# PRBonn/semantic_suma

Measured on AMD Instinct MI355X. Metric: scans_per_sec, higher is better.
Workload: dtype f32; 1 GPU; BASELINE configs[1]: synthetic KITTI-like sequence, 64x2048 range images, semantic-weighted ICP (10 GN iterations + stats pass) + surfel fusion, one sequence per GPU, scans resident in HBM, processScan called scan after scan by the native host loop (suma_pipeline_run_scans); timed after 300 untimed scans of the same sequence (5 warm-up + pre-roll to the steady map size: 1016645 surfels at the star; preroll_scans=300, map_surfels_start=1016645, map_surfels_end=2308753, parallelism=single GPU

## Files before the change

### semantic_suma_amd/core.py

```python
from __future__ import annotations

import ctypes as C
import os

import numpy as np

from .types import (ACC_WORDS, DRAW_COLORS, DRAW_LIGHTS, DRAW_MATERIAL, DRAW_MAX_LIGHTS, SURFEL_DTYPE, DrawParams,
                    IcpStats, LoopParams, LoopStatus, PosegraphParams, PosegraphStats, SemanticKnnParams,
                    SemanticParams, SumaParams, WORLD_SURFEL_DTYPE, WorldParams, WorldStats, CheckpointInfo,
                    LocalizerParams, LocalizerResult)

_HERE = os.path.dirname(os.path.abspath(__file__))
LIB_PATH = os.environ.get("SUMA_HIP_LIB") or os.path.join(_HERE, "libsuma_hip.so")
_LIB = None


class SumaError(RuntimeError):
    """Raised for every negative return code of the C-ABI (the reference throws std::runtime_error)."""


class LoopResult(C.Structure):
    _fields_ = [("gn_pose", C.c_double * 16), ("after_minimize", IcpStats), ("passed", C.c_int32),
                ("pose_old", C.c_float * 16), ("composed", IcpStats), ("JtJ", C.c_double * 36)]

# ... 6 lines not shown
class ScanRef(C.Structure):
    _fields_ = [("points", C.c_void_p), ("labels", C.c_void_p), ("probs", C.c_void_p), ("n", C.c_uint32)]


class SequenceJob(C.Structure):
    _fields_ = [("scans", C.POINTER(ScanRef)), ("n_scans", C.c_uint32), ("on_device", C.c_int32)]


class SequenceResult(C.Structure):
    _fields_ = [("status", C.c_int32), ("scans_done", C.c_uint32), ("map_surfels", C.c_uint32), ("track_loss", C.c_uint32),
                ("end_pose", C.c_double * 16), ("seconds", C.c_double), ("error", C.c_char * 160)]


class HypothesisJob(C.Structure):
    _fields_ = [("scans", C.POINTER(ScanRef)), ("n_scans", C.c_uint32), ("on_device", C.c_int32),
                ("perturbations", C.c_void_p), ("n_hyp", C.c_uint32), ("rank", C.c_uint32), ("world", C.c_uint32)]


EXCHANGE_FN = C.CFUNCTYPE(C.c_int, C.c_void_p, C.POINTER(C.c_double), C.POINTER(C.c_double), C.c_uint32)


class IcpObjective(C.Structure):
    _fields_ = [("icp_max_distance", C.c_float), ("icp_max_angle", C.c_float), ("weight_function", C.c_int32),
                ("factor", C.c_float), ("bilinear_sampling", C.c_int32)]


class KernelTime(C.Structure):
    _fields_ = [("name", C.c_char * 48), ("launches", C.c_uint64), ("total_ms", C.c_double), ("bytes", C.c_double)]


def lib():
    global _LIB
    if _LIB is not None:
        return _LIB
    if not os.path.exists(LIB_PATH):
        raise SumaError(f"{LIB_PATH} not found: build it with `make -C semantic_suma_amd/csrc` "
                        "(there is no CPU fallback for the HIP path)")
    L = C.CDLL(LIB_PATH)
    vp, u32, i32, f32 = C.c_void_p, C.c_uint32, C.c_int32, C.c_float
    pp = C.POINTER(vp)
    L.suma_version.restype = C.c_char_p
    L.suma_posegraph_last_error.restype = C.c_char_p
    L.suma_posegraph_last_error.argtypes = [vp]
    L.suma_posegraph_create.argtypes = [C.c_int, u32, u32, pp]
    L.suma_posegraph_destroy.argtypes = [vp]
    L.suma_posegraph_destroy.restype = None
    L.suma_posegraph_clear.argtypes = [vp]
    L.suma_posegraph_clone.argtypes = [vp, pp]
    L.suma_posegraph_set_initial.argtypes = [vp, i32, vp]
    L.suma_posegraph_add_edge.argtypes = [vp, i32, i32, vp, vp]
    L.suma_posegraph_pose.argtypes = [vp, i32, vp]
    L.suma_posegraph_poses.argtypes = [vp, vp, u32, C.POINTER(u32)]
    L.suma_posegraph_size.argtypes = [vp]
    L.suma_posegraph_size.restype = i32
    L.suma_posegraph_edge_count.argtypes = [vp]
    L.suma_posegraph_edge_count.restype = u32
    L.suma_posegraph_error.argtypes = [vp, C.POINTER(C.c_double)]
    L.suma_posegraph_reinitialize.argtypes = [vp]
    L.suma_posegraph_optimize.argtypes = [vp, u32, C.POINTER(PosegraphParams), C.POINTER(PosegraphStats)]
    L.suma_posegraph_linearize.argtypes = [vp, vp, vp, vp, vp, vp, vp, u32, C.POINTER(u32)]
    L.suma_posegraph_reserve.argtypes = [vp, u32, u32]
    L.suma_posegraph_edge.argtypes = [vp, u32, C.POINTER(i32), C.POINTER(i32), vp, vp]
    L.suma_loop_params_default.argtypes = [C.POINTER(LoopParams)]
    L.suma_loop_params_default.restype = None
    L.suma_pipeline_enable_loop_closing.argtypes = [vp, C.POINTER(LoopParams)]
    L.suma_pipeline_check_loop_closure.argtypes = [vp]
    L.suma_pipeline_loop_status.argtypes = [vp, C.POINTER(LoopStatus)]
    L.suma_pipeline_posegraph.argtypes = [vp]
    L.suma_pipeline_posegraph.restype = vp
    L.suma_pipeline_trajectory_distances.argtypes = [vp, vp, u32, C.POINTER(u32)]
    L.suma_loop_find_candidate.argtypes = [vp, vp, u32, vp, f32, f32, i32]
    L.suma_loop_find_candidate.restype = i32
    L.suma_last_error.restype = C.c_char_p
    L.suma_last_error.argtypes = [vp]
    L.suma_ctx_create.argtypes = [C.POINTER(SumaParams), C.c_int, pp]
    L.suma_ctx_destroy.argtypes = [vp]
    L.suma_ctx_destroy.restype = None
    L.suma_set_params.argtypes = [vp, C.POINTER(SumaParams)]
    L.suma_synchronize.argtypes = [vp]
    L.suma_ctx_stream.restype = vp
    L.suma_ctx_stream.argtypes = [vp]
    L.suma_frame_create.argtypes = [vp, u32, u32, pp]
    L.suma_frame_destroy.argtypes = [vp]
    L.suma_frame_destroy.restype = None
    L.suma_frame_copy.argtypes = [vp, vp, vp]
    L.suma_frame_download.argtypes = [vp, vp, C.c_int, vp]
    L.suma_frame_upload.argtypes = [vp, vp, C.c_int, vp]
    L.suma_frame_width.restype = u32
    L.suma_frame_width.argtypes = [vp]
    L.suma_frame_height.restype = u32
    L.suma_frame_height.argtypes = [vp]
    L.suma_frame_device_ptr.restype = vp
    L.suma_frame_device_ptr.argtypes = [vp, C.c_int]
    L.suma_frame_swap.argtypes = [vp, vp, vp]
    L.suma_frame_export.argtypes = [vp, vp, C.c_int, pp, C.POINTER(u32), C.POINTER(u32), C.POINTER(u32)]
    L.suma_icp_set_objective.argtypes = [vp, C.POINTER(IcpObjective)]
    L.suma_icp_information.argtypes = [vp, vp]
    L.suma_map_export_surfels.argtypes = [vp, pp, C.POINTER(u32)]
    L.suma_map_export_data_surfels.argtypes = [vp, pp, C.POINTER(u32), C.POINTER(u32)]
    L.suma_pipeline_prefetch_scan.argtypes = [vp, vp, vp, vp, u32]
    L.suma_pipeline_process_prefetched.argtypes = [vp, i32]
    L.suma_pipeline_process_scan_async.argtypes = [vp, vp, vp, vp, u32, i32]
    L.suma_device_download.argtypes = [vp, vp, vp, C.c_uint64]
    L.suma_preprocess.argtypes = [vp, vp, vp, vp, u32, u32, vp]
    L.suma_preprocess_device.argtypes = [vp, vp, vp, vp, u32, u32, vp]
    L.suma_icp_set_data.argtypes = [vp, vp, vp]
    L.suma_icp_jacobian_products.argtypes = [vp, vp, u32, vp, vp, vp, C.POINTER(IcpStats)]
    L.suma_icp_minimize.argtypes = [vp, vp, vp, vp, u32, C.POINTER(u32), C.POINTER(IcpStats)]
    L.suma_icp_history.argtypes = [vp, vp, u32, C.POINTER(u32)]
    L.suma_icp_history_sequence.argtypes = [vp]
    L.suma_icp_history_sequence.restype = C.c_uint64
    L.suma_frame_touch.argtypes = [vp, vp]
    L.suma_pipeline_minimize_stats.argtypes = [vp, C.POINTER(IcpStats)]
    L.suma_icp_minimize_batch.argtypes = [vp, vp, u32, vp, vp]
    L.suma_map_reset.argtypes = [vp]
    L.suma_map_update.argtypes = [vp, vp, vp]
    L.suma_map_render.argtypes = [vp, vp, vp, f32, vp]
    L.suma_map_render_active.argtypes = [vp, vp, f32]
    L.suma_map_render_inactive.argtypes = [vp, vp, f32]
    L.suma_map_render_composed.argtypes = [vp, vp, vp, f32]
    L.suma_map_frame.restype = vp
    L.suma_map_frame.argtypes = [vp, C.c_int]
    L.suma_map_update_poses.argtypes = [vp, vp, u32]
    L.suma_map_size.argtypes = [vp, C.POINTER(u32)]
    L.suma_map_timestamp.argtypes = [vp, C.POINTER(u32)]
    L.suma_map_download.argtypes = [vp, vp, u32, C.POINTER(u32)]
    L.suma_map_upload.argtypes = [vp, vp, u32, u32]
    L.suma_map_download_index_map.argtypes = [vp, vp]
    L.suma_map_download_radius_conf.argtypes = [vp, vp]
    L.suma_map_download_poses.argtypes = [vp, vp, u32, C.POINTER(u32)]
    L.suma_map_download_integrated.argtypes = [vp, vp]
    L.suma_map_counts.argtypes = [vp, C.POINTER(u32), C.POINTER(u32), C.POINTER(u32), vp]
    L.suma_map_cache_stats.argtypes = [vp, C.POINTER(u32), C.POINTER(u32), C.POINTER(u32)]
    L.suma_map_download_cached_tile.argtypes = [vp, C.c_int32, C.c_int32, vp, u32, C.POINTER(u32)]
    L.suma_icp_set_iteration.argtypes = [vp, u32]
    L.suma_pipeline_host_entry_times.argtypes = [vp, vp, C.c_int]
    L.suma_loop_closure_verify.argtypes = [vp, vp, vp, vp, u32, vp, f32, f32, f32, C.POINTER(LoopResult)]
    L.suma_loop_closure_verify_serial.argtypes = [vp, vp, vp, vp, u32, vp, f32, f32, f32, C.POINTER(LoopResult)]
    L.suma_pipeline_create.argtypes = [C.POINTER(SumaParams), C.c_int, pp]
    L.suma_pipeline_destroy.argtypes = [vp]
    L.suma_pipeline_destroy.restype = None
    L.suma_pipeline_ctx.restype = vp
    L.suma_pipeline_ctx.argtypes = [vp]
    L.suma_pipeline_process_scan.argtypes = [vp, vp, vp, vp, u32, i32]
    L.suma_pipeline_process_scan_device.argtypes = [vp, vp, vp, vp, u32, i32]
    L.suma_pipeline_pose.argtypes = [vp, vp]
    L.suma_pipeline_begin_scan.argtypes = [vp, vp, vp, vp, u32]
    L.suma_pipeline_begin_scan_device.argtypes = [vp, vp, vp, vp, u32]
    L.suma_pipeline_begin_prefetched.argtypes = [vp]
    L.suma_pipeline_update_pose.argtypes = [vp, i32]
    L.suma_pipeline_update_map.argtypes = [vp]
    L.suma_pipeline_integrate_loop_closures.argtypes = [vp, vp, u32, vp]
    L.suma_pipeline_set_pose_old.argtypes = [vp, vp]
    L.suma_pipeline_get_pose.argtypes = [vp, C.c_int, vp]
    L.suma_pipeline_result_new.argtypes = [vp, C.POINTER(IcpStats)]
    L.suma_pipeline_verify_loop_closure.argtypes = [vp, vp, vp, u32, f32, f32, C.POINTER(LoopResult)]
    L.suma_pipeline_track_loop_closure.argtypes = [vp, C.c_double, C.c_double, C.c_double, C.POINTER(LoopTrack)]
    L.suma_loop_closure_track.argtypes = [vp, vp, vp, vp, vp, f32, C.c_double, C.c_double, C.c_double, C.POINTER(LoopTrack)]
    L.suma_se3_log.argtypes = [vp, vp]
    L.suma_se3_log.restype = None
    L.suma_pipeline_reset.argtypes = [vp]
    L.suma_pipeline_minimize_hypotheses.argtypes = [vp, vp, u32, i32, vp, vp]
    L.suma_pipeline_apply_increment.argtypes = [vp, vp]
    L.suma_run_sequences.argtypes = [C.POINTER(SumaParams), C.c_int, C.POINTER(SequenceJob), u32, u32, i32,
                                     C.POINTER(SequenceResult)]
    L.suma_run_hypotheses.argtypes = [C.POINTER(SumaParams), C.c_int, C.POINTER(HypothesisJob), i32, EXCHANGE_FN, vp, vp,
                                      vp, C.c_char_p]
    L.suma_pipeline_run_scans.argtypes = [vp, C.POINTER(SequenceJob), i32, C.POINTER(u32), vp]
    L.suma_pipeline_last_increment.argtypes = [vp, vp]
    L.suma_pipeline_last_stats.argtypes = [vp, C.POINTER(IcpStats)]
    L.suma_pipeline_timestamp.restype = u32
    L.suma_pipeline_timestamp.argtypes = [vp]
    L.suma_pipeline_track_loss.restype = u32
    L.suma_pipeline_track_loss.argtypes = [vp]
    L.suma_pipeline_frame.restype = vp
    L.suma_pipeline_frame.argtypes = [vp, C.c_int]
    sp = C.POINTER(SemanticParams)
    L.suma_semantic_project.argtypes = [vp, sp, vp, u32, vp, vp, vp]
    L.suma_semantic_unproject.argtypes = [vp, sp, vp, C.c_int, vp, u32, vp, vp]
    L.suma_pipeline_begin_scan_scores.argtypes = [vp, sp, vp, vp, C.c_int, vp, u32, vp]
    L.suma_pipeline_process_scan_scores.argtypes = [vp, sp, vp, vp, C.c_int, vp, u32, vp, i32]
    kp = C.POINTER(SemanticKnnParams)
    L.suma_semantic_unproject_knn.argtypes = [vp, sp, kp, vp, vp, C.c_int, vp, vp, u32, vp, vp]
    L.suma_pipeline_begin_scan_scores_knn.argtypes = [vp, sp, kp, vp, vp, C.c_int, vp, vp, u32, vp]
    L.suma_pipeline_process_scan_scores_knn.argtypes = [vp, sp, kp, vp, vp, C.c_int, vp, vp, u32, vp, i32]
    L.suma_map_draw.argtypes = [vp, C.POINTER(DrawParams), vp, vp]
    L.suma_world_params_default.argtypes = [C.POINTER(WorldParams)]
    L.suma_world_params_default.restype = None
    L.suma_map_cached_tiles.argtypes = [vp, vp, u32, C.POINTER(u32)]
    L.suma_map_export_world.argtypes = [vp, C.POINTER(WorldParams), vp, u32, C.POINTER(WorldStats)]
    L.suma_device_alloc.argtypes = [vp, C.c_uint64, pp]
    L.suma_device_free.argtypes = [vp, vp]
    L.suma_device_upload.argtypes = [vp, vp, vp, C.c_uint64]
    L.suma_profile_enable.argtypes = [vp, C.c_int]
    L.suma_profile_reset.argtypes = [vp]
    L.suma_profile_get.argtypes = [vp, C.POINTER(KernelTime), u32]
    u64p = C.POINTER(C.c_uint64)
    L.suma_pipeline_checkpoint_size.argtypes = [vp, u64p]
    L.suma_pipeline_checkpoint_save.argtypes = [vp, vp, C.c_uint64, u64p]
    L.suma_pipeline_checkpoint_load.argtypes = [vp, vp, C.c_uint64]
    L.suma_checkpoint_info.argtypes = [vp, C.c_uint64, C.POINTER(CheckpointInfo)]
    L.suma_checkpoint_params.argtypes = [vp, C.c_uint64, C.POINTER(SumaParams)]
    L.suma_checkpoint_digest.argtypes = [vp, C.c_uint64]
    L.suma_checkpoint_digest.restype = C.c_uint64
    lpp, lrp = C.POINTER(LocalizerParams), C.POINTER(LocalizerResult)
    L.suma_localizer_params_default.argtypes = [C.POINTER(SumaParams), lpp]
    L.suma_localizer_params_default.restype = None
    L.suma_localizer_create.argtypes = [C.POINTER(SumaParams), lpp, C.c_int, pp]
    L.suma_localizer_destroy.argtypes = [vp]
    L.suma_localizer_destroy.restype = None
    L.suma_localizer_ctx.argtypes = [vp]
    L.suma_localizer_ctx.restype = vp
    L.suma_localizer_set_map.argtypes = [vp, vp, u32, C.POINTER(u32)]
    L.suma_localizer_set_map_device.argtypes = [vp, vp, u32, C.POINTER(u32)]
    L.suma_localizer_set_pose.argtypes = [vp, vp]
    L.suma_localizer_process_scan.argtypes = [vp, vp, vp, vp, u32, i32, lrp]
    L.suma_localizer_process_scan_device.argtypes = [vp, vp, vp, vp, u32, i32, lrp]
    L.suma_localizer_window.argtypes = [vp, vp, C.POINTER(u32), C.POINTER(u32)]
    L.suma_localizer_download_window.argtypes = [vp, vp, u32, C.POINTER(u32)]
    _LIB = L
    return L


def _ptr(a):
    return None if a is None else a.ctypes.data_as(C.c_void_p)


def _cm(T, dtype):
    return np.ascontiguousarray(np.asarray(T, dtype=dtype).reshape(4, 4).T)


class Context:

    def __init__(self, params: SumaParams, device: int = 0, handle=None, owner=None):
        self.L = lib()
        self.params = params
        self._owner = owner
        if handle is None:
            h = C.c_void_p()
            rc = self.L.suma_ctx_create(C.byref(params), device, C.byref(h))
            if rc != 0:
                raise SumaError(f"suma_ctx_create failed ({rc}): {self.L.suma_last_error(None).decode()}")
            self.h, self.owned = h, True
        else:
            self.h, self.owned = handle, False

    def check(self, rc: int, what: str = ""):
        if rc != 0:
            raise SumaError(f"{what} failed ({rc}): {self.L.suma_last_error(self.h).decode()}")

    def set_params(self, params: SumaParams):
        self.check(self.L.suma_set_params(self.h, C.byref(params)), "suma_set_params")
        self.params = params

    def synchronize(self):
        self.check(self.L.suma_synchronize(self.h), "suma_synchronize")

    @property
    def stream(self) -> int:
        return int(self.L.suma_ctx_stream(self.h) or 0)

    def device_array(self, host: np.ndarray) -> int:
        host = np.ascontiguousarray(host)
        p = C.c_void_p()
        self.check(self.L.suma_device_alloc(self.h, host.nbytes, C.byref(p)), "suma_device_alloc")
        self.check(self.L.suma_device_upload(self.h, p, _ptr(host), host.nbytes), "suma_device_upload")
        return p.value

    def device_download(self, d_ptr: int, nbytes: int) -> np.ndarray:
        out = np.empty(nbytes, dtype=np.uint8)
        self.check(self.L.suma_device_download(self.h, _ptr(out), C.c_void_p(d_ptr), nbytes), "suma_device_download")
        return out

    def device_free(self, p: int):
        self.check(self.L.suma_device_free(self.h, C.c_void_p(p)), "suma_device_free")

    def profile(self, on):
        self.check(self.L.suma_profile_enable(self.h, int(on)))

    def profile_reset(self):
        self.check(self.L.suma_profile_reset(self.h))

    def profile_get(self):
        buf = (KernelTime * 64)()
        n = self.L.suma_profile_get(self.h, buf, 64)
        if n < 0:
            self.check(n, "suma_profile_get")
        return [dict(name=buf[i].name.decode(), launches=int(buf[i].launches), total_ms=float(buf[i].total_ms),
                     bytes=float(buf[i].bytes)) for i in range(min(n, 64))]

    def close(self):
        if getattr(self, "owned", False) and self.h:
            self.L.suma_ctx_destroy(self.h)
            self.h = None

    def __del__(self):
        try:
            self.close()
        except Exception:
            pass


class Frame:

    def __init__(self, ctx: Context, width: int, height: int, handle=None):
        self.ctx, self.width, self.height = ctx, width, height
        if handle is None:
            h = C.c_void_p()
            ctx.check(ctx.L.suma_frame_create(ctx.h, width, height, C.byref(h)), "suma_frame_create")
            self.h, self.owned = h, True
        else:
            self.h, self.owned = C.c_void_p(handle), False

    def download(self, which: int) -> np.ndarray:
        out = np.empty((self.height, self.width, 4), dtype=np.float32)
        self.ctx.check(self.ctx.L.suma_frame_download(self.ctx.h, self.h, which, _ptr(out)), "suma_frame_download")
        return out

    def upload(self, which: int, data: np.ndarray):
        data = np.ascontiguousarray(data, dtype=np.float32).reshape(self.height, self.width, 4)
        self.ctx.check(self.ctx.L.suma_frame_upload(self.ctx.h, self.h, which, _ptr(data)), "suma_frame_upload")

    def set(self, vertex, normal, semantic):
        self.upload(0, vertex)
        self.upload(1, normal)
        self.upload(2, semantic)

    @property
    def vertex(self):
        return self.download(0)

    @property
    def normal(self):
        return self.download(1)

    @property
    def semantic(self):
        return self.download(2)

    def swap(self, other: "Frame"):
        self.ctx.check(self.ctx.L.suma_frame_swap(self.ctx.h, self.h, other.h), "suma_frame_swap")

    def export(self, which: int):
        p, w, h, rb = C.c_void_p(), C.c_uint32(0), C.c_uint32(0), C.c_uint32(0)
        self.ctx.check(self.ctx.L.suma_frame_export(self.ctx.h, self.h, which, C.byref(p), C.byref(w), C.byref(h),
                                                    C.byref(rb)), "suma_frame_export")
        return p.value, w.value, h.value, rb.value

    def touch(self):
        self.ctx.check(self.ctx.L.suma_frame_touch(self.ctx.h, self.h), "suma_frame_touch")

    def copy(self, other: "Frame"):
        self.ctx.check(self.ctx.L.suma_frame_copy(self.ctx.h, self.h, other.h), "suma_frame_copy")

    def __del__(self):
        try:
            if getattr(self, "owned", False) and self.h and self.ctx.h:
                self.ctx.L.suma_frame_destroy(self.h)
                self.h = None
        except Exception:
            pass


class Preprocessing:

    def __init__(self, ctx: Context):
        self.ctx = ctx

    def process(self, points, frame: Frame, labels, probs, timestamp: int) -> Frame:
        points = np.ascontiguousarray(points, dtype=np.float32).reshape(-1, 4)
        labels = None if labels is None else np.ascontiguousarray(labels, dtype=np.float32)
        probs = None if probs is None else np.ascontiguousarray(probs, dtype=np.float32)
        c = self.ctx
        c.check(c.L.suma_preprocess(c.h, _ptr(points), _ptr(labels), _ptr(probs), points.shape[0], timestamp, frame.h),
                "suma_preprocess")
        return frame


class Frame2Model:
    num_parameters = 6
    _PARAM_NAMES = {"icp-max-distance": "icp_max_distance", "icp-max-angle": "icp_max_angle", "factor": "factor",
                    "bilinear_sampling": "bilinear_sampling"}
    _WEIGHTING = {"none": 0, "huber": 1, "turkey": 2, "stability": 3}

    def __init__(self, ctx: Context, params: SumaParams = None):
        self.ctx = ctx
        p = ctx.params if params is None else params
        self.objective = IcpObjective(p.icp_max_distance, p.icp_max_angle, p.weight_function, p.factor,
                                      p.bilinear_sampling)
        self._current = self._last = None
        self._pose = np.eye(4)
        self._iteration = 0
        self.stats = IcpStats()
        self.acc = np.zeros(ACC_WORDS, dtype=np.int64)

    def setParameter(self, name: str, value):
        if name == "weighting":
            self.objective.weight_function = self._WEIGHTING[value]
        elif name in self._PARAM_NAMES:
            setattr(self.objective, self._PARAM_NAMES[name], value)

    def setData(self, current: Frame, last: Frame):
        self._current, self._last = current, last
        self._iteration = 0

    def _bind(self):
        if self._current is None:
            raise SumaError("Frame2Model::setData has not been called")
        c = self.ctx
        c.check(c.L.suma_icp_set_data(c.h, self._current.h, self._last.h), "suma_icp_set_data")
# ... 1065 lines not shown
```

### semantic_suma_amd/csrc/k_render.hip

```cpp
#include <cstring>

#include "suma_internal.h"
#define EXDIV_FN __device__ __forceinline__
#include "exact_div.h"

enum { TIE_LOW_INDEX = 0, TIE_HIGH_INDEX_OLD = 1, TIE_HIGH_INDEX_NEW = 2 };

struct RenderSlot {
  int enabled;
  int mode;
  int tie;
  unsigned long long* zbuf;
  m4 inv_pose;
};

struct RenderArgs {
  const suma_surfel* surfels;
  const DevState* ds;
  const float* poses;
  proj_t q;
  float conf_threshold;
  int use_stability;
  int32_t thr;
  RenderSlot slot[2];
  int merged;
  const float* inv_pose_dev;
  int k7_enabled;
  int k7_same_proj;
  proj_t k7_q;
  unsigned long long* k7_zbuf;
};

struct rvtx {
  int32_t X, Y;
  float z, tu, tv;
};

__device__ __forceinline__ double edge_fn(const rvtx& a, const rvtx& b, int32_t px, int32_t py) {
  const double ux = (double)(b.X - a.X), uy = (double)(b.Y - a.Y), vx = (double)(px - a.X), vy = (double)(py - a.Y);
  return __builtin_fma(ux, vy, -(uy * vx));
}
__device__ __forceinline__ float edge_to_float(double w) { return (float)(w + 0.0); }
__device__ __forceinline__ bool owns_edge(const rvtx& s, const rvtx& t) {
  int32_t dx = t.X - s.X, dy = t.Y - s.Y;
  return dy > 0 || (dy == 0 && dx < 0);
}

__device__ __forceinline__ unsigned long long render_key(uint32_t z24, uint32_t id, int tie) {
  if (tie == TIE_LOW_INDEX) return ((unsigned long long)z24 << 32) | id;
  unsigned long long pass = (tie == TIE_HIGH_INDEX_OLD) ? 1u : 0u;
  return ((unsigned long long)z24 << 33) | (pass << 32) | (unsigned long long)(0xffffffffu - id);
}

__device__ __forceinline__ unsigned long long raster_key(rvtx A, rvtx B, rvtx C, int32_t i, int32_t j, uint32_t id,
                                                         int tie) {
  double area = edge_fn(A, B, C.X, C.Y);
  if (area < 0) {
    rvtx t = B;
    B = C;
    C = t;
    area = -area;
  }
  const int32_t px = 256 * i + 128, py = 256 * j + 128;
  const double w0 = edge_fn(B, C, px, py), w1 = edge_fn(C, A, px, py), w2 = edge_fn(A, B, px, py);
  const bool covered = (area != 0) && (w0 > 0 || (w0 == 0 && owns_edge(B, C))) &&
                       (w1 > 0 || (w1 == 0 && owns_edge(C, A))) && (w2 > 0 || (w2 == 0 && owns_edge(A, B)));
  unsigned long long key = SUMA_EMPTY_KEY;
  if (covered) {
    const float fa = (float)area;
#ifdef SUMA_BARY_PLAIN_DIV
    float b0 = edge_to_float(w0) / fa, b1 = edge_to_float(w1) / fa, b2 = edge_to_float(w2) / fa;
#else
    const float fr = exdiv_refine(fa, __builtin_amdgcn_rcpf(fa));
    float b0 = exdiv_quot(edge_to_float(w0), fa, fr), b1 = exdiv_quot(edge_to_float(w1), fa, fr),
          b2 = exdiv_quot(edge_to_float(w2), fa, fr);
#endif
    float tu = (b0 * A.tu + b1 * B.tu) + b2 * C.tu;
    float tv = (b0 * A.tv + b1 * B.tv) + b2 * C.tv;
    float z = (b0 * A.z + b1 * B.z) + b2 * C.z;
    if (!((tu * tu + tv * tv) > 1.0f) && (z >= 0.0f && z <= 1.0f)) key = render_key(depth24(z), id, tie);
  }
  return key;
}

__device__ __forceinline__ void surfel_to_sensor(const float* __restrict__ poses, const float* inv_pose, float count,
                                                 v3 pos, v3 nrm, v3* p, v3* n) {
  float Ps[16], M[16];
  const float4* src = reinterpret_cast<const float4*>(poses + 16 * (size_t)(int32_t)count);
#pragma unroll
  for (int k = 0; k < 4; ++k) {
    float4 col = src[k];
    Ps[4 * k] = col.x;
    Ps[4 * k + 1] = col.y;
    Ps[4 * k + 2] = col.z;
    Ps[4 * k + 3] = col.w;
  }
  m4_mul(inv_pose, Ps, M);
  *p = m4_point(M, pos);
  *n = m4_dir(M, nrm);
}

#ifdef SUMA_PHASE_TIMING
__device__ unsigned long long g_k4_phase[PH_BLOCKS][9];
extern "C" int suma_debug_k4_phases(unsigned long long* host, int reset) {
  hipError_t e = hipMemcpyFromSymbol(host, HIP_SYMBOL(g_k4_phase), sizeof(g_k4_phase));
  if (e == hipSuccess && reset) {
    void* p = nullptr;
    e = hipGetSymbolAddress(&p, HIP_SYMBOL(g_k4_phase));
    if (e == hipSuccess) e = hipMemset(p, 0, sizeof(g_k4_phase));
  }
  return (int)e;
}
#endif

#if !defined(K4_NO_PREFETCH)
#define K4_PREFETCH 1
#endif
#ifdef K4_PREFETCH
#define K4_BARRIER() lds_barrier()
#else
#define K4_BARRIER() __syncthreads()
#endif
#define RENDER_THREADS 256
#define RENDER_WAVES (RENDER_THREADS / 64)
#define RENDER_BATCH 2
#define SUMA_RENDER_MAX_BLOCKS 65536u

__device__ __forceinline__ uint32_t render_block_rank(bool flag, uint32_t* s_w, uint32_t* total) {
  const int lane = threadIdx.x & 63, wave = threadIdx.x >> 6;
  const unsigned long long ball = __ballot(flag);
  if (lane == 0) s_w[wave] = __popcll(ball);
  K4_BARRIER();
  uint32_t off = 0, tot = 0;
#pragma unroll
  for (int w = 0; w < RENDER_WAVES; ++w) {
    uint32_t c = s_w[w];
    if (w < wave) off += c;
    tot += c;
  }
  *total = tot;
  return off + __popcll(ball & ((1ull << lane) - 1ull));
}

template <bool BIG>
__global__ void __launch_bounds__(RENDER_THREADS) __attribute__((amdgpu_waves_per_eu(5, 8))) k_render(RenderArgs a) {
  __shared__ float s_cand[RENDER_THREADS][9];
  __shared__ int32_t s_rec[RENDER_THREADS][17];
  __shared__ uint32_t s_incl[RENDER_THREADS];
  __shared__ uint32_t s_w[2][RENDER_WAVES], s_w2[RENDER_WAVES];
  __shared__ uint8_t s_mask[RENDER_THREADS];
  const uint32_t S = a.ds->n_surfels;
  const float4* __restrict__ sf = reinterpret_cast<const float4*>(a.surfels);
  const int lane = threadIdx.x & 63, wave = threadIdx.x >> 6;
  const uint32_t ntile = (S + RENDER_THREADS - 1) / RENDER_THREADS;
  const int npass = a.merged ? 1 : 2;
  uint32_t trip = 0;
  float4 s0 = f4(0, 0, 0, 0), s1 = s0, s2 = s0;
  auto fetch_tile = [&](uint32_t t) {
    const uint32_t tt = t < ntile ? t : ntile - 1u;
    uint32_t j = (ntile - 1u - tt) * RENDER_THREADS + threadIdx.x;
    j = j < S ? j : S - 1u;
    s0 = sf[4 * (size_t)j];
    s1 = sf[4 * (size_t)j + 1];
    s2 = sf[4 * (size_t)j + 2];
  };
#ifdef K4_PREFETCH
  if (ntile) fetch_tile(blockIdx.x);
  const int last_pass = a.merged ? 0 : (a.slot[1].enabled ? 1 : 0);
#endif
  PH_BEGIN;
  for (uint32_t tile = blockIdx.x; tile < ntile; tile += gridDim.x) {
    PH(7);
    const uint32_t blk0 = (ntile - 1u - tile) * RENDER_THREADS;
    const uint32_t i = blk0 + threadIdx.x;
#ifndef K4_PREFETCH
    fetch_tile(tile);
#endif
    const bool live = (i < S) && !(a.use_stability && !(s1.w > a.conf_threshold));
    const float radius = s0.w, count = s2.w;
    const int32_t creation = (int32_t)count;
    const int32_t ts = (int32_t)__float_as_uint(s2.x);
#ifdef SUMA_PHASE_TIMING
    if (live && ts == 0x7fffffff) ph_acc[7] += 1;
#endif
    PH(0);
    for (int sl = 0; sl < npass; ++sl) {
      const RenderSlot& slot = a.slot[a.merged ? 1 : sl];
      if (!a.merged && !slot.enabled) continue;
      const float* inv_pose = (sl == 0 && a.inv_pose_dev != nullptr) ? a.inv_pose_dev : slot.inv_pose.m;
      uint32_t selmask;
      {
        const bool sel_old = live && (creation < a.thr), sel_new = live && (creation >= a.thr || ts >= a.thr);
        if (a.merged)
          selmask = ((sel_old && a.slot[0].enabled) ? 1u : 0u) | (sel_new ? 2u : 0u);
        else
          selmask = ((slot.mode == 0) ? sel_old : sel_new) ? (1u << sl) : 0u;
      }
      const bool selected = selmask != 0;
      const bool k7 = (sl == 0) && a.k7_enabled && (i < S);
      bool cand = false;
      unsigned long long k7_key = SUMA_EMPTY_KEY;
      uint32_t k7_pix = 0;
      v3 p = mk3(0, 0, 0), n = p;
      float ppx = 0.f;
      if (selected || k7) {
        surfel_to_sensor(a.poses, inv_pose, count, xyz(s0), xyz(s1), &p, &n);
        float lp = len3(p);
        if (dot3(n, divs3(neg3(p), lp)) > 0.01f) {
          v3 pp = mk3(0, 0, 0);
          if (selected || a.k7_same_proj) pp = project01(a.q, p);
          if (k7) {
            const v3 pr = a.k7_same_proj ? pp : project01(a.k7_q, p);
            float fx = sdm_floor(pr.x * a.k7_q.width), fy = sdm_floor(pr.y * a.k7_q.height);
            float zn = 2.0f * pr.z - 1.0f;
            if (fx >= 0.0f && fx < a.k7_q.width && fy >= 0.0f && fy < a.k7_q.height && zn >= -1.0f && zn <= 1.0f) {
              k7_key = ((unsigned long long)depth24(0.5f * zn + 0.5f) << 32) | i;
              k7_pix = (uint32_t)(int32_t)fy * (uint32_t)a.k7_q.W + (uint32_t)(int32_t)fx;
            }
          }
          if (selected) {
            cand = (pp.x >= 0.0f && pp.y >= 0.0f && pp.z >= 0.0f && pp.x < 1.0f && pp.y < 1.0f && pp.z < 1.0f);
            ppx = pp.x;
          }
        }
      }
#ifdef K4_PREFETCH
      if (sl == last_pass) fetch_tile(tile + gridDim.x);
#endif
      uint32_t ncand;
      const uint32_t crank = render_block_rank(cand, s_w[trip & 1u], &ncand);
      trip += 1;
      PH(1);
      if (ncand == 0) {
        if (k7_key != SUMA_EMPTY_KEY) zbuf_min(&a.k7_zbuf[k7_pix], k7_key);
        continue;
      }
      if (cand) {
        float* r = s_cand[crank];
        r[0] = p.x;
        r[1] = p.y;
        r[2] = p.z;
        r[3] = n.x;
        r[4] = n.y;
        r[5] = n.z;
        r[6] = radius;
        r[7] = ppx;
        r[8] = __uint_as_float(i);
        s_mask[crank] = (uint8_t)selmask;
      }
      K4_BARRIER();
      PH(2);
      uint32_t ntests = 0;
      if (threadIdx.x < ncand) {
        const float* r = s_cand[threadIdx.x];
        const v3 cp = mk3(r[0], r[1], r[2]), cn = mk3(r[3], r[4], r[5]);
        const float crad = r[6], cppx = r[7];
        v3 u = normalize3(mk3(cn.y - cn.z, -cn.x, cn.x));
        v3 v = normalize3(cross3(cn, u));
        v3 ru = scale3(crad, u), rv = scale3(crad, v);
        v3 corner[4];
        corner[0] = sub3(sub3(cp, ru), rv);
        corner[1] = sub3(add3(cp, ru), rv);
        corner[2] = add3(sub3(cp, ru), rv);
        corner[3] = add3(add3(cp, ru), rv);
        int32_t X[4], Y[4];
        float Z[4];
        bool bad = false;
#pragma unroll
        for (int k = 0; k < 4; ++k) {
          const float depth = len3(corner[k]);
          const float pitch = -sdm_asin(corner[k].z / depth);
          const float y01 = 1.0f - ((pitch * SUMA_RAD2DEG_F) + a.q.fov_up) / a.q.fov;
          Z[k] = 0.5f * (2.0f * ((depth - a.q.min_depth) / (a.q.max_depth - a.q.min_depth)) - 1.0f) + 0.5f;
          const float yw = y01 * a.q.height;
          if (sdm_isnan(yw) || sdm_isnan(Z[k])) bad = true;
          Y[k] = (int32_t)sdm_floor(yw * 256.0f + 0.5f);
        }
        const int32_t minY = min(min(Y[0], Y[1]), min(Y[2], Y[3])), maxY = max(max(Y[0], Y[1]), max(Y[2], Y[3]));
        int32_t j0 = (minY - 128 + 255) >> 8, j1 = (maxY - 128) >> 8;
        j0 = max(j0, 0);
        j1 = min(j1, a.q.H - 1);
        if (!bad && j0 <= j1) {
#pragma unroll
          for (int k = 0; k < 4; ++k) {
            const float yaw = sdm_atan2(corner[k].y, corner[k].x);
            float x01 = 0.5f * ((-yaw * SUMA_INV_PI_F) + 1.0f);
            if (cppx - x01 > 0.5f) x01 += 1.0f;
            if (x01 - cppx > 0.5f) x01 -= 1.0f;
            const float xw = x01 * a.q.width;
            if (sdm_isnan(xw)) bad = true;
            X[k] = (int32_t)sdm_floor(xw * 256.0f + 0.5f);
          }
          if (!bad) {
            const int32_t minX = min(min(X[0], X[1]), min(X[2], X[3])), maxX = max(max(X[0], X[1]), max(X[2], X[3]));
            int32_t i0 = (minX - 128 + 255) >> 8, i1 = (maxX - 128) >> 8;
            i0 = max(i0, 0);
            i1 = min(i1, a.q.W - 1);
            if (i0 <= i1) {
              const int32_t w = i1 - i0 + 1;
              ntests = (uint32_t)w * (uint32_t)(j1 - j0 + 1);
              int32_t* q = s_rec[threadIdx.x];
#pragma unroll
              for (int k = 0; k < 4; ++k) {
                q[k] = X[k];
                q[4 + k] = Y[k];
                q[8 + k] = __float_as_int(Z[k]);
              }
              q[12] = i0;
              q[13] = j0;
              q[14] = w;
              q[15] = __float_as_int(r[8]);
              q[16] = (int32_t)s_mask[threadIdx.x];
            }
          }
        }
      }
      PH(3);
      uint32_t incl = wave_inclusive_scan(ntests);
      if (lane == 63) s_w2[wave] = incl;
      K4_BARRIER();
      uint32_t woff = 0, total = 0;
#pragma unroll
      for (int w = 0; w < RENDER_WAVES; ++w) {
        uint32_t c = s_w2[w];
        if (w < wave) woff += c;
        total += c;
      }
      s_incl[threadIdx.x] = incl + woff;
      K4_BARRIER();
      PH(4);
      unsigned long long k7_cur = 0;
      if (k7_key != SUMA_EMPTY_KEY)
        k7_cur = __hip_atomic_load(&a.k7_zbuf[k7_pix], __ATOMIC_RELAXED, __HIP_MEMORY_SCOPE_AGENT);
      unsigned long long* const zb0 = a.slot[0].zbuf;
      unsigned long long* const zb1 = a.slot[1].zbuf;
      for (uint32_t t0 = threadIdx.x; t0 < total; t0 += RENDER_BATCH * RENDER_THREADS) {
        unsigned long long key[RENDER_BATCH];
        uint32_t pix[RENDER_BATCH], msk[RENDER_BATCH];
#pragma unroll
        for (int u = 0; u < RENDER_BATCH; ++u) {
          const uint32_t t = t0 + (uint32_t)u * RENDER_THREADS;
          key[u] = SUMA_EMPTY_KEY;
          pix[u] = 0;
          msk[u] = 0;
          if (t < total) {
            int lo = 0, hi = RENDER_THREADS - 1;
#pragma unroll
            for (int it = 0; it < 8; ++it) {
              int mid = (lo + hi) >> 1;
              if (s_incl[mid] > t)
                hi = mid;
              else
                lo = mid + 1;
            }
            const int src = lo;
            const uint32_t excl = src ? s_incl[src - 1] : 0u;
            const int32_t* r = s_rec[src];
            const uint32_t q = t - excl, w = (uint32_t)r[14];
            const uint32_t qj = BIG ? q / w : (uint32_t)(((float)q + 0.5f) * __builtin_amdgcn_rcpf((float)w));
            const uint32_t qi = q - __umul24(qj, w);
            const int32_t pi = r[12] + (int32_t)qi, pj = r[13] + (int32_t)qj;
            rvtx vt[4];
#pragma unroll
            for (int k = 0; k < 4; ++k) {
              vt[k].X = r[k];
              vt[k].Y = r[4 + k];
              vt[k].z = __int_as_float(r[8 + k]);
              vt[k].tu = (k & 1) ? 1.0f : -1.0f;
              vt[k].tv = (k & 2) ? 1.0f : -1.0f;
            }
            const uint32_t id = (uint32_t)r[15];
            const unsigned long long ka = raster_key(vt[0], vt[1], vt[2], pi, pj, id, slot.tie);
            const unsigned long long kb = raster_key(vt[2], vt[1], vt[3], pi, pj, id, slot.tie);
            key[u] = ka < kb ? ka : kb;
            pix[u] = __umul24((uint32_t)pj, (uint32_t)a.q.W) + (uint32_t)pi;
            msk[u] = (uint32_t)r[16];
          }
        }
        unsigned long long cur0[RENDER_BATCH], cur1[RENDER_BATCH];
#pragma unroll
        for (int u = 0; u < RENDER_BATCH; ++u) {
          cur0[u] = cur1[u] = 0;
          if (key[u] != SUMA_EMPTY_KEY) {
            if (msk[u] & 1u) cur0[u] = __hip_atomic_load(&zb0[pix[u]], __ATOMIC_RELAXED, __HIP_MEMORY_SCOPE_AGENT);
            if (msk[u] & 2u) cur1[u] = __hip_atomic_load(&zb1[pix[u]], __ATOMIC_RELAXED, __HIP_MEMORY_SCOPE_AGENT);
          }
        }
#pragma unroll
        for (int u = 0; u < RENDER_BATCH; ++u) {
          if (key[u] < cur0[u]) atomicMin(&zb0[pix[u]], key[u]);
          if (key[u] < cur1[u]) atomicMin(&zb1[pix[u]], key[u]);
        }
      }
      if (k7_key < k7_cur) atomicMin(&a.k7_zbuf[k7_pix], k7_key);
      PH(5);
      K4_BARRIER();
      PH(6);
    }
  }
  PH_END(g_k4_phase);
}

__device__ __forceinline__ uint32_t key_id(unsigned long long key, int tie) {
  uint32_t low = (uint32_t)(key & 0xffffffffull);
  return tie == TIE_LOW_INDEX ? low : (0xffffffffu - low);
}

struct ResolveOut {
  float4 v, n, s;
};

__device__ __forceinline__ ResolveOut resolve_pixel(unsigned long long key, int tie, const suma_surfel* surfels,
                                                    const float* poses, const float* inv_a, const float* inv_b) {
  ResolveOut o;
  if (key == SUMA_EMPTY_KEY) {
    o.v = o.n = o.s = f4(0.f, 0.f, 0.f, 0.f);
    return o;
  }
  uint32_t id = key_id(key, tie);
  const float4* sf = reinterpret_cast<const float4*>(surfels) + 4 * (size_t)id;
  float4 s0 = sf[0], s1 = sf[1], s2 = sf[2], s3 = sf[3];
  const float* inv = inv_a;
  if (tie != TIE_LOW_INDEX && ((key >> 32) & 1ull) == 0) inv = inv_b;
  v3 p, n;
  surfel_to_sensor(poses, inv, s2.w, xyz(s0), xyz(s1), &p, &n);
  o.v = f4(p.x, p.y, p.z, 1.0f);
  o.n = f4(n.x, n.y, n.z, 1.0f);
  o.s = s3;
  return o;
}

struct ResolveArgs {
  const suma_surfel* surfels;
  const float* poses;
  unsigned long long *zbuf_a, *zbuf_b;
  m4 inv_a, inv_b;
  int tie;
  uint32_t Pm;
  float max_distance;
  float4 *va, *na, *sa;
  float4 *vb, *nb, *sb;
  float4 *vo, *no, *so;
  float4 *vm, *nm, *sm;
  const float4* sm_src;
  const float* inv_dev;
};

__global__ void __launch_bounds__(256) k_resolve(ResolveArgs a) {
  uint32_t pix = blockIdx.x * blockDim.x + threadIdx.x;
  if (pix >= a.Pm) return;
  unsigned long long key = a.zbuf_a[pix];
  a.zbuf_a[pix] = SUMA_EMPTY_KEY;
  const float* ia = a.inv_dev ? a.inv_dev : a.inv_a.m;
  const float* ib = a.inv_dev ? a.inv_dev : a.inv_b.m;
  ResolveOut o = resolve_pixel(key, a.tie, a.surfels, a.poses, ia, ib);
  if (a.va) a.va[pix] = o.v;
  if (a.na) a.na[pix] = o.n;
  if (a.sa) a.sa[pix] = o.s;
  if (a.vm) {
    a.vm[pix] = o.v;
    a.nm[pix] = o.n;
    a.sm[pix] = a.sm_src[pix];
  }
}

__global__ void __launch_bounds__(256) k_resolve_compose(ResolveArgs a) {
  uint32_t pix = blockIdx.x * blockDim.x + threadIdx.x;
  if (pix >= a.Pm) return;
  unsigned long long ka = a.zbuf_a[pix], kb = a.zbuf_b[pix];
  a.zbuf_a[pix] = SUMA_EMPTY_KEY;
  a.zbuf_b[pix] = SUMA_EMPTY_KEY;
  ResolveOut o = resolve_pixel(ka, TIE_LOW_INDEX, a.surfels, a.poses, a.inv_a.m, a.inv_a.m);
  ResolveOut nw = resolve_pixel(kb, TIE_LOW_INDEX, a.surfels, a.poses, a.inv_b.m, a.inv_b.m);
  a.va[pix] = o.v;
  a.na[pix] = o.n;
  a.sa[pix] = o.s;
  a.vb[pix] = nw.v;
  a.nb[pix] = nw.n;
  a.sb[pix] = nw.s;
  float4 v = nw.v, n = nw.n, s = nw.s;
  bool valid = (o.v.w > 0.5f && o.n.w > 0.5f);
  bool new_valid = (v.w > 0.5f && n.w > 0.5f);
  if (!new_valid && valid && (v.w < 0.5f || len3(sub3(xyz(v), xyz(o.v))) < a.max_distance)) {
    v = o.v;
    n = o.n;
    s = o.s;
  }
  a.vo[pix] = v;
  a.no[pix] = n;
  a.so[pix] = s;
}

static void set_m4(m4& d, const float* s) {
  for (int i = 0; i < 16; ++i) d.m[i] = s[i];
}

static void run_render(suma_ctx* c, const RenderArgs& a, uint32_t grid) {
  if ((size_t)a.q.W * (size_t)a.q.H >= ((size_t)1 << 21))
    k_render<true><<<grid, RENDER_THREADS, 0, c->ls>>>(a);
  else
    k_render<false><<<grid, RENDER_THREADS, 0, c->ls>>>(a);
}
static RenderArgs render_args(suma_ctx* c, float conf_threshold, int32_t thr) {
  RenderArgs a;
  a.surfels = c->surfels[c->cur];
  a.ds = c->ds;
  a.poses = c->poses;
  a.q = c->pm;
  a.conf_threshold = conf_threshold;
  a.use_stability = c->p.use_stability;
  a.thr = thr;
  a.slot[0].enabled = a.slot[1].enabled = 0;
  a.slot[0].zbuf = a.slot[1].zbuf = c->zbuf_a;
  a.slot[0].tie = a.slot[1].tie = TIE_LOW_INDEX;
  a.merged = 0;
  a.inv_pose_dev = nullptr;
  a.k7_enabled = 0;
  a.k7_q = c->pd;
  a.k7_same_proj = (memcmp(&c->pd, &c->pm, sizeof(proj_t)) == 0) ? 1 : 0;
  a.k7_zbuf = c->zbuf_data;
  return a;
}
static uint32_t stream_grid(suma_ctx* c) {
  uint64_t est = (uint64_t)c->known_surfels + 2 * c->P;
  uint64_t blocks = (est + 255) / 256;
  if (blocks > SUMA_RENDER_MAX_BLOCKS) blocks = SUMA_RENDER_MAX_BLOCKS;
  if (blocks < 256) blocks = 256;
  return (uint32_t)blocks;
}
static ResolveArgs resolve_args(suma_ctx* c) {
  ResolveArgs r;
  memset(&r, 0, sizeof(r));
  r.surfels = c->surfels[c->cur];
  r.poses = c->poses;
  r.zbuf_a = c->zbuf_a;
  r.zbuf_b = c->zbuf_b;
  r.Pm = (uint32_t)c->Pm;
  r.max_distance = c->p.max_loop_closure_distance;
  return r;
}

hipError_t launch_map_render(suma_ctx* c, const float* pose_old, const float* pose_new, float conf_threshold,
                             suma_frame* out) {
  float inv_old[16], inv_new[16];
  rigid_inverse_f(pose_old, inv_old);
  rigid_inverse_f(pose_new, inv_new);
  const double S = (double)c->known_surfels;
  const uint32_t Pm = (uint32_t)c->Pm;
  if (c->p.compose_rendering) {
    int32_t thr = (int32_t)(c->timestamp - 100u);
    RenderArgs a = render_args(c, conf_threshold, thr);
    a.slot[0].enabled = thr > 0 ? 1 : 0;
    a.slot[0].mode = 0;
    a.slot[0].tie = TIE_LOW_INDEX;
    a.slot[0].zbuf = c->zbuf_a;
    set_m4(a.slot[0].inv_pose, inv_old);
    a.slot[1].enabled = 1;
    a.slot[1].mode = 1;
    a.slot[1].tie = TIE_LOW_INDEX;
    a.slot[1].zbuf = c->zbuf_b;
    set_m4(a.slot[1].inv_pose, inv_new);
    a.merged = (memcmp(inv_old, inv_new, sizeof(inv_old)) == 0 && !getenv("SUMA_RENDER_NO_MERGE")) ? 1 : 0;
    {
      ProfScope ps(c, "k4_render_surfels", 64.0 * S);
      run_render(c, a, stream_grid(c));
    }
    ResolveArgs r = resolve_args(c);
    set_m4(r.inv_a, inv_old);
    set_m4(r.inv_b, inv_new);
    r.va = c->old_frame->map[0];
    r.na = c->old_frame->map[1];
    r.sa = c->old_frame->map[2];
    r.vb = c->new_frame->map[0];
    r.nb = c->new_frame->map[1];
    r.sb = c->new_frame->map[2];
    r.vo = out->map[0];
    r.no = out->map[1];
    r.so = out->map[2];
    {
      ProfScope ps(c, "k5_resolve_compose", (16.0 + 144.0) * Pm);
      k_resolve_compose<<<(Pm + 255) / 256, 256, 0, c->ls>>>(r);
    }
  } else {
    RenderArgs a = render_args(c, conf_threshold, 0);
    a.slot[0].enabled = 1;
    a.slot[0].mode = 1;
    a.slot[0].tie = TIE_LOW_INDEX;
    a.slot[0].zbuf = c->zbuf_a;
    set_m4(a.slot[0].inv_pose, inv_old);
    {
      ProfScope ps(c, "k4_render_surfels", 64.0 * S);
      run_render(c, a, stream_grid(c));
    }
    ResolveArgs r = resolve_args(c);
    set_m4(r.inv_a, inv_old);
    set_m4(r.inv_b, inv_old);
    r.tie = TIE_LOW_INDEX;
    r.va = out->map[0];
    r.na = out->map[1];
    r.sa = out->map[2];
    {
      ProfScope ps(c, "k5_resolve", (8.0 + 48.0) * Pm);
      k_resolve<<<(Pm + 255) / 256, 256, 0, c->ls>>>(r);
    }
    size_t bytes = c->Pm * sizeof(float4);
    for (int m = 0; m < 3; ++m) {
      hipMemcpyAsync(c->new_frame->map[m], out->map[m], bytes, hipMemcpyDeviceToDevice, c->ls);
      hipMemcpyAsync(c->old_frame->map[m], out->map[m], bytes, hipMemcpyDeviceToDevice, c->ls);
    }
  }
  return hipGetLastError();
}

hipError_t launch_map_render_single(suma_ctx* c, const float* pose, float conf_threshold, int active, int fuse_k7,
                                    suma_frame* mirror) {
  float inv[16] = {1, 0, 0, 0, 0, 1, 0, 0, 0, 0, 1, 0, 0, 0, 0, 1};
  if (pose) rigid_inverse_f(pose, inv);
  int32_t thr = (int32_t)(c->timestamp - 100u);
  RenderArgs a = render_args(c, conf_threshold, thr);
  if (!pose) a.inv_pose_dev = c->pose_block + 16;
  a.slot[0].enabled = 1;
  a.slot[0].mode = active ? 1 : 0;
  a.slot[0].tie = TIE_LOW_INDEX;
  a.slot[0].zbuf = c->zbuf_a;
  set_m4(a.slot[0].inv_pose, inv);
  a.k7_enabled = fuse_k7;
  {
    ProfScope ps(c, fuse_k7 ? "k4k7_render_indexmap" : "k4_render_surfels", 64.0 * (double)c->known_surfels);
    run_render(c, a, stream_grid(c));
  }
  ResolveArgs r = resolve_args(c);
  set_m4(r.inv_a, inv);
  set_m4(r.inv_b, inv);
  r.tie = TIE_LOW_INDEX;
  if (!pose) r.inv_dev = c->pose_block + 16;
  suma_frame* tgt = active ? c->new_frame : c->old_frame;
  r.va = tgt->map[0];
  r.na = tgt->map[1];
  r.sa = nullptr;
  if (mirror) {
    r.vm = mirror->map[0];
    r.nm = mirror->map[1];
    r.sm = mirror->map[2];
    r.sm_src = tgt->map[2];
  }
  {
    ProfScope ps(c, "k5_resolve", (8.0 + 32.0 + (mirror ? 64.0 : 0.0)) * (double)c->Pm);
    k_resolve<<<((uint32_t)c->Pm + 255) / 256, 256, 0, c->ls>>>(r);
  }
  return hipGetLastError();
}

hipError_t launch_map_render_composed(suma_ctx* c, const float* pose_old, const float* pose_new,
                                      float conf_threshold) {
  float inv_old[16], inv_new[16];
  rigid_inverse_f(pose_old, inv_old);
  rigid_inverse_f(pose_new, inv_new);
  int32_t thr = (int32_t)(c->timestamp - 100u);
  RenderArgs a = render_args(c, conf_threshold, thr);
  a.slot[0].enabled = 1;
  a.slot[0].mode = 0;
  a.slot[0].tie = TIE_HIGH_INDEX_OLD;
  a.slot[0].zbuf = c->zbuf_a;
  set_m4(a.slot[0].inv_pose, inv_old);
  a.slot[1].enabled = 1;
  a.slot[1].mode = 1;
  a.slot[1].tie = TIE_HIGH_INDEX_NEW;
  a.slot[1].zbuf = c->zbuf_a;
  set_m4(a.slot[1].inv_pose, inv_new);
  {
    ProfScope ps(c, "k4_render_surfels", 64.0 * (double)c->known_surfels);
    run_render(c, a, stream_grid(c));
  }
  ResolveArgs r = resolve_args(c);
  set_m4(r.inv_a, inv_old);
  set_m4(r.inv_b, inv_new);
  r.tie = TIE_HIGH_INDEX_OLD;
  r.va = c->composed_frame->map[0];
  r.na = c->composed_frame->map[1];
  r.sa = nullptr;
  {
    ProfScope ps(c, "k5_resolve", (8.0 + 32.0) * (double)c->Pm);
    k_resolve<<<((uint32_t)c->Pm + 255) / 256, 256, 0, c->ls>>>(r);
  }
  return hipGetLastError();
}
```

### semantic_suma_amd/csrc/k_update.hip

```cpp
#include <cstddef>
#include <cstring>

#include "suma_internal.h"

#define ST_AGG 1u
#define ST_INC 2u

__device__ __forceinline__ unsigned long long st_pack(uint32_t epoch, uint32_t flag, uint32_t value) {
  return ((unsigned long long)epoch << 34) | ((unsigned long long)flag << 32) | value;
}

struct Pair {
  uint32_t a, x;
};
__device__ __forceinline__ void lookback_publish(unsigned long long* __restrict__ status,
                                                 unsigned long long* __restrict__ group, uint32_t tile, uint32_t agg,
                                                 uint32_t epoch, uint32_t aggx = 0) {
  __hip_atomic_store(&status[tile], st_pack(epoch, ST_AGG, (aggx << 16) | agg), __ATOMIC_RELAXED, __HIP_MEMORY_SCOPE_AGENT);
  __hip_atomic_fetch_add(&group[tile >> 6], (1ull << 56) | ((unsigned long long)aggx << 32) | (unsigned long long)agg,
                         __ATOMIC_RELAXED, __HIP_MEMORY_SCOPE_AGENT);
}
#define SUMA_SPIN_LIMIT (1u << 26)
#ifndef LB_BATCH
#define LB_BATCH 4
// ... 37 lines not shown
  if (timed_out) {
    atomicOr(fault, 8u);
    atomicOr(fault + (offsetof(DevState, fault_site) - offsetof(DevState, overflow)) / 4, 0x2u);
  }
  Pair r;
  r.a = (uint32_t)__builtin_amdgcn_readlane((int)wave_inclusive_scan(sum), 63);
  r.x = PAIR ? (uint32_t)__builtin_amdgcn_readlane((int)wave_inclusive_scan(sumx), 63) : 0u;
  return r;
}
__device__ __forceinline__ uint32_t lookback_collect(unsigned long long* __restrict__ status,
                                                     unsigned long long* __restrict__ group, uint32_t tile, uint32_t epoch,
                                                     int lane, uint32_t* __restrict__ fault) {
  return lookback_collect2<false>(status, group, tile, epoch, lane, fault).a;
}
__device__ uint32_t lookback_prefix(unsigned long long* __restrict__ status, unsigned long long* __restrict__ group,
                                    uint32_t tile, uint32_t agg, uint32_t epoch, int lane, uint32_t* __restrict__ fault) {
  if (lane == 0) lookback_publish(status, group, tile, agg, epoch);
  return lookback_collect(status, group, tile, epoch, lane, fault);
}

struct BlockRank {
  uint32_t rank, total;
};
#define TILE_WAVES (SUMA_TILE / 64)
__device__ __forceinline__ BlockRank block_rank(bool flag, uint32_t* s_wave ) {
  const int lane = threadIdx.x & 63, wave = threadIdx.x >> 6;
  const unsigned long long ball = __ballot(flag);
  const uint32_t below = __popcll(ball & ((1ull << lane) - 1ull));
  if (lane == 0) s_wave[wave] = __popcll(ball);
  __syncthreads();
  uint32_t off = 0, tot = 0;
#pragma unroll
  for (int w = 0; w < (int)TILE_WAVES; ++w) {
    uint32_t cnt = s_wave[w];
    if (w < wave) off += cnt;
    tot += cnt;
  }
  BlockRank r;
  r.rank = off + below;
  r.total = tot;
  return r;
}

__device__ __forceinline__ void block_rank2(bool fa, bool fb, uint32_t* s_wa, uint32_t* s_wb, BlockRank* ra, BlockRank* rb) {
  const int lane = threadIdx.x & 63, wave = threadIdx.x >> 6;
  const unsigned long long ba = __ballot(fa), bb = __ballot(fb);
  const unsigned long long lo = (1ull << lane) - 1ull;
  if (lane == 0) {
    s_wa[wave] = __popcll(ba);
    s_wb[wave] = __popcll(bb);
  }
  __syncthreads();
  uint32_t offa = 0, tota = 0, offb = 0, totb = 0;
#pragma unroll
  for (int w = 0; w < (int)TILE_WAVES; ++w) {
    const uint32_t ca = s_wa[w], cb = s_wb[w];
    if (w < wave) {
      offa += ca;
      offb += cb;
    }
    tota += ca;
    totb += cb;
  }
  ra->rank = offa + __popcll(ba & lo);
  ra->total = tota;
  rb->rank = offb + __popcll(bb & lo);
  rb->total = totb;
}

__device__ __forceinline__ bool is_finaliser(uint32_t failing_ticket, uint32_t ntiles) {
  return failing_ticket == ntiles + gridDim.x - 1;
}
__device__ __forceinline__ void finalise_tickets(DevState* ds, unsigned long long* group_next, uint32_t group_words) {
  for (uint32_t gi = threadIdx.x; gi < group_words; gi += blockDim.x) group_next[gi] = 0;
  if (threadIdx.x == 0) ds->ticket = 0;
}

__device__ __forceinline__ void commit_extraction(DevState* ds, CacheSlot* slots, uint32_t slot, uint32_t base,
                                                  uint32_t arena_cap, uint32_t n) {
  if (n > SUMA_EXTRACT_CAPACITY) {
    n = SUMA_EXTRACT_CAPACITY;
    atomicOr(&ds->overflow, 4u);
  }
  if ((uint64_t)base + n > arena_cap) {
    n = arena_cap - base;
    atomicOr(&ds->overflow, 2u);
  }
  slots[slot].offset = base;
  slots[slot].count = n;
  ds->cache_used = base + n;
  ds->n_extracted = n;
}

__device__ __forceinline__ void write_pose_entry(float* poses, float* poses_inv, uint32_t pose_idx, const m4& pose) {
  float inv[16];
  rigid_inverse_dev(pose.m, inv);
  for (int i = 0; i < 16; ++i) {
    poses[16 * (size_t)pose_idx + i] = pose.m[i];
    poses_inv[16 * (size_t)pose_idx + i] = inv[i];
  }
}
__global__ void __launch_bounds__(256)
    k8_radius(const float4* __restrict__ V, const float4* __restrict__ N, K8Out o, uint32_t P, DevState* ds,
              float* poses, float* poses_inv, uint32_t pose_idx, m4 pose, const float4* __restrict__ Sem) {
  uint32_t pix = blockIdx.x * blockDim.x + threadIdx.x;
  if (pix >= P) return;
  if (pix == 0) {
    ds->n_updated = 0;
    ds->n_data = 0;
    ds->n_kept_updated = 0;
    ds->n_kept_data = 0;
    write_pose_entry(poses, poses_inv, pose_idx, pose);
  }
  k8_pixel(o, pix, V[pix], N[pix], Sem[pix]);
}
__global__ void k8_pose_only(float* poses, float* poses_inv, uint32_t pose_idx, m4 pose) {
  if (threadIdx.x == 0 && blockIdx.x == 0) write_pose_entry(poses, poses_inv, pose_idx, pose);
}

struct UpdArgs {
  const suma_surfel* in;
  suma_surfel* out;
  DevState* ds;
  const float* poses;
  const float* poses_inv;
  unsigned long long* zbuf;
  unsigned long long* status;
  unsigned long long *group, *group_next;
  uint32_t group_words;
  uint32_t epoch;
  const float4 *V, *N, *Sem;
  const float4* radius_conf;
  const float4* pixrec;
  uint8_t* integrated;
  uint32_t* index_map;
  proj_t q;
  m4 pose, inv_pose;
  int32_t timestamp;
  uint32_t max_surfels;
  float confidence_threshold, map_max_distance, update_angle_thresh;
  float p_stable, p_unstable, log_prior, log_unstable, sigma_angle, sigma_distance, max_weight;
  int32_t use_stability, unstable_age, confidence_mode, active_timestamps, weighting_scheme, averaging_scheme,
      update_always;
  float cx, cy, extent;
  uint8_t* ex_flags;
  float ex_cx, ex_cy, ex_extent;
  suma_surfel* x_arena;
  CacheSlot* x_slots;
  uint32_t x_cap, x_slot;
  float* poses_w;
  float* poses_inv_w;
  uint32_t pose_idx;
  int write_pose;
};

__device__ __forceinline__ void load_pose(const float* __restrict__ table, int32_t idx, float* M) {
  const float4* src = reinterpret_cast<const float4*>(table + 16 * (size_t)idx);
#pragma unroll
  for (int k = 0; k < 4; ++k) {
    float4 col = src[k];
    M[4 * k] = col.x;
    M[4 * k + 1] = col.y;
    M[4 * k + 2] = col.z;
    M[4 * k + 3] = col.w;
  }
}

__global__ void __launch_bounds__(256) k7_indexmap(UpdArgs a) {
  const uint32_t S = a.ds->n_surfels;
  const float4* __restrict__ sf = reinterpret_cast<const float4*>(a.in);
  for (uint32_t i = blockIdx.x * blockDim.x + threadIdx.x; i < S; i += gridDim.x * blockDim.x) {
    float4 s0 = sf[4 * (size_t)i], s1 = sf[4 * (size_t)i + 1];
    float count = sf[4 * (size_t)i + 2].w;
    float Ps[16], M[16];
    load_pose(a.poses, (int32_t)count, Ps);
    m4_mul(a.inv_pose.m, Ps, M);
    v3 p = m4_point(M, xyz(s0)), n = m4_dir(M, xyz(s1));
    float lp = len3(p);
    if (!(dot3(n, divs3(neg3(p), lp)) > 0.01f)) continue;
    v3 pr = project01(a.q, p);
    float fx = sdm_floor(pr.x * a.q.width), fy = sdm_floor(pr.y * a.q.height);
    if (!(fx >= 0.0f && fx < a.q.width && fy >= 0.0f && fy < a.q.height)) continue;
    float zn = 2.0f * pr.z - 1.0f;
    if (!(zn >= -1.0f && zn <= 1.0f)) continue;
    unsigned long long key = ((unsigned long long)depth24(0.5f * zn + 0.5f) << 32) | i;
    zbuf_min(&a.zbuf[(size_t)(int32_t)fy * a.q.W + (size_t)(int32_t)fx], key);
  }
}

__device__ __forceinline__ v3 slerp3(v3 v0, v3 v1, float weight) {
  float omega = sdm_acos(dot3(normalize3(v0), normalize3(v1)));
  float so = sdm_sin(omega);
  if (!(so > 0.0f)) return v0;
  float eta = 1.0f / so;
  float w0 = eta * sdm_sin(weight * omega);
  float w1 = eta * sdm_sin((1.0f - weight) * omega);
  return add3(scale3(w0, v0), scale3(w1, v1));
}

struct Surfel4 {
  float4 a, b, c, d;
};

__device__ __forceinline__ bool in_active_area(const UpdArgs& a, const Surfel4& s, bool* in_tile) {
  float Ps[16];
  load_pose(a.poses, (int32_t)s.c.w, Ps);
  v3 pos = m4_point(Ps, xyz(s.a));
  *in_tile = !(sdm_abs(pos.x - a.ex_cx) > a.ex_extent || sdm_abs(pos.y - a.ex_cy) > a.ex_extent);
  if ((int32_t)__float_as_uint(s.c.x) < 0) return false;
  if (sdm_abs(pos.x - a.cx) > a.extent || sdm_abs(pos.y - a.cy) > a.extent) return false;
  return true;
}

__device__ __forceinline__ void store_surfel(suma_surfel* out, uint32_t idx, const Surfel4& s) {
  float4* o = reinterpret_cast<float4*>(out) + 4 * (size_t)idx;
  store_stream(o, s.a);
  store_stream(o + 1, s.b);
  store_stream(o + 2, s.c);
  store_stream(o + 3, s.d);
}

struct K9Pre {
  v3 old_position, old_normal;
  float imz;
  int32_t tx, ty;
  uint32_t rpix;
  bool in_tex, visible, inside;
};
struct K9Rec {
  float4 dv, dn, dx;
  unsigned long long k7key;
};

__device__ __forceinline__ K9Pre k9_prepare(const UpdArgs& a, const Surfel4& in) {
  K9Pre p;
  const int32_t creation_timestamp = (int32_t)in.c.w;
  float Ps[16];
  load_pose(a.poses, creation_timestamp, Ps);
  p.old_position = m4_point(Ps, xyz(in.a));
  p.old_normal = m4_dir(Ps, xyz(in.b));
  const v3 vertex = m4_point(a.inv_pose.m, p.old_position);
  const v3 normal = normalize3(m4_dir(a.inv_pose.m, p.old_normal));
  p.visible = dot3(normal, divs3(neg3(vertex), len3(vertex))) > 0.0f;
  const v3 pr = project01(a.q, vertex);
  const float imx = sdm_floor(pr.x * a.q.width) + 0.5f, imy = sdm_floor(pr.y * a.q.height) + 0.5f;
  p.imz = pr.z;
  p.in_tex = (imx >= 0.0f && imx < a.q.width && imy >= 0.0f && imy < a.q.height);
  p.tx = p.in_tex ? (int32_t)sdm_floor(imx) : -1;
  p.ty = p.in_tex ? (int32_t)sdm_floor(imy) : -1;
  p.rpix = (uint32_t)max(p.ty, 0) * (uint32_t)a.q.W + (uint32_t)max(p.tx, 0);
  p.inside = (imx < a.q.width && imy < a.q.height && p.imz < 1.0f) && !(imx < 0.0f && imy < 0.0f && p.imz < 0.0f);
  return p;
}

__device__ __forceinline__ K9Rec k9_gather(const UpdArgs& a, const K9Pre& p) {
  K9Rec r;
  const float4* __restrict__ rec = a.pixrec + 4 * (size_t)p.rpix;
  r.dv = rec[0];
  r.dn = rec[1];
  r.dx = rec[2];
  r.k7key = a.zbuf[p.rpix];
  return r;
}

__device__ __forceinline__ bool k9_finish(const UpdArgs& a, uint32_t i, const Surfel4& in, const K9Pre& p,
                                          const K9Rec& g, Surfel4& o, int32_t* mark_pix) {
  const int32_t timestamp = a.timestamp;
  const int32_t W = a.q.W;
  const int32_t surfel_age = timestamp - (int32_t)__float_as_uint(in.c.x);
  const int32_t creation_timestamp = (int32_t)in.c.w;
  const v3 old_position = p.old_position, old_normal = p.old_normal;
  const float old_radius = in.a.w, old_confidence = in.b.w, old_weight = in.c.z;

  bool keep = true;
  if (old_confidence < a.confidence_threshold && a.use_stability) keep = (surfel_age < a.unstable_age);
  o = in;
  o.c.y = pack_rgb(0.3f, 0.3f, 0.3f);

  float4 dv = g.dv, dn = g.dn, dx = g.dx;
  if (!p.in_tex) dv = dn = dx = f4(0.f, 0.f, 0.f, 0.f);
  const float4 ds = f4(dx.x, 0.f, 0.f, dx.y), rc = f4(dx.z, 0.f, 0.f, 0.f);
  const unsigned long long k7key = g.k7key;
  const bool valid = (dv.w > 0.5f) && (dn.w > 0.5f);
  const float imz = p.imz;
  const int32_t tx = p.tx, ty = p.ty;

  float penalty = 0.0f;
  float update_confidence = a.log_prior;
  bool mark = false;

  if (valid && p.inside && p.visible) {
    const float data_label = ds.x * 255.0f, data_prob = ds.w;
    const float model_label = in.d.x * 255.0f, model_prob = in.d.w;
    if (sdm_round(data_label) != sdm_round(model_label)) {
      if (is_dynamic_label(model_label)) penalty = 1.0f;
    }
    const v3 v = xyz(dv), n = xyz(dn);
    const v3 v_global = m4_point(a.pose.m, v);
    const v3 n_global = normalize3(m4_dir(a.pose.m, n));
    const v3 view_dir = divs3(neg3(v), len3(v));
    const float distance = sdm_abs(dot3(old_normal, sub3(v_global, old_position)));
    const float angle = len3(cross3(n_global, old_normal));
    const float new_radius = rc.x, new_confidence = rc.y;

    if ((distance < a.map_max_distance) && (angle < a.update_angle_thresh)) {
      mark = true;
      const float confidence = old_confidence + new_confidence;
      o.b.w = confidence;
      o.c.x = __uint_as_float((uint32_t)timestamp);
      float avg_radius = fmin_(new_radius, old_radius);
      avg_radius = fmax_(avg_radius, 0.0f);
      o.a.w = avg_radius;
      keep = true;
      o.c.y = pack_rgb(0.0f, 0.7f, 0.0f);
      o.c.w = (float)creation_timestamp;

      float pst = a.p_stable;
      if (a.confidence_mode == 1 || a.confidence_mode == 3)
        pst *= sdm_exp((-angle * angle) / (a.sigma_angle * a.sigma_angle));
      if (a.confidence_mode == 2 || a.confidence_mode == 3)
        pst *= sdm_exp((-distance * distance) / (a.sigma_distance * a.sigma_distance));
      pst = fclamp(pst, a.p_unstable, 1.0f);
      update_confidence = sdm_log(pst / (1.0f - pst));

      if ((new_radius < old_radius && timestamp - creation_timestamp < a.active_timestamps) || a.update_always) {
        float w1 = 0.9f, w2 = 0.1f;
        if (a.weighting_scheme > 0) {
          w1 = old_weight;
          w2 = 1.0f;
          if (a.weighting_scheme == 2) w2 = dot3(n, view_dir);
          o.c.z = fmin_(a.max_weight, w1 + w2);
          float sum = w1 + w2;
          w1 /= sum;
          w2 /= sum;
        }
        v3 avg_position = add3(scale3(w1, old_position), scale3(w2, v_global));
        v3 avg_normal = slerp3(old_normal, n_global, w1);
        float avg_prob;
        if (sdm_round(data_label) != sdm_round(model_label))
          avg_prob = w1 * model_prob + w2 * (1.0f - data_prob);
        else
          avg_prob = w1 * model_prob + w2 * data_prob;
        o.d.w = avg_prob;
        if (a.averaging_scheme == 1) {
          avg_position = add3(old_position, scale3(w2 * distance, old_normal));
          avg_normal = slerp3(old_normal, n_global, w1);
        }
        avg_normal = normalize3(avg_normal);
        float Pi[16];
        load_pose(a.poses_inv, creation_timestamp, Pi);
        avg_position = m4_point(Pi, avg_position);
        avg_normal = m4_dir(Pi, avg_normal);
        o.a = f4(avg_position.x, avg_position.y, avg_position.z, avg_radius);
        o.b = f4(avg_normal.x, avg_normal.y, avg_normal.z, confidence);
        o.c.y = pack_rgb(1.0f, 0.0f, 1.0f);
      }
    } else {
      int32_t idx = (k7key == SUMA_EMPTY_KEY) ? -1 : (int32_t)(uint32_t)(k7key & 0xffffffffull);
      if (idx == (int32_t)i) {
        update_confidence = sdm_log(a.p_unstable / (1.0f - a.p_unstable));
        o.c.y = pack_rgb(0.0f, 1.0f, 1.0f);
      }
    }
  }
  update_confidence = update_confidence - penalty;
  if (a.use_stability)
    o.b.w = fmin_((old_confidence + update_confidence) - a.log_prior, 20.0f);
  else
    o.b.w = old_confidence;
  if (o.b.w < a.log_unstable && a.use_stability) keep = false;

  *mark_pix = -1;
  if (keep && mark) {
    float zn = 2.0f * imz - 1.0f;
    if (zn >= -1.0f && zn <= 1.0f) *mark_pix = ty * W + tx;
  }
  return keep;
}

#ifndef K9_PER
#define K9_PER 1
#endif
#define K9_THREADS (SUMA_TILE / K9_PER)
#define K9_WAVES (K9_THREADS / 64)
static_assert(SUMA_TILE % K9_PER == 0 && K9_THREADS <= 1024, "K9 tile split");

__device__ __forceinline__ Surfel4 load_surfel(const float4* __restrict__ sf, uint32_t i) {
  Surfel4 r;
  r.a = sf[4 * (size_t)i];
  r.b = sf[4 * (size_t)i + 1];
  r.c = sf[4 * (size_t)i + 2];
  r.d = sf[4 * (size_t)i + 3];
  return r;
}

#if defined(__HIP_DEVICE_COMPILE__) && !defined(UPD_NO_ARG_RELOAD)
#define UPD_ARG_RELOAD 1
#endif
#ifdef UPD_ARG_RELOAD
typedef const UpdArgs __attribute__((address_space(4))) * UpdArgsK;
__device__ __forceinline__ UpdArgsK upd_args_again(UpdArgsK p) {
  asm volatile("" : "+s"(p));
  return p;
}
#endif

#ifdef SUMA_PHASE_TIMING
__device__ unsigned long long g_k9_phase[PH_BLOCKS][9];
extern "C" int suma_debug_k9_phases(unsigned long long* host, int reset) {
  hipError_t e = hipMemcpyFromSymbol(host, HIP_SYMBOL(g_k9_phase), sizeof(g_k9_phase));
  if (e == hipSuccess && reset) {
    void* p = nullptr;
    e = hipGetSymbolAddress(&p, HIP_SYMBOL(g_k9_phase));
    if (e == hipSuccess) e = hipMemset(p, 0, sizeof(g_k9_phase));
  }
  return (int)e;
}
#endif

#ifndef K9_DEFER
#define K9_DEFER 1
#endif
#define K9_BUFS (K9_DEFER ? 2 : 1)
template <bool XF>
__global__ void __launch_bounds__(K9_THREADS)
#if !K9_DEFER
    __attribute__((amdgpu_waves_per_eu(2 * K9_WAVES / 4, 2 * K9_WAVES / 4)))
#endif
    k9_update(UpdArgs a) {
  __shared__ float4 s_out[K9_BUFS][SUMA_TILE][4];
  __shared__ uint16_t s_slot[K9_BUFS][SUMA_TILE];
  __shared__ uint8_t s_ext[K9_BUFS][SUMA_TILE];
  __shared__ uint16_t s_xrank[XF ? K9_BUFS : 1][XF ? SUMA_TILE : 1];
  __shared__ uint32_t s_cnt_emit[K9_PER][K9_WAVES], s_cnt_keep[K9_WAVES], s_cnt_x[K9_PER][K9_WAVES];
  __shared__ uint32_t s_tile, s_prefix, s_prefix_x;
  const uint32_t xbase = XF ? a.ds->cache_used : 0u;
  float4* __restrict__ xdst4 = reinterpret_cast<float4*>(a.x_arena);
  const uint32_t S = a.ds->n_surfels;
  const uint32_t ntiles = (S + SUMA_TILE - 1) / SUMA_TILE;
  const float4* __restrict__ sf = reinterpret_cast<const float4*>(a.in);
  float4* __restrict__ dst4 = reinterpret_cast<float4*>(a.out);
  const int lane = threadIdx.x & 63, wave = threadIdx.x >> 6;
  uint32_t keep_count = 0;
  if (a.write_pose && blockIdx.x == 0 && threadIdx.x == 0) write_pose_entry(a.poses_w, a.poses_inv_w, a.pose_idx, a.pose);
  uint32_t prev_tile = 0xffffffffu, prev_total = 0, prev_totalx = 0, buf = 0;
#ifdef UPD_ARG_RELOAD
  const UpdArgsK ka = (UpdArgsK)__builtin_amdgcn_kernarg_segment_ptr();
#endif
  auto stream_out = [&](uint32_t pb, uint32_t tile_id, uint32_t count, uint32_t countx) {
    const uint32_t prefix = s_prefix, prefix_x = XF ? s_prefix_x : 0u;
    for (uint32_t c = threadIdx.x; c < 4u * count; c += K9_THREADS) {
      const uint64_t d = 4ull * prefix + c;
      if (d < 4ull * a.max_surfels) {
        const uint32_t slot = s_slot[pb][c >> 2];
        const float4 v = s_out[pb][slot][c & 3u];
        store_stream(&dst4[d], v);
        if (XF) {
          if (s_ext[pb][slot]) {
            const uint32_t xr = prefix_x + s_xrank[pb][slot];
            if (xr < SUMA_EXTRACT_CAPACITY && (uint64_t)xbase + xr < a.x_cap)
              store_stream(&xdst4[4ull * ((uint64_t)xbase + xr) + (c & 3u)], v);
          }
        } else if (a.ex_flags != nullptr && (c & 3u) == 0) {
          a.ex_flags[d >> 2] = s_ext[pb][slot];
        }
      }
    }
    if (tile_id == ntiles - 1 && threadIdx.x == 0) {
      const uint32_t tot = prefix + count;
      a.ds->n_kept_updated = tot < a.max_surfels ? tot : a.max_surfels;
      if (XF) a.ds->n_ext_update = prefix_x + countx;
    }
  };
  PH_BEGIN;
  for (;;) {
    PH(7);
    lds_barrier();
    if (threadIdx.x == 0)
      s_tile = __hip_atomic_fetch_add(&a.ds->ticket, 1u, __ATOMIC_RELAXED, __HIP_MEMORY_SCOPE_AGENT);
    lds_barrier();
    const uint32_t tile = s_tile;
    PH(0);
    uint32_t total = 0, totalx = 0;
    if (tile < ntiles) {
      uint32_t idx[K9_PER];
      bool live[K9_PER], emit[K9_PER];
      Surfel4 in[K9_PER];
      K9Pre pre[K9_PER];
      K9Rec rec[K9_PER];
#pragma unroll
      for (int u = 0; u < K9_PER; ++u) {
        idx[u] = tile * SUMA_TILE + (uint32_t)u * K9_THREADS + threadIdx.x;
        live[u] = idx[u] < S;
        in[u] = load_surfel(sf, live[u] ? idx[u] : 0u);
      }
#ifdef UPD_ARG_RELOAD
      const UpdArgs aA = *upd_args_again(ka);
#else
      const UpdArgs& aA = a;
#endif
#pragma unroll
      for (int u = 0; u < K9_PER; ++u) pre[u] = k9_prepare(aA, in[u]);
#ifdef SUMA_PHASE_TIMING
      if (__float_as_uint(in[0].a.x) == 0x7fc12345u) ph_acc[7] += 1;
#endif
      PH(1);
#pragma unroll
      for (int u = 0; u < K9_PER; ++u) rec[u] = k9_gather(aA, pre[u]);
#ifdef UPD_ARG_RELOAD
      const UpdArgs aB = *upd_args_again(ka);
#else
      const UpdArgs& aB = a;
#endif
      uint32_t kept = 0;
      unsigned long long eb[K9_PER], xb[K9_PER];
      bool xt[K9_PER];
#pragma unroll
      for (int u = 0; u < K9_PER; ++u) {
        Surfel4 o;
        int32_t mark_pix;
        const bool keep = k9_finish(aB, idx[u], in[u], pre[u], rec[u], o, &mark_pix) && live[u];
        if (keep && mark_pix >= 0) aB.integrated[mark_pix] = 1;
        bool in_tile;
        emit[u] = in_active_area(aB, o, &in_tile) && keep;
        const uint32_t slot = (uint32_t)u * K9_THREADS + threadIdx.x;
        xt[u] = in_tile && emit[u];
        xb[u] = XF ? __ballot(xt[u]) : 0ull;
        s_ext[buf][slot] = in_tile ? 1 : 0;
        s_out[buf][slot][0] = o.a;
        s_out[buf][slot][1] = o.b;
        s_out[buf][slot][2] = o.c;
        s_out[buf][slot][3] = o.d;
        eb[u] = __ballot(emit[u]);
        kept += __popcll(__ballot(keep));
      }
      PH(2);
      if (lane == 0) {
        s_cnt_keep[wave] = kept;
#pragma unroll
        for (int u = 0; u < K9_PER; ++u) {
          s_cnt_emit[u][wave] = __popcll(eb[u]);
          if (XF) s_cnt_x[u][wave] = __popcll(xb[u]);
        }
      }
      lds_barrier();
      uint32_t kc = 0, base = 0, basex = 0;
      const unsigned long long below = (1ull << lane) - 1ull;
#pragma unroll
      for (int u = 0; u < K9_PER; ++u) {
        uint32_t off = 0, tot = 0;
#pragma unroll
        for (int w = 0; w < K9_WAVES; ++w) {
          const uint32_t cnt = s_cnt_emit[u][w];
          if (w < wave) off += cnt;
          tot += cnt;
        }
        if (emit[u]) s_slot[buf][base + off + __popcll(eb[u] & below)] = (uint16_t)((uint32_t)u * K9_THREADS + threadIdx.x);
        base += tot;
        if (XF) {
          uint32_t offx = 0, totx = 0;
#pragma unroll
          for (int w = 0; w < K9_WAVES; ++w) {
            const uint32_t cnt = s_cnt_x[u][w];
            if (w < wave) offx += cnt;
            totx += cnt;
          }
          if (xt[u]) s_xrank[buf][(uint32_t)u * K9_THREADS + threadIdx.x] = (uint16_t)(basex + offx + __popcll(xb[u] & below));
          basex += totx;
        }
      }
#pragma unroll
      for (int w = 0; w < K9_WAVES; ++w) kc += s_cnt_keep[w];
      total = base;
      totalx = basex;
      if (threadIdx.x == 0) {
        keep_count += kc;
        lookback_publish(a.status, a.group, tile, total, a.epoch, totalx);
      }
      PH(3);
    }
    if (prev_tile != 0xffffffffu) {
      if (threadIdx.x < 64) {
        const Pair pre = lookback_collect2<XF>(a.status, a.group, prev_tile, a.epoch, threadIdx.x, &a.ds->overflow);
        if (threadIdx.x == 0) {
          s_prefix = pre.a;
          if (XF) s_prefix_x = pre.x;
        }
      }
      lds_barrier();
      PH(4);
      stream_out(buf ^ 1u, prev_tile, prev_total, prev_totalx);
      PH(5);
    }
    if (tile >= ntiles) break;
    prev_tile = tile;
    prev_total = total;
    prev_totalx = totalx;
#if K9_DEFER
    buf ^= 1u;
#else
    if (threadIdx.x < 64) {
      const Pair pre = lookback_collect2<XF>(a.status, a.group, prev_tile, a.epoch, threadIdx.x, &a.ds->overflow);
      if (threadIdx.x == 0) {
        s_prefix = pre.a;
        if (XF) s_prefix_x = pre.x;
      }
    }
    lds_barrier();
    stream_out(0u, prev_tile, prev_total, prev_totalx);
    prev_tile = 0xffffffffu;
#endif
  }
  PH_END(g_k9_phase);
  if (threadIdx.x == 0 && keep_count)
    __hip_atomic_fetch_add(&a.ds->n_updated, keep_count, __ATOMIC_RELAXED, __HIP_MEMORY_SCOPE_AGENT);
  if (is_finaliser(s_tile, ntiles)) {
    finalise_tickets(a.ds, a.group_next, a.group_words);
    if (threadIdx.x == 0 && ntiles == 0) {
      a.ds->n_kept_updated = 0;
      if (XF) a.ds->n_ext_update = 0;
    }
  }
}

template <bool XF>
__global__ void __launch_bounds__(SUMA_TILE) k10_generate(UpdArgs a) {
  __shared__ uint32_t s_tile;
  __shared__ uint32_t s_wave_a[TILE_WAVES], s_wave_b[TILE_WAVES], s_wave_x[TILE_WAVES];
  __shared__ uint32_t s_prefix, s_prefix_x;
  __shared__ uint8_t s_flag[SUMA_TILE];
  __shared__ uint32_t s_rank[SUMA_TILE];
  const int32_t W = a.q.W, H = a.q.H;
  const uint32_t P = (uint32_t)W * (uint32_t)H;
  const uint32_t ntiles = (P + SUMA_TILE - 1) / SUMA_TILE;
  const uint32_t base = a.ds->n_kept_updated;
  const uint32_t xbase = XF ? a.ds->cache_used : 0u;
  const uint32_t xfirst = XF ? a.ds->n_ext_update : 0u;
  const float color = pack_rgb(0.0f, 0.0f, 1.0f);
  uint32_t new_count = 0;
#ifdef UPD_ARG_RELOAD
  const UpdArgsK ka = (UpdArgsK)__builtin_amdgcn_kernarg_segment_ptr();
#endif
  for (;;) {
    __syncthreads();
    if (threadIdx.x == 0)
      s_tile = __hip_atomic_fetch_add(&a.ds->ticket, 1u, __ATOMIC_RELAXED, __HIP_MEMORY_SCOPE_AGENT);
    __syncthreads();
    const uint32_t tile = s_tile;
    if (tile >= ntiles) break;
#ifdef UPD_ARG_RELOAD
    const UpdArgs aT = *upd_args_again(ka);
#else
    const UpdArgs& aT = a;
#endif
    const bool patch = (SUMA_TILE % (uint32_t)H) == 0;
    const uint32_t cols = patch ? SUMA_TILE / (uint32_t)H : 1u;
    uint32_t q;
    if (patch) {
      const uint32_t yy = threadIdx.x / cols, xx = threadIdx.x - yy * cols;
      q = xx * (uint32_t)H + yy;
    } else {
      q = threadIdx.x;
    }
    const uint32_t t = tile * SUMA_TILE + q;
    bool gen = false, emit = false, in_tile = false;
    Surfel4 s;
    if (t < P) {
      const int32_t x = (int32_t)(t / (uint32_t)H), y = (int32_t)(t % (uint32_t)H);
      const size_t pix = (size_t)y * W + x;
      const float4 v = aT.V[pix], n = aT.N[pix], rc = aT.radius_conf[pix];
      const unsigned long long key = aT.zbuf[pix];
      aT.index_map[pix] = (key == SUMA_EMPTY_KEY) ? 0u : (uint32_t)(key & 0xffffffffull) + 1u;
      aT.zbuf[pix] = SUMA_EMPTY_KEY;
      bool invalid = (v.w < 1.0f) || (n.w < 1.0f);
      invalid = invalid || (rc.w < 0.5f);
      const bool integrated = aT.integrated[pix] != 0;
      const v3 vv = xyz(v), nn = xyz(n);
      const v3 view_dir = divs3(neg3(vv), len3(vv));
      gen = (!invalid && !integrated && (dot3(nn, view_dir) > 0.01f));
      if (gen) {
        const v3 ng = normalize3(nn);
        const float4 sem = aT.Sem[pix];
        float conf = aT.log_prior;
        if (is_dynamic_label(sem.x * 255.0f)) conf = aT.log_prior - 0.5f;
        s.a = f4(v.x, v.y, v.z, rc.x);
        s.b = f4(ng.x, ng.y, ng.z, conf);
        s.c = f4(__uint_as_float((uint32_t)aT.timestamp), color, 1.0f, (float)aT.timestamp);
        s.d = sem;
        emit = in_active_area(aT, s, &in_tile);
      }
    }
    {
      const unsigned long long gb = __ballot(gen);
      if ((threadIdx.x & 63) == 0) s_wave_b[threadIdx.x >> 6] = __popcll(gb);
    }
    s_flag[q] = (emit ? 1 : 0) | ((XF && emit && in_tile) ? 2 : 0);
    __syncthreads();
    BlockRank br, brx;
    if (XF) {
      block_rank2((s_flag[threadIdx.x] & 1) != 0, (s_flag[threadIdx.x] & 2) != 0, s_wave_a, s_wave_x, &br, &brx);
      s_rank[threadIdx.x] = br.rank | (brx.rank << 16);
    } else {
      br = block_rank(s_flag[threadIdx.x] != 0, s_wave_a);
      brx.rank = brx.total = 0;
      s_rank[threadIdx.x] = br.rank;
    }
    if (threadIdx.x == 0)
      for (int w = 0; w < (int)TILE_WAVES; ++w) new_count += s_wave_b[w];
    if (threadIdx.x < 64) {
      if (threadIdx.x == 0) lookback_publish(aT.status, aT.group, tile, br.total, aT.epoch, brx.total);
      const Pair pre = lookback_collect2<XF>(aT.status, aT.group, tile, aT.epoch, threadIdx.x, &aT.ds->overflow);
      if (threadIdx.x == 0) {
        s_prefix = pre.a;
        if (XF) s_prefix_x = pre.x;
      }
    }
    __syncthreads();
    if (emit) {
      const uint32_t rk = s_rank[q];
      uint64_t dst = (uint64_t)base + s_prefix + (XF ? (rk & 0xffffu) : rk);
      if (dst < aT.max_surfels) {
        store_surfel(aT.out, (uint32_t)dst, s);
        if (XF) {
          if (in_tile) {
            const uint64_t xr = (uint64_t)xfirst + s_prefix_x + (rk >> 16);
            if (xr < SUMA_EXTRACT_CAPACITY && (uint64_t)xbase + xr < aT.x_cap) store_surfel(aT.x_arena, (uint32_t)(xbase + xr), s);
          }
        } else if (aT.ex_flags != nullptr) {
          aT.ex_flags[dst] = in_tile ? 1 : 0;
        }
      }
    }
    if (tile == ntiles - 1 && threadIdx.x == 0) {
      uint64_t kept = (uint64_t)s_prefix + br.total;
      uint64_t total = (uint64_t)base + kept;
      aT.ds->n_kept_data = (uint32_t)kept;
      if (total > aT.max_surfels) {
        total = aT.max_surfels;
        atomicOr(&aT.ds->overflow, 1u);
      }
      aT.ds->n_surfels = (uint32_t)total;
      if (XF) aT.ds->n_extracted = xfirst + s_prefix_x + brx.total;
    }
  }
  if (threadIdx.x == 0 && new_count)
    __hip_atomic_fetch_add(&a.ds->n_data, new_count, __ATOMIC_RELAXED, __HIP_MEMORY_SCOPE_AGENT);
  if (is_finaliser(s_tile, ntiles)) {
    finalise_tickets(a.ds, a.group_next, a.group_words);
    if (XF && threadIdx.x == 0) commit_extraction(a.ds, a.x_slots, a.x_slot, xbase, a.x_cap, a.ds->n_extracted);
  }
}

static void set_m4(m4& d, const float* s) {
  for (int i = 0; i < 16; ++i) d.m[i] = s[i];
}

static uint32_t compact_grid(suma_ctx* c, uint64_t items) {
  uint64_t blocks = (items + SUMA_TILE - 1) / SUMA_TILE;
  if (blocks > SUMA_COMPACT_BLOCKS) blocks = SUMA_COMPACT_BLOCKS;
  if (blocks < 1) blocks = 1;
  return (uint32_t)blocks;
}
static uint32_t stream_grid(suma_ctx* c, uint64_t items) {
  uint64_t blocks = (items + 255) / 256;
  if (blocks > SUMA_STREAM_BLOCKS) blocks = SUMA_STREAM_BLOCKS;
  if (blocks < 256) blocks = 256;
  return (uint32_t)blocks;
}

K8Out launch_k8_out(suma_ctx* c) {
  K8Out o;
  o.radius_conf = c->radius_conf;
  o.integrated = c->integrated;
  o.pixrec = c->pixrec;
  o.pixel_size = c->mc.pixel_size;
  o.angle_thresh = c->mc.radconf_angle_thresh;
  o.min_radius = c->p.min_radius;
  o.max_radius = c->p.max_radius;
  return o;
}

hipError_t launch_map_update(suma_ctx* c, const float* pose, const float* inv_pose, const suma_frame* f, float cx,
                             float cy, float extent, int k7_done, const float* ex, int fused_slot) {
  const uint32_t P = (uint32_t)c->P;
  const double S = (double)c->known_surfels;
  UpdArgs a;
  memset(&a, 0, sizeof(a));
  a.in = c->surfels[c->cur];
  a.out = c->surfels[c->cur ^ 1];
  a.ds = c->ds;
  a.poses = c->poses;
  a.poses_inv = c->poses_inv;
  a.poses_w = c->poses;
  a.poses_inv_w = c->poses_inv;
  a.zbuf = c->zbuf_data;
  a.status = c->tile_status;
  a.group_words = c->group_words;
  a.V = f->map[SUMA_MAP_VERTEX];
  a.N = f->map[SUMA_MAP_NORMAL];
  a.Sem = f->map[SUMA_MAP_SEMANTIC];
  a.radius_conf = c->radius_conf;
  a.pixrec = c->pixrec;
  a.integrated = c->integrated;
  a.index_map = c->index_map;
  a.q = c->pd;
  set_m4(a.pose, pose);
  set_m4(a.inv_pose, inv_pose);
  a.timestamp = (int32_t)c->timestamp;
  a.max_surfels = c->p.max_surfels;
  a.confidence_threshold = c->p.confidence_threshold;
  a.map_max_distance = c->p.map_max_distance;
  a.update_angle_thresh = c->mc.update_angle_thresh;
  a.p_stable = c->p.p_stable;
  a.p_unstable = c->mc.p_unstable;
  a.log_prior = c->mc.log_prior;
  a.log_unstable = c->mc.log_unstable;
  a.sigma_angle = c->p.sigma_angle;
  a.sigma_distance = c->p.sigma_distance;
  a.max_weight = c->p.max_weight;
  a.use_stability = c->p.use_stability;
  a.unstable_age = c->p.unstable_age;
  a.confidence_mode = c->p.confidence_mode;
  a.active_timestamps = c->p.active_timestamps;
  a.weighting_scheme = c->p.weighting_scheme;
  a.averaging_scheme = c->p.averaging_scheme;
  a.update_always = c->p.update_always;
  a.cx = cx;
  a.cy = cy;
  a.extent = extent;
  a.ex_flags = (ex && fused_slot < 0) ? c->extract_flags : nullptr;
  const bool xf = ex && fused_slot >= 0;
  a.x_arena = xf ? c->cache_arena : nullptr;
  a.x_slots = c->cache_slots;
  a.x_cap = c->cache_cap;
  a.x_slot = xf ? (uint32_t)fused_slot : 0u;
  a.ex_cx = ex ? ex[0] : 0.0f;
  a.ex_cy = ex ? ex[1] : 0.0f;
  a.ex_extent = ex ? ex[2] : 0.0f;
  hipStream_t st = c->ls;
  const uint32_t gridS = stream_grid(c, (uint64_t)c->known_surfels + 2 * c->P);
  a.pose_idx = c->timestamp;
  a.write_pose = 0;
  if (c->k8_fused_frame == f && c->k8_fused_stamp == c->timestamp && c->k8_fused_params == c->params_version) {
    a.write_pose = 1;
  } else {
    ProfScope ps(c, "k8_radius", 48.0 * P);
    k8_radius<<<(P + 255) / 256, 256, 0, st>>>(a.V, a.N, launch_k8_out(c), P, c->ds, c->poses, c->poses_inv, c->timestamp,
                                                a.pose, a.Sem);
  }
  c->k8_fused_frame = nullptr;
  if (!k7_done) {
    ProfScope ps(c, "k7_indexmap", 64.0 * S + 8.0 * P);
    k7_indexmap<<<gridS, 256, 0, st>>>(a);
  }
  {
    ProfScope ps(c, "k9_update_surfels", 128.0 * S + 16.0 * P);
    a.epoch = ++c->epoch;
    a.group = c->tile_group + (size_t)(a.epoch & 1u) * c->group_words;
    a.group_next = c->tile_group + (size_t)((a.epoch + 1u) & 1u) * c->group_words;
    const uint32_t grid = compact_grid(c, (uint64_t)c->known_surfels + 2 * c->P);
    if (xf)
      k9_update<true><<<grid, K9_THREADS, 0, st>>>(a);
    else
      k9_update<false><<<grid, K9_THREADS, 0, st>>>(a);
  }
  {
    ProfScope ps(c, "k10_generate_surfels", (80.0 + 12.0) * P + 64.0 * P * 0.5);
    a.epoch = ++c->epoch;
    a.group = c->tile_group + (size_t)(a.epoch & 1u) * c->group_words;
    a.group_next = c->tile_group + (size_t)((a.epoch + 1u) & 1u) * c->group_words;
    if (xf)
      k10_generate<true><<<compact_grid(c, P), SUMA_TILE, 0, st>>>(a);
    else
      k10_generate<false><<<compact_grid(c, P), SUMA_TILE, 0, st>>>(a);
  }
  return hipGetLastError();
}

__global__ void k_set_poses(float* poses, float* poses_inv, const float* src, uint32_t first, uint32_t n) {
  uint32_t k = blockIdx.x * blockDim.x + threadIdx.x;
  if (k >= n) return;
  float m[16], inv[16];
  for (int i = 0; i < 16; ++i) m[i] = src[16 * (size_t)k + i];
  rigid_inverse_dev(m, inv);
  for (int i = 0; i < 16; ++i) {
    poses[16 * (size_t)(first + k) + i] = m[i];
    poses_inv[16 * (size_t)(first + k) + i] = inv[i];
  }
}
__global__ void k_identity_poses(float* poses, float* poses_inv, uint32_t n) {
  uint32_t k = blockIdx.x * blockDim.x + threadIdx.x;
  if (k >= n) return;
  for (int i = 0; i < 16; ++i) {
    float v = (i % 5 == 0) ? 1.0f : 0.0f;
    poses[16 * (size_t)k + i] = v;
    poses_inv[16 * (size_t)k + i] = v;
  }
}

__global__ void k_clear_keys(unsigned long long* z, uint32_t n) {
  uint32_t i = blockIdx.x * blockDim.x + threadIdx.x;
  if (i < n) z[i] = SUMA_EMPTY_KEY;
}
hipError_t launch_clear_index_zbuf(suma_ctx* c) {
  uint32_t P = (uint32_t)c->P;
  k_clear_keys<<<(P + 255) / 256, 256, 0, c->ls>>>(c->zbuf_data, P);
  return hipGetLastError();
}

hipError_t launch_set_poses(suma_ctx* c, const float* d_src, uint32_t first, uint32_t n) {
  if (n == 0) return hipSuccess;
  k_set_poses<<<(n + 255) / 256, 256, 0, c->ls>>>(c->poses, c->poses_inv, d_src, first, n);
  return hipGetLastError();
}
hipError_t launch_fill_identity_poses(suma_ctx* c) {
  uint32_t n = c->p.max_poses;
  k_identity_poses<<<(n + 255) / 256, 256, 0, c->ls>>>(c->poses, c->poses_inv, n);
  return hipGetLastError();
}

struct ExtractArgs {
  const suma_surfel* in;
  suma_surfel* arena;
  DevState* ds;
  CacheSlot* slots;
  const float* poses;
  unsigned long long* status;
  unsigned long long *group, *group_next;
  uint32_t group_words;
  uint32_t epoch, slot, arena_cap;
  float cx, cy, extent;
  const uint8_t* flags;
};

#define K12_ITEMS 4u
template <bool FLAGS>
__global__ void __launch_bounds__(SUMA_TILE) k12_extract(ExtractArgs a) {
  __shared__ uint32_t s_tile, s_prefix;
  __shared__ uint32_t s_cnt[K12_ITEMS][TILE_WAVES];
  const uint32_t S = a.ds->n_surfels;
  const uint32_t span = SUMA_TILE * K12_ITEMS;
  const uint32_t ntiles = (S + span - 1) / span;
  const float4* __restrict__ sf = reinterpret_cast<const float4*>(a.in);
  const uint32_t base = a.ds->cache_used;
  const int lane = threadIdx.x & 63, wave = threadIdx.x >> 6;
  for (;;) {
    __syncthreads();
    if (threadIdx.x == 0)
      s_tile = __hip_atomic_fetch_add(&a.ds->ticket, 1u, __ATOMIC_RELAXED, __HIP_MEMORY_SCOPE_AGENT);
    __syncthreads();
    const uint32_t tile = s_tile;
    if (tile >= ntiles) break;
    float4 pa[K12_ITEMS];
    float cnt[K12_ITEMS];
    uint32_t fl[K12_ITEMS];
#pragma unroll
    for (uint32_t k = 0; k < K12_ITEMS; ++k) {
      const uint32_t i = tile * span + k * SUMA_TILE + threadIdx.x;
      pa[k] = f4(0.f, 0.f, 0.f, 0.f);
      cnt[k] = 0.f;
      fl[k] = 0;
      if (i < S) {
        if (FLAGS) {
          fl[k] = a.flags[i];
        } else {
          pa[k] = sf[4 * (size_t)i];
          cnt[k] = sf[4 * (size_t)i + 2].w;
        }
      }
    }
    bool sel[K12_ITEMS];
    uint32_t below[K12_ITEMS];
#pragma unroll
    for (uint32_t k = 0; k < K12_ITEMS; ++k) {
      const uint32_t i = tile * span + k * SUMA_TILE + threadIdx.x;
      sel[k] = false;
      if (FLAGS) {
        sel[k] = fl[k] != 0;
      } else if (i < S) {
        float Ps[16];
        load_pose(a.poses, (int32_t)cnt[k], Ps);
        v3 pos = m4_point(Ps, xyz(pa[k]));
        sel[k] = !(sdm_abs(pos.x - a.cx) > a.extent || sdm_abs(pos.y - a.cy) > a.extent);
      }
      const unsigned long long b = __ballot(sel[k]);
      below[k] = __popcll(b & ((1ull << lane) - 1ull));
      if (lane == 0) s_cnt[k][wave] = __popcll(b);
    }
    __syncthreads();
    uint32_t total = 0, rank[K12_ITEMS];
#pragma unroll
    for (uint32_t k = 0; k < K12_ITEMS; ++k) {
      uint32_t off = total;
#pragma unroll
      for (int w = 0; w < (int)TILE_WAVES; ++w) {
        const uint32_t c = s_cnt[k][w];
        if (w < wave) off += c;
        total += c;
      }
      rank[k] = off + below[k];
    }
    if (threadIdx.x < 64) {
      uint32_t pre = lookback_prefix(a.status, a.group, tile, total, a.epoch, threadIdx.x, &a.ds->overflow);
      if (threadIdx.x == 0) s_prefix = pre;
    }
    __syncthreads();
#pragma unroll
    for (uint32_t k = 0; k < K12_ITEMS; ++k) {
      if (sel[k]) {
        const uint32_t i = tile * span + k * SUMA_TILE + threadIdx.x;
        const uint32_t dst = s_prefix + rank[k];
        if (dst < SUMA_EXTRACT_CAPACITY && (uint64_t)base + dst < a.arena_cap) {
          Surfel4 s;
          s.a = FLAGS ? sf[4 * (size_t)i] : pa[k];
          s.b = sf[4 * (size_t)i + 1];
          s.c = sf[4 * (size_t)i + 2];
          s.d = sf[4 * (size_t)i + 3];
          store_surfel(a.arena, base + dst, s);
        }
      }
    }
    if (tile == ntiles - 1 && threadIdx.x == 0) a.ds->n_extracted = s_prefix + total;
  }
  if (is_finaliser(s_tile, ntiles)) {
    finalise_tickets(a.ds, a.group_next, a.group_words);
    if (threadIdx.x == 0) commit_extraction(a.ds, a.slots, a.slot, base, a.arena_cap, (ntiles == 0) ? 0u : a.ds->n_extracted);
  }
}

hipError_t launch_extract(suma_ctx* c, uint32_t slot, float cx, float cy, float extent, int use_flags) {
  ExtractArgs a;
  a.flags = use_flags ? c->extract_flags : nullptr;
  a.in = c->surfels[c->cur];
  a.arena = c->cache_arena;
  a.ds = c->ds;
  a.slots = c->cache_slots;
  a.poses = c->poses;
  a.status = c->tile_status;
  a.epoch = ++c->epoch;
  a.group_words = c->group_words;
  a.group = c->tile_group + (size_t)(a.epoch & 1u) * c->group_words;
  a.group_next = c->tile_group + (size_t)((a.epoch + 1u) & 1u) * c->group_words;
  a.slot = slot;
  a.arena_cap = c->cache_cap;
  a.cx = cx;
  a.cy = cy;
  a.extent = extent;
  ProfScope ps(c, "k12_extract_submap", (use_flags ? 1.0 : 64.0) * (double)c->known_surfels);
  const uint32_t grid = compact_grid(c, ((uint64_t)c->known_surfels + 2 * c->P + K12_ITEMS - 1) / K12_ITEMS);
  if (use_flags)
    k12_extract<true><<<grid, SUMA_TILE, 0, c->ls>>>(a);
  else
    k12_extract<false><<<grid, SUMA_TILE, 0, c->ls>>>(a);
  return hipGetLastError();
}

__global__ void __launch_bounds__(256)
    k_append_cached(suma_surfel* surfels, const suma_surfel* arena, DevState* ds, const CacheSlot* slots,
                    uint32_t slot, uint32_t max_surfels, const float* poses, uint8_t* ex_flags, float ex_cx, float ex_cy,
                    float ex_extent) {
  const CacheSlot cs = slots[slot];
  const uint32_t S = ds->n_surfels;
  const float4* __restrict__ src = reinterpret_cast<const float4*>(arena + cs.offset);
  float4* __restrict__ dst = reinterpret_cast<float4*>(surfels);
  uint32_t n = cs.count;
  if ((uint64_t)S + n > max_surfels) n = max_surfels - S;
  for (uint64_t k = (uint64_t)blockIdx.x * blockDim.x + threadIdx.x; k < 4ull * n; k += (uint64_t)gridDim.x * blockDim.x)
    dst[4ull * S + k] = src[k];
  if (ex_flags != nullptr)
    for (uint64_t k = (uint64_t)blockIdx.x * blockDim.x + threadIdx.x; k < n; k += (uint64_t)gridDim.x * blockDim.x) {
      const float4 pa = src[4 * k];
      float Ps[16];
      load_pose(poses, (int32_t)src[4 * k + 2].w, Ps);
      const v3 pos = m4_point(Ps, xyz(pa));
      ex_flags[S + k] = !(sdm_abs(pos.x - ex_cx) > ex_extent || sdm_abs(pos.y - ex_cy) > ex_extent) ? 1 : 0;
    }
}
__global__ void k_append_commit(DevState* ds, const CacheSlot* slots, uint32_t slot, uint32_t max_surfels) {
  uint32_t S = ds->n_surfels, n = slots[slot].count;
  if ((uint64_t)S + n > max_surfels) {
    n = max_surfels - S;
    atomicOr(&ds->overflow, 1u);
  }
  ds->n_surfels = S + n;
}

hipError_t launch_append_cached(suma_ctx* c, uint32_t slot) {
  float ex[3] = {0.f, 0.f, 0.f};
  if (c->flagged.valid) {
    ex[0] = (float)(2.0 * c->flagged.i * c->p.submap_extent);
    ex[1] = (float)(2.0 * c->flagged.j * c->p.submap_extent);
    ex[2] = c->p.submap_extent;
  }
  k_append_cached<<<1024, 256, 0, c->ls>>>(c->surfels[c->cur], c->cache_arena, c->ds, c->cache_slots, slot,
                                               c->p.max_surfels, c->poses, c->flagged.valid ? c->extract_flags : nullptr,
                                               ex[0], ex[1], ex[2]);
  k_append_commit<<<1, 1, 0, c->ls>>>(c->ds, c->cache_slots, slot, c->p.max_surfels);
  return hipGetLastError();
}
```

### semantic_suma_amd/csrc/suma_api.hip

```cpp
#include <cmath>
#include <cstdio>
#include <cstring>
#include <mutex>
#include <new>
#include <set>

#include <time.h>

#include "suma_internal.h"

static std::mutex g_ctx_mu;
static std::set<const suma_ctx*> g_live_ctx;
static bool ctx_alive(const suma_ctx* c) {
  std::lock_guard<std::mutex> lk(g_ctx_mu);
  return g_live_ctx.count(c) != 0;
}

static thread_local std::string g_create_error;

extern "C" const char* suma_version(void) { return "suma-hip 0.1 (gfx950)"; }
extern "C" const char* suma_last_error(const suma_ctx* ctx) { return ctx ? ctx->err.c_str() : g_create_error.c_str(); }
int fail_without_ctx(int code, const std::string& msg) {
  g_create_error = msg;
  return code;
// ... 40 lines not shown
  float hpix = (float)tan(0.5 * ((double)hfov * M_PI / 180.0) / (double)p.data_width);
  c->mc.pixel_size = vpix < hpix ? hpix : vpix;
  c->mc.p_unstable = 1.0f - p.p_stable;
  c->mc.log_prior = (float)log((double)p.p_prior / (1.0 - (double)p.p_prior));
  c->mc.log_unstable = (float)log((double)c->mc.p_unstable / (1.0 - (double)c->mc.p_unstable));
  c->mc.radconf_angle_thresh = (float)cos((double)deg2rad_f(p.max_angle));
  c->mc.update_angle_thresh = sinf(((float)M_PI / 180.f) * p.map_max_angle);
}

#define CK(expr)                                                                 \
  do {                                                                           \
    hipError_t e__ = (expr);                                                     \
    if (e__ != hipSuccess) {                                                     \
      c->err = std::string(#expr) + ": " + hipGetErrorString(e__);               \
      return SUMA_ERR_HIP;                                                       \
    }                                                                            \
  } while (0)

static inline void accessed(suma_ctx* c, const suma_frame* f) {
  if (f) const_cast<suma_frame*>(f)->last_access = ++c->enq_seq;
}
static inline void host_synced(suma_ctx* c) { c->done_seq = c->enq_seq; }

int fail(suma_ctx* c, int code, const std::string& msg) {
  c->err = msg;
  return code;
}

int prof_begin(suma_ctx* c, const char* name, double bytes, uint32_t launches) {
  int id = -1;
  for (size_t i = 0; i < c->prof_names.size(); ++i)
    if (c->prof_names[i] == name) id = (int)i;
  if (id < 0) {
    id = (int)c->prof_names.size();
    c->prof_names.push_back(name);
    c->prof_ms.push_back(0.0);
    c->prof_bytes.push_back(0.0);
    c->prof_launches.push_back(0);
  }
  ProfEvent ev;
  ev.id = id;
  ev.bytes = bytes;
  ev.launches = launches;
  for (hipEvent_t* e : {&ev.a, &ev.b}) {
    if (!c->prof_pool.empty()) {
      *e = c->prof_pool.back();
      c->prof_pool.pop_back();
    } else if (hipEventCreate(e) != hipSuccess) {
      return -1;
    }
  }
  ev.stream = c->ls;
  hipEventRecord(ev.a, ev.stream);
  c->prof_events.push_back(ev);
  return (int)c->prof_events.size() - 1;
}
void prof_end(suma_ctx* c, int token) { hipEventRecord(c->prof_events[token].b, c->prof_events[token].stream); }

static void prof_collect(suma_ctx* c) {
  if (c->prof_events.empty()) return;
  hipStreamSynchronize(c->stream);
  if (c->side_stream) hipStreamSynchronize(c->side_stream);
  for (auto& ev : c->prof_events) {
    float ms = 0.f;
    if (hipEventElapsedTime(&ms, ev.a, ev.b) == hipSuccess) {
      c->prof_ms[ev.id] += ms;
      c->prof_bytes[ev.id] += ev.bytes;
      c->prof_launches[ev.id] += ev.launches;
    }
    c->prof_pool.push_back(ev.a);
    c->prof_pool.push_back(ev.b);
  }
  c->prof_events.clear();
}

extern "C" int suma_profile_enable(suma_ctx* c, int on) {
  if (!c) return SUMA_ERR_INVALID;
  prof_collect(c);
  c->profiling = on < 0 ? 0 : (on > 3 ? 1 : on);
  if (c->prof_filter.empty()) c->prof_filter = "k6_icp_step";
  return SUMA_OK;
}
extern "C" int suma_profile_reset(suma_ctx* c) {
  if (!c) return SUMA_ERR_INVALID;
  prof_collect(c);
  for (size_t i = 0; i < c->prof_ms.size(); ++i) {
    c->prof_ms[i] = 0.0;
    c->prof_bytes[i] = 0.0;
    c->prof_launches[i] = 0;
  }
  return SUMA_OK;
}
extern "C" int suma_profile_get(suma_ctx* c, suma_kernel_time* out, uint32_t cap) {
  if (!c) return SUMA_ERR_INVALID;
  prof_collect(c);
  uint32_t n = (uint32_t)c->prof_names.size();
  for (uint32_t i = 0; i < n && i < cap; ++i) {
    memset(&out[i], 0, sizeof(out[i]));
    snprintf(out[i].name, sizeof(out[i].name), "%s", c->prof_names[i].c_str());
    out[i].launches = c->prof_launches[i];
    out[i].total_ms = c->prof_ms[i];
    out[i].bytes = c->prof_bytes[i];
  }
  return (int)n;
}

static int frame_create_raw(suma_ctx* c, uint32_t w, uint32_t h, suma_frame** out) {
  suma_frame* f = new (std::nothrow) suma_frame();
  if (!f) return fail(c, SUMA_ERR_NOMEM, "out of host memory");
  f->ctx = c;
  f->width = w;
  f->height = h;
  size_t P = (size_t)w * h;
  hipError_t e = f->block.alloc(3 * P);
  if (e != hipSuccess) {
    delete f;
    c->err = std::string("hipMalloc(frame): ") + hipGetErrorString(e);
    return SUMA_ERR_HIP;
  }
  hipMemsetAsync(f->block, 0, 3 * P * sizeof(float4), c->stream);
  for (int m = 0; m < 3; ++m) f->map[m] = f->block + m * P;
  accessed(c, f);
  *out = f;
  return SUMA_OK;
}

static int read_state(suma_ctx* c) {
  CK(hipMemcpyAsync(c->h_ds, c->ds, sizeof(DevState), hipMemcpyDeviceToHost, c->stream));
  CK(hipStreamSynchronize(c->stream));
  c->known_surfels = c->h_ds->n_surfels;
  return SUMA_OK;
}

static int map_reset_impl(suma_ctx* c) {
  c->cache_bound = 0;
  if (c->k7.valid) CK(launch_clear_index_zbuf(c));
  CK(hipMemsetAsync(c->ds, 0, sizeof(DevState), c->stream));
  if (c->cache_slots) CK(hipMemsetAsync(c->cache_slots, 0, (size_t)c->cache_slots_cap * sizeof(CacheSlot), c->stream));
  c->cache_compactions = 0;
  c->cache_nothing_stale = false;
  c->flagged.valid = false;
  c->k7_spec.on = true;
  c->k7_spec.have_last = false;
  CK(launch_fill_identity_poses(c));
  c->timestamp = 0;
  c->cur = 0;
  c->origin_i = c->origin_j = 0;
  c->cache_index.clear();
  c->extraction.clear();
  c->known_surfels = 0;
  c->map_version++;
  c->rendered.valid = false;
  c->k7.valid = false;
  c->k8_fused_frame = nullptr;
  return SUMA_OK;
}

static const char* filter_params_error(const suma_params* p) {
  if (p->filter_sampling != SUMA_FILTER_SAMPLING_GL_INITIAL && p->filter_sampling != SUMA_FILTER_SAMPLING_NEAREST)
    return "filter_sampling: unknown value";
  if (p->filter_vertexmap && !(p->bilateral_sigma_space > 0.0f && p->bilateral_sigma_range > 0.0f))
    return "filter_vertexmap needs bilateral_sigma_space and bilateral_sigma_range > 0 (config/default.xml holds no "
           "bilateral_sigma_space; Preprocessing.cpp:86 would throw on the missing key)";
  if (p->model_width > SUMA_MAX_MODEL_WIDTH)
    return "model_width above 5461 columns is outside the range of the rasteriser's fixed-point window coordinates "
           "(k_render.hip: |X| < 2^21 in 1/256 pixel)";
  if ((p->filter_vertexmap || p->avg_vertexmap) && (p->data_width > 8192 || p->data_height > 8192))
    return "avg_vertexmap / filter_vertexmap: images above 8192 texels per side are not covered (k_filters.hip)";
  return nullptr;
}

extern "C" int suma_ctx_create(const suma_params* params, int hip_device, suma_ctx** out) {
  if (!params || !out) {
    g_create_error = "suma_ctx_create: null argument";
    return SUMA_ERR_INVALID;
  }
  *out = nullptr;
  int ndev = 0;
  hipError_t e = hipGetDeviceCount(&ndev);
  if (e != hipSuccess || ndev <= 0) {
    g_create_error = std::string("no HIP device available (") + hipGetErrorString(e) +
                     "); this library has no CPU fallback";
    return SUMA_ERR_HIP;
  }
  if (hip_device < 0 || hip_device >= ndev) {
    g_create_error = "suma_ctx_create: device index out of range";
    return SUMA_ERR_INVALID;
  }
  if (params->data_width == 0 || params->data_height == 0 || params->model_width == 0 || params->model_height == 0 ||
      params->max_surfels == 0 || params->max_poses == 0) {
    g_create_error = "suma_ctx_create: zero image size or capacity";
    return SUMA_ERR_INVALID;
  }
  if (const char* fe = filter_params_error(params)) {
    g_create_error = std::string("suma_ctx_create: ") + fe;
    return SUMA_ERR_INVALID;
  }
  suma_ctx* c = new (std::nothrow) suma_ctx();
  if (!c) {
    g_create_error = "out of host memory";
    return SUMA_ERR_NOMEM;
  }
  c->p = *params;
  c->device = hip_device;
  derive(c);
  c->P = (size_t)params->data_width * params->data_height;
  c->Pm = (size_t)params->model_width * params->model_height;
  int rc = SUMA_OK;
  auto body = [&]() -> int {
    CK(hipSetDevice(hip_device));
    CK(hipStreamCreateWithFlags(&c->stream, hipStreamNonBlocking));
    c->ls = c->stream;
    CK(c->sync_flags.alloc(16));
    CK(hipMemsetAsync(c->sync_flags, 0, 16 * sizeof(uint32_t), c->stream));
    const size_t P = c->P, Pm = c->Pm;
    CK(c->zbuf_data.alloc(P));
    CK(hipMemsetAsync(c->zbuf_data, 0xFF, P * 8, c->stream));
    CK(c->eroded.alloc(P));
    CK(c->radius_conf.alloc(P));
    CK(hipMemsetAsync(c->radius_conf, 0, P * sizeof(float4), c->stream));
    CK(c->pixrec.alloc(P * 4));
    CK(c->integrated.alloc(P));
    CK(hipMemsetAsync(c->integrated, 0, P, c->stream));
    CK(c->extract_flags.alloc(params->max_surfels));
    CK(c->index_map.alloc(P));
    CK(hipMemsetAsync(c->index_map, 0, P * 4, c->stream));
    CK(c->zbuf_a.alloc(Pm));
    CK(c->zbuf_b.alloc(Pm));
    CK(hipMemsetAsync(c->zbuf_a, 0xFF, Pm * 8, c->stream));
    CK(hipMemsetAsync(c->zbuf_b, 0xFF, Pm * 8, c->stream));
    for (int b = 0; b < 2; ++b) CK(c->surfels[b].alloc(params->max_surfels));
    CK(c->poses.alloc((size_t)params->max_poses * 16));
    CK(c->poses_inv.alloc((size_t)params->max_poses * 16));
    c->n_tiles_cap = (uint32_t)(((size_t)params->max_surfels + 2 * P) / SUMA_TILE + 2);
    CK(c->tile_status.alloc(c->n_tiles_cap));
    CK(hipMemsetAsync(c->tile_status, 0, (size_t)c->n_tiles_cap * 8, c->stream));
    c->group_words = c->n_tiles_cap / 64 + 2;
    CK(c->tile_group.alloc((size_t)2 * c->group_words));
    CK(hipMemsetAsync(c->tile_group, 0, (size_t)2 * c->group_words * 8, c->stream));
    CK(c->ds.alloc(1));
    CK(c->h_ds.alloc(1));
    memset(c->h_ds, 0, sizeof(DevState));
    c->icp_blocks = 256;
    CK(c->gn.alloc(2 * SUMA_MAX_HYP));
    CK(hipMemsetAsync(c->gn, 0, 2 * SUMA_MAX_HYP * sizeof(GnState), c->stream));
    CK(c->gn_partial.alloc((size_t)2 * SUMA_MAX_HYP * c->icp_blocks * SUMA_ACC_WORDS));
    CK(hipMemset(c->gn_partial, 0, (size_t)2 * SUMA_MAX_HYP * c->icp_blocks * SUMA_ACC_WORDS * sizeof(int64_t)));
    c->gn_history_cap = 1025;
    CK(c->gn_history.alloc((size_t)c->gn_history_cap * 16));
    CK(c->gn_T0s.alloc((size_t)SUMA_MAX_HYP * 16));
    CK(c->h_gn.alloc(SUMA_MAX_HYP));
    CK(c->pose_block.alloc(32));
    CK(c->h_rec.alloc(2));
    memset(c->h_rec, 0, 2 * sizeof(HostResult));
    uint64_t cache = params->cache_surfels ? params->cache_surfels : 16ull * params->max_surfels;
    if (cache > 0xffffffffull) cache = 0xffffffffull;
    c->cache_cap = (uint32_t)cache;
    CK(c->cache_arena.alloc(c->cache_cap));
    c->cache_slots_cap = 65536;
    CK(c->cache_slots.alloc(c->cache_slots_cap));
    int r = frame_create_raw(c, params->model_width, params->model_height, &c->old_frame);
    if (r) return r;
    r = frame_create_raw(c, params->model_width, params->model_height, &c->new_frame);
    if (r) return r;
    r = frame_create_raw(c, params->model_width, params->model_height, &c->composed_frame);
    if (r) return r;
    r = map_reset_impl(c);
    if (r) return r;
    CK(hipStreamSynchronize(c->stream));
    return SUMA_OK;
  };
  rc = body();
  if (rc != SUMA_OK) {
    g_create_error = c->err;
    suma_ctx_destroy(c);
    return rc;
  }
  {
    std::lock_guard<std::mutex> lk(g_ctx_mu);
    g_live_ctx.insert(c);
  }
  *out = c;
  return SUMA_OK;
}

extern "C" void suma_ctx_destroy(suma_ctx* c) {
  if (!c) return;
  {
    std::lock_guard<std::mutex> lk(g_ctx_mu);
    g_live_ctx.erase(c);
  }
  hipSetDevice(c->device);
  ingest_destroy(c);
  if (c->stream) hipStreamSynchronize(c->stream);
  if (c->side_stream) {
    hipStreamSynchronize(c->side_stream);
    side_stream_released(c);
    hipStreamDestroy(c->side_stream);
    if (c->pre_event) hipEventDestroy(c->pre_event);
    if (c->order_event) hipEventDestroy(c->order_event);
  }
  for (auto& ev : c->prof_events) {
    hipEventDestroy(ev.a);
    hipEventDestroy(ev.b);
  }
  for (auto& e : c->prof_pool) hipEventDestroy(e);
  suma_frame_destroy(c->old_frame);
  suma_frame_destroy(c->new_frame);
  suma_frame_destroy(c->composed_frame);
  if (c->stream) hipStreamDestroy(c->stream);
  delete c;
}

extern "C" int suma_set_params(suma_ctx* c, const suma_params* p) {
  if (!c || !p) return SUMA_ERR_INVALID;
  if (p->data_width != c->p.data_width || p->data_height != c->p.data_height || p->model_width != c->p.model_width ||
      p->model_height != c->p.model_height || p->max_surfels != c->p.max_surfels || p->max_poses != c->p.max_poses)
    return fail(c, SUMA_ERR_INVALID, "suma_set_params: image sizes and capacities are fixed at creation");
  if (const char* fe = filter_params_error(p)) {
    c->err = std::string("suma_set_params: ") + fe;
    return SUMA_ERR_INVALID;
  }
  uint32_t cache = c->p.cache_surfels;
  c->p = *p;
  c->p.cache_surfels = cache;
  derive(c);
  c->params_version++;
  c->obj_set = false;
  return SUMA_OK;
}
extern "C" int suma_synchronize(suma_ctx* c) {
  if (!c) return SUMA_ERR_INVALID;
  if (c->side_stream) CK(hipStreamSynchronize(c->side_stream));
  CK(hipStreamSynchronize(c->stream));
  return SUMA_OK;
}
extern "C" void* suma_ctx_stream(suma_ctx* c) { return c ? (void*)c->stream : nullptr; }

extern "C" int suma_frame_create(suma_ctx* c, uint32_t w, uint32_t h, suma_frame** out) {
  if (!c || !out || w == 0 || h == 0) return SUMA_ERR_INVALID;
  return frame_create_raw(c, w, h, out);
}
extern "C" void suma_frame_destroy(suma_frame* f) {
  if (!f) return;
  if (suma_ctx* c = ctx_alive(f->ctx) ? f->ctx : nullptr) {
    if (c->k8_fused_frame == f) c->k8_fused_frame = nullptr;
    if (c->gate_frame == f) c->gate_frame = nullptr;
    if (c->rendered.out == f) c->rendered.valid = false;
  }
  delete f;
}
extern "C" int suma_frame_copy(suma_ctx* c, suma_frame* dst, const suma_frame* src) {
  if (!c || !dst || !src || dst->width != src->width || dst->height != src->height) return SUMA_ERR_INVALID;
  size_t bytes = 3 * (size_t)src->width * src->height * sizeof(float4);
  if (c->gate_pending) CK(flush_gate(c));
  dst->version++;
  accessed(c, dst);
  accessed(c, src);
  CK(hipMemcpyAsync(dst->map[0], src->map[0], bytes, hipMemcpyDeviceToDevice, c->stream));
  return SUMA_OK;
}
extern "C" int suma_frame_download(suma_ctx* c, const suma_frame* f, int which, suma_float4* host) {
  if (!c || !f || !host || which < 0 || which > 2) return SUMA_ERR_INVALID;
  size_t bytes = (size_t)f->width * f->height * sizeof(float4);
  if (c->gate_pending) CK(flush_gate(c));
  CK(hipMemcpyAsync(host, f->map[which], bytes, hipMemcpyDeviceToHost, c->stream));
  CK(hipStreamSynchronize(c->stream));
  host_synced(c);
  return SUMA_OK;
}
extern "C" int suma_frame_touch(suma_ctx* c, suma_frame* f) {
  if (!c || !f) return SUMA_ERR_INVALID;
  f->version++;
  return SUMA_OK;
}
extern "C" int suma_frame_upload(suma_ctx* c, suma_frame* f, int which, const suma_float4* host) {
  if (!c || !f || !host || which < 0 || which > 2) return SUMA_ERR_INVALID;
  size_t bytes = (size_t)f->width * f->height * sizeof(float4);
  if (c->gate_pending) CK(flush_gate(c));
  f->version++;
  CK(hipMemcpyAsync(f->map[which], host, bytes, hipMemcpyHostToDevice, c->stream));
  CK(hipStreamSynchronize(c->stream));
  host_synced(c);
  return SUMA_OK;
// ... 415 lines not shown
  }
  DevBuf<suma_surfel> fresh;
  CK(fresh.alloc(c->cache_cap));
  uint32_t off = 0;
  hipError_t e = hipSuccess;
  for (auto& q : slots) {
    if (q.count && e == hipSuccess)
      e = hipMemcpyAsync(fresh + off, c->cache_arena + q.offset, (size_t)q.count * sizeof(suma_surfel),
                         hipMemcpyDeviceToDevice, c->stream);
    q.offset = off;
    off += q.count;
  }
  if (ns && e == hipSuccess) e = hipMemcpyAsync(c->cache_slots, slots.data(), ns * sizeof(CacheSlot), hipMemcpyHostToDevice, c->stream);
  if (e == hipSuccess) e = hipMemcpyAsync(&c->ds->cache_used, &off, sizeof(uint32_t), hipMemcpyHostToDevice, c->stream);
  if (e == hipSuccess) e = hipStreamSynchronize(c->stream);
  CK(e);
  c->cache_arena = std::move(fresh);
  c->h_ds->cache_used = off;
  c->cache_bound = off;
  c->cache_compactions += 1;
  c->cache_nothing_stale = false;
  return SUMA_OK;
}

static int extract_surfels(suma_ctx* c, bool partially) {
  while (!c->extraction.empty()) {
    auto idx = c->extraction.back();
    c->extraction.pop_back();
    float cx, cy;
    submap_center(c, idx.first, idx.second, &cx, &cy);
    const auto account = [&]() {
      const uint64_t most = (uint64_t)c->known_surfels + 2 * c->P;
      c->cache_bound += most < SUMA_EXTRACT_CAPACITY ? most : SUMA_EXTRACT_CAPACITY;
    };
    if (c->flagged.valid && c->flagged.fused && c->flagged.i == idx.first && c->flagged.j == idx.second) {
      c->flagged.valid = false;
      account();
      if (partially) break;
      continue;
    }
    if (c->flagged.valid && c->flagged.fused)
      return fail(c, SUMA_ERR_INVALID, "internal: the update extracted a tile other than the one updateActiveSubmaps asks for");
    uint32_t slot;
    int r = cache_slot_for(c, idx.first, idx.second, &slot);
    if (r) return r;
    r = cache_compact_if_needed(c, slot);
    if (r) return r;
    const int use_flags = (c->flagged.valid && c->flagged.i == idx.first && c->flagged.j == idx.second) ? 1 : 0;
    c->flagged.valid = false;
    CK(launch_extract(c, slot, cx, cy, c->p.submap_extent, use_flags));
    account();
    if (partially) break;
  }
  return SUMA_OK;
}

static int append_cached(suma_ctx* c, int32_t i, int32_t j) {
  auto it = c->cache_index.find(std::make_pair(i, j));
  if (it == c->cache_index.end()) return SUMA_OK;
  CK(launch_append_cached(c, it->second));
  return SUMA_OK;
}

static bool peek_extraction(const suma_ctx* c, const float* pose, int32_t* ti, int32_t* tj, bool* appends) {
  *appends = false;
  const auto cached = [&](int32_t i, int32_t j) { return c->cache_index.find(std::make_pair(i, j)) != c->cache_index.end(); };
  if (!c->p.partial_extraction || getenv("SUMA_NO_EXTRACT_FLAGS")) return false;
  const int32_t dim = c->p.submap_dimension;
  const float ext = c->p.submap_extent;
  int32_t oi = c->origin_i, oj = c->origin_j;
  float cx, cy;
  submap_center(c, oi, oj, &cx, &cy);
  const float changex = pose[12] - cx, changey = pose[13] - cy, factor = 1.1f;
  bool have = !c->extraction.empty();
  std::pair<int32_t, int32_t> last = have ? c->extraction.back() : std::make_pair(0, 0);
  if (fabsf(changex) > factor * ext) {
    const int32_t dir = (changex < 0) ? -1 : 1;
    last = {oi - dir * dim, oj + dim};
    have = true;
    oi += dir;
    for (int32_t k = -dim; k <= dim; ++k) *appends |= cached(oi + dir * dim, oj + k);
  }
  if (fabsf(changey) > factor * ext) {
    const int32_t dir = (changey < 0) ? -1 : 1;
    last = {oi + dim, oj - dir * dim};
    have = true;
    for (int32_t r0 = -dim; r0 <= dim; ++r0) *appends |= cached(oi + r0, oj + dir + dir * dim);
  }
  if (!have) return false;
  *ti = last.first;
  *tj = last.second;
  return true;
}

static int update_active_submaps(suma_ctx* c, const float* pose) {
  const int32_t dim = c->p.submap_dimension;
  const float ext = c->p.submap_extent;
  float cx, cy;
  submap_center(c, c->origin_i, c->origin_j, &cx, &cy);
  float changex = pose[12] - cx, changey = pose[13] - cy;
  const float factor = 1.1f;
  if (fabsf(changex) > factor * ext || fabsf(changey) > factor * ext) {
    if (fabsf(changex) > factor * ext) {
      int32_t dir = (changex < 0) ? -1 : 1;
      for (int32_t k = -dim; k <= dim; ++k) c->extraction.push_back({c->origin_i - dir * dim, c->origin_j + k});
      c->origin_i += dir;
      for (int32_t k = -dim; k <= dim; ++k) {
        int r = append_cached(c, c->origin_i + dir * dim, c->origin_j + k);
        if (r) return r;
      }
    }
    if (fabsf(changey) > factor * ext) {
      int32_t dir = (changey < 0) ? -1 : 1;
      for (int32_t r0 = -dim; r0 <= dim; ++r0) c->extraction.push_back({c->origin_i + r0, c->origin_j - dir * dim});
      c->origin_j += dir;
      for (int32_t r0 = -dim; r0 <= dim; ++r0) {
        int r = append_cached(c, c->origin_i + r0, c->origin_j + dir * dim);
        if (r) return r;
      }
    }
  }
  if (!c->extraction.empty()) return extract_surfels(c, c->p.partial_extraction != 0);
  return SUMA_OK;
}

extern "C" int suma_map_update(suma_ctx* c, const float pose[16], const suma_frame* frame) {
  if (c && c->gate_pending) CK(flush_gate(c));
  if (!c || !pose || !frame) return SUMA_ERR_INVALID;
  if (frame->width != c->p.data_width || frame->height != c->p.data_height)
    return fail(c, SUMA_ERR_INVALID, "suma_map_update: frame size differs from data_width x data_height");
  if (c->timestamp >= c->p.max_poses)
    return fail(c, SUMA_ERR_CAPACITY, "pose table full (max_poses; reference: maxPoses_ = 10000, SurfelMap.h:205)");
  float inv_pose[16];
  rigid_inverse_f(pose, inv_pose);
  float cx, cy;
  submap_center(c, c->origin_i, c->origin_j, &cx, &cy);
  float extent = 2.0f * (float)c->p.submap_dimension * c->p.submap_extent + c->p.submap_extent;
  if (c->p.partial_extraction && !c->extraction.empty()) extent += 2.0f * c->p.submap_extent;
  int k7_done = 0;
  if (c->k7.valid) {
    k7_done = (c->k7.map_version == c->map_version && c->k7.params_version == c->params_version &&
               memcmp(c->k7.pose, pose, 16 * sizeof(float)) == 0 && frame->width == c->p.data_width);
    if (!k7_done) {
      CK(launch_clear_index_zbuf(c));
      c->k7_spec.on = false;
    }
    c->k7.valid = false;
  }
  if (k7_done || (c->k7_spec.have_last && c->k7_spec.map_version == c->map_version &&
                  c->k7_spec.params_version == c->params_version &&
                  memcmp(c->k7_spec.last_pose, pose, 16 * sizeof(float)) == 0))
    c->k7_spec.on = true;
  c->k7_spec.have_last = false;
  accessed(c, frame);
  if (c->k8_fused_frame == frame && c->k8_fused_version != frame->version) c->k8_fused_frame = nullptr;
  float ex[3];
  int32_t ti = 0, tj = 0;
  bool appends = false;
  const bool flag_tile = peek_extraction(c, pose, &ti, &tj, &appends);
  int fused_slot = -1;
  if (flag_tile) {
    submap_center(c, ti, tj, &ex[0], &ex[1]);
    ex[2] = c->p.submap_extent;
    if (!appends && !getenv("SUMA_NO_FUSED_EXTRACT") && c->cache_index.size() < c->cache_slots_cap) {
      uint32_t slot;
      if (cache_slot_for(c, ti, tj, &slot) == SUMA_OK && cache_compact_if_needed(c, slot) == SUMA_OK) fused_slot = (int)slot;
    }
  }
  c->flagged.valid = flag_tile;
  c->flagged.i = ti;
  c->flagged.j = tj;
  c->flagged.fused = fused_slot >= 0;
  c->flagged.slot = fused_slot >= 0 ? (uint32_t)fused_slot : 0u;
  CK(launch_map_update(c, pose, inv_pose, frame, cx, cy, extent, k7_done, flag_tile ? ex : nullptr, fused_slot));
  c->cur ^= 1;
  c->map_version++;
  int r = update_active_submaps(c, pose);
  if (r) return r;
  c->timestamp += 1;
  return SUMA_OK;
}

static int map_render_dedup(suma_ctx* c, const float* pose_old, const float* pose_new, float conf_threshold,
                            suma_frame* out) {
  auto& r = c->rendered;
  if (r.valid && r.out == out && r.map_version == c->map_version && r.params_version == c->params_version &&
      r.out_version == out->version && r.old_version == c->old_frame->version && r.new_version == c->new_frame->version &&
      memcmp(&r.conf_threshold, &conf_threshold, sizeof(float)) == 0 &&
      memcmp(r.pose_old, pose_old, 16 * sizeof(float)) == 0 && memcmp(r.pose_new, pose_new, 16 * sizeof(float)) == 0)
    return SUMA_OK;
  if (c->gate_pending && c->gate_frame == out) CK(flush_gate(c));
  CK(launch_map_render(c, pose_old, pose_new, conf_threshold, out));
  out->version++;
  if (c->old_frame != out) c->old_frame->version++;
  if (c->new_frame != out) c->new_frame->version++;
  accessed(c, out);
  accessed(c, c->old_frame);
  accessed(c, c->new_frame);
  r.out_version = out->version;
  r.old_version = c->old_frame->version;
  r.new_version = c->new_frame->version;
  r.valid = true;
  r.out = out;
  r.map_version = c->map_version;
  r.params_version = c->params_version;
  r.conf_threshold = conf_threshold;
  memcpy(r.pose_old, pose_old, 16 * sizeof(float));
  memcpy(r.pose_new, pose_new, 16 * sizeof(float));
  return SUMA_OK;
}

extern "C" int suma_map_render(suma_ctx* c, const float pose_old[16], const float pose_new[16], float conf_threshold,
                               suma_frame* out) {
  if (!c || !pose_old || !pose_new || !out) return SUMA_ERR_INVALID;
  if (out->width != c->p.model_width || out->height != c->p.model_height)
    return fail(c, SUMA_ERR_INVALID, "suma_map_render: frame size differs from model_width x model_height");
  return map_render_dedup(c, pose_old, pose_new, conf_threshold, out);
}
extern "C" int suma_map_render_active(suma_ctx* c, const float pose[16], float conf_threshold) {
  if (!c || !pose) return SUMA_ERR_INVALID;
  if (c->gate_pending && c->gate_frame == c->new_frame) CK(flush_gate(c));
  int fuse_k7 = 0;
  if (c->k7.valid) {
    CK(launch_clear_index_zbuf(c));
    c->k7.valid = false;
    c->k7_spec.on = false;
  } else if (c->k7_spec.on && c->p.data_width == c->p.model_width && !getenv("SUMA_NO_K7_SPECULATION")) {
    fuse_k7 = 1;
  }
  CK(launch_map_render_single(c, pose, conf_threshold, 1, fuse_k7, nullptr));
  c->new_frame->version++;
  accessed(c, c->new_frame);
  if (fuse_k7) {
    c->k7.valid = true;
    c->k7.map_version = c->map_version;
    c->k7.params_version = c->params_version;
    memcpy(c->k7.pose, pose, 16 * sizeof(float));
  }
  c->k7_spec.have_last = true;
  c->k7_spec.map_version = c->map_version;
  c->k7_spec.params_version = c->params_version;
  memcpy(c->k7_spec.last_pose, pose, 16 * sizeof(float));
  return SUMA_OK;
}
extern "C" int suma_map_render_inactive(suma_ctx* c, const float pose[16], float conf_threshold) {
  if (!c || !pose) return SUMA_ERR_INVALID;
  if (c->gate_pending && c->gate_frame == c->old_frame) CK(flush_gate(c));
  CK(launch_map_render_single(c, pose, conf_threshold, 0, 0, nullptr));
  c->old_frame->version++;
  accessed(c, c->old_frame);
  return SUMA_OK;
}
extern "C" int suma_map_render_composed(suma_ctx* c, const float pose_old[16], const float pose_new[16],
                                        float conf_threshold) {
  if (!c || !pose_old || !pose_new) return SUMA_ERR_INVALID;
  if (c->gate_pending && c->gate_frame == c->composed_frame) CK(flush_gate(c));
  CK(launch_map_render_composed(c, pose_old, pose_new, conf_threshold));
  c->composed_frame->version++;
  accessed(c, c->composed_frame);
  return SUMA_OK;
}
extern "C" suma_frame* suma_map_frame(suma_ctx* c, int which) {
  if (!c) return nullptr;
  return which == SUMA_FRAME_OLD ? c->old_frame : (which == SUMA_FRAME_NEW ? c->new_frame : c->composed_frame);
}

extern "C" int suma_map_update_poses(suma_ctx* c, const float* poses16, uint32_t n) {
  if (!c || (!poses16 && n)) return SUMA_ERR_INVALID;
  if (n > c->p.max_poses) n = c->p.max_poses;
  if (n == 0) return SUMA_OK;
  hipError_t e;
  {
    DevBuf<float> d_tmp;
    CK(d_tmp.alloc((size_t)n * 16));
    e = hipMemcpyAsync(d_tmp, poses16, (size_t)n * 16 * sizeof(float), hipMemcpyHostToDevice, c->stream);
    if (e == hipSuccess) e = launch_set_poses(c, d_tmp, 0, n);
    if (e == hipSuccess) e = hipStreamSynchronize(c->stream);
  }
  c->map_version++;
  CK(e);
  return SUMA_OK;
}

int check_overflow(suma_ctx* c) {
  if (c->h_ds->overflow & 1u) return fail(c, SUMA_ERR_CAPACITY, "surfel capacity (max_surfels) exceeded; map truncated");
  if (c->h_ds->overflow & 2u) return fail(c, SUMA_ERR_CAPACITY, "submap cache arena (cache_surfels) exhausted");
  if (c->h_ds->overflow & 8u) {
    char msg[160];
    snprintf(msg, sizeof(msg), "stable-compaction / stream hand-off timed out (internal error, site mask 0x%x)", c->h_ds->fault_site);
    return fail(c, SUMA_ERR_HIP, msg);
  }
  return SUMA_OK;
}

extern "C" int suma_map_size(suma_ctx* c, uint32_t* n) {
  if (!c || !n) return SUMA_ERR_INVALID;
  int r = read_state(c);
  if (r) return r;
  *n = c->h_ds->n_surfels;
  return check_overflow(c);
}
extern "C" int suma_map_timestamp(suma_ctx* c, uint32_t* t) {
  if (!c || !t) return SUMA_ERR_INVALID;
  *t = c->timestamp;
  return SUMA_OK;
}
extern "C" int suma_map_download(suma_ctx* c, suma_surfel* host, uint32_t cap, uint32_t* n) {
  if (!c) return SUMA_ERR_INVALID;
  int r = read_state(c);
  if (r) return r;
  uint32_t S = c->h_ds->n_surfels;
  if (n) *n = S;
  uint32_t m = S < cap ? S : cap;
  if (m && host) {
    CK(hipMemcpyAsync(host, c->surfels[c->cur], (size_t)m * sizeof(suma_surfel), hipMemcpyDeviceToHost, c->stream));
    CK(hipStreamSynchronize(c->stream));
  }
  return SUMA_OK;
}
extern "C" int suma_map_export_surfels(suma_ctx* c, void** d_ptr, uint32_t* n) {
  if (!c || !d_ptr || !n) return SUMA_ERR_INVALID;
  int r = read_state(c);
  if (r) return r;
  *d_ptr = (void*)c->surfels[c->cur];
  *n = c->h_ds->n_surfels;
  return check_overflow(c);
}
extern "C" int suma_map_export_data_surfels(suma_ctx* c, void** d_ptr, uint32_t* first, uint32_t* n_data) {
  if (!c || !d_ptr || !first || !n_data) return SUMA_ERR_INVALID;
  int r = read_state(c);
  if (r) return r;
  *d_ptr = (void*)c->surfels[c->cur];
  *first = c->h_ds->n_kept_updated;
  *n_data = c->h_ds->n_kept_data;
  return check_overflow(c);
}
extern "C" int suma_map_upload(suma_ctx* c, const suma_surfel* host, uint32_t n, uint32_t timestamp) {
  if (!c || (!host && n)) return SUMA_ERR_INVALID;
  if (n > c->p.max_surfels) n = c->p.max_surfels;
  if (n) CK(hipMemcpyAsync(c->surfels[c->cur], host, (size_t)n * sizeof(suma_surfel), hipMemcpyHostToDevice, c->stream));
  CK(hipMemcpyAsync(&c->ds->n_surfels, &n, sizeof(uint32_t), hipMemcpyHostToDevice, c->stream));
  CK(hipStreamSynchronize(c->stream));
  c->timestamp = timestamp;
  c->known_surfels = n;
  c->map_version++;
  return SUMA_OK;
}
extern "C" int suma_map_download_index_map(suma_ctx* c, uint32_t* host) {
  if (!c || !host) return SUMA_ERR_INVALID;
  CK(hipMemcpyAsync(host, c->index_map, c->P * 4, hipMemcpyDeviceToHost, c->stream));
  CK(hipStreamSynchronize(c->stream));
  return SUMA_OK;
}
extern "C" int suma_map_download_radius_conf(suma_ctx* c, suma_float4* host) {
  if (!c || !host) return SUMA_ERR_INVALID;
  CK(hipMemcpyAsync(host, c->radius_conf, c->P * sizeof(float4), hipMemcpyDeviceToHost, c->stream));
  CK(hipStreamSynchronize(c->stream));
  return SUMA_OK;
}
extern "C" int suma_map_download_poses(suma_ctx* c, float* host, uint32_t capacity, uint32_t* n) {
  if (!c || !n || (capacity && !host)) return SUMA_ERR_INVALID;
  *n = c->timestamp;
  const uint32_t m = c->timestamp < capacity ? c->timestamp : capacity;
  if (m) {
    CK(hipMemcpyAsync(host, c->poses, (size_t)m * 16 * sizeof(float), hipMemcpyDeviceToHost, c->stream));
    CK(hipStreamSynchronize(c->stream));
    host_synced(c);
  }
  return SUMA_OK;
}
extern "C" int suma_map_download_integrated(suma_ctx* c, uint8_t* host) {
  if (!c || !host) return SUMA_ERR_INVALID;
  CK(hipMemcpyAsync(host, c->integrated, c->P, hipMemcpyDeviceToHost, c->stream));
  CK(hipStreamSynchronize(c->stream));
  return SUMA_OK;
}
extern "C" int suma_map_counts(suma_ctx* c, uint32_t* n_updated, uint32_t* n_new, uint32_t* n_cached,
                               int32_t origin_ij[2]) {
  if (!c) return SUMA_ERR_INVALID;
  int r = read_state(c);
  if (r) return r;
  if (n_updated) *n_updated = c->h_ds->n_updated;
  if (n_new) *n_new = c->h_ds->n_data;
  if (n_cached) {
    uint32_t ns = (uint32_t)c->cache_index.size();
    std::vector<CacheSlot> slots(ns);
    if (ns) {
      CK(hipMemcpyAsync(slots.data(), c->cache_slots, ns * sizeof(CacheSlot), hipMemcpyDeviceToHost, c->stream));
      CK(hipStreamSynchronize(c->stream));
    }
    uint32_t s = 0;
    for (auto& q : slots) s += q.count;
    *n_cached = s;
  }
  if (origin_ij) {
    origin_ij[0] = c->origin_i;
    origin_ij[1] = c->origin_j;
  }
  return SUMA_OK;
}

// ... 215 lines not shown
  for (int k = 0; k < 4; ++k) {
    bool data = k < 2;
    r = frame_create_raw(c, data ? params->data_width : params->model_width,
                         data ? params->data_height : params->model_height, fr[k]);
    if (r) {
      g_create_error = c->err;
      suma_pipeline_destroy(s);
      return r;
    }
  }
  if (s->h_res.alloc(3) != hipSuccess) {
    g_create_error = "hipHostMalloc failed";
    suma_pipeline_destroy(s);
    return SUMA_ERR_HIP;
  }
  memset(s->h_res, 0, 3 * sizeof(HostResult));
  if (ensure_side_stream(c) != SUMA_OK) {
    g_create_error = "side stream setup failed: " + c->err;
    suma_pipeline_destroy(s);
    return SUMA_ERR_HIP;
  }
  mat4_eye(s->current_pose);
  mat4_eye(s->last_pose);
  mat4_eye(s->pose_old);
  mat4_eye(s->pose_new);
  mat4_eye(s->last_increment);
  mat4_eye(s->last_pose_old);
  float p_unstable = 0.1f;
  s->log_unstable = (float)log((double)(p_unstable / (1.0f - p_unstable)));
  *out = s;
  return SUMA_OK;
}
extern "C" void suma_pipeline_destroy(suma_pipeline* s) {
  if (!s) return;
  loop_destroy(s);
  ingest_destroy(s->c);
  if (s->c && s->c->stream) hipStreamSynchronize(s->c->stream);
  suma_frame_destroy(s->last_frame);
  suma_frame_destroy(s->current_frame);
  suma_frame_destroy(s->current_model);
  suma_frame_destroy(s->last_model);
  suma_ctx_destroy(s->c);
  delete s;
}
extern "C" suma_ctx* suma_pipeline_ctx(suma_pipeline* s) { return s ? s->c : nullptr; }
extern "C" int suma_pipeline_pose(const suma_pipeline* s, double pose[16]) {
  if (!s || !pose) return SUMA_ERR_INVALID;
  memcpy(pose, s->current_pose, 16 * sizeof(double));
  return SUMA_OK;
}
extern "C" int suma_pipeline_last_increment(const suma_pipeline* s, double inc[16]) {
  if (!s || !inc) return SUMA_ERR_INVALID;
  memcpy(inc, s->last_increment, 16 * sizeof(double));
  return SUMA_OK;
}
extern "C" int suma_pipeline_last_stats(const suma_pipeline* s, suma_icp_stats* st) {
  if (!s || !st) return SUMA_ERR_INVALID;
  int r = resolve_stats(const_cast<suma_pipeline*>(s), true);
  *st = s->stats;
  return r;
}
extern "C" int suma_pipeline_minimize_stats(const suma_pipeline* s, suma_icp_stats* st) {
  if (!s || !st) return SUMA_ERR_INVALID;
  *st = s->stats_mst;
  return SUMA_OK;
}
extern "C" uint32_t suma_pipeline_timestamp(const suma_pipeline* s) { return s ? s->timestamp : 0; }
extern "C" uint32_t suma_pipeline_track_loss(const suma_pipeline* s) { return s ? s->track_loss : 0; }
extern "C" suma_frame* suma_pipeline_frame(suma_pipeline* s, int which) {
  if (!s) return nullptr;
  return which == 0 ? s->current_frame : (which == 1 ? s->last_model : s->current_model);
}

static int resolve_stats(suma_pipeline* s, bool need_sync) {
  if (!s->stats_pending) return SUMA_OK;
  suma_ctx* c = s->c;
  if (need_sync) CK(hipStreamSynchronize(c->stream));
  int r = wait_host_result(c, &s->h_res[1 + s->stats_slot], s->stats_seq);
  s->stats_pending = false;
  if (r) return fail(c, SUMA_ERR_HIP, "statistics pass did not report (launch failed?)");
  suma_icp_stats st;
  fill_stats_host(s->h_res[1 + s->stats_slot], &st);
  st.iterations = s->stats_mst.iterations;
  st.converged = s->stats_mst.converged;
  s->stats = st;
  return SUMA_OK;
}

static float conf_threshold(const suma_pipeline* s) {
  float ct = s->c->p.confidence_threshold;
  const uint32_t time_init = 10;
  if (s->timestamp < time_init) {
    float alpha = (float)s->timestamp / (float)time_init;
    ct = (float)((1.0 - (double)alpha) * (double)s->log_unstable + (double)(alpha * s->c->p.confidence_threshold));
  }
  return ct;
}

static GnChain pipeline_chain(suma_pipeline* s, const suma_frame* model, const double* T0s, uint32_t n_hyp,
                              int32_t fixed_iterations, bool fallback) {
  suma_ctx* c = s->c;
  c->icp_current = s->current_frame;
  c->icp_model = model;
  GnChain ch = gn_chain_ctx(c, T0s, n_hyp);
  if (fixed_iterations > 0) {
    ch.max_iterations = (uint32_t)fixed_iterations;
    ch.epsilon = 0.0;
    ch.delta = 0.0;
  }
  if (fallback && !c->obj_set) {
    ch.obj.icp_max_distance = c->p.fallback_max_distance;
    ch.obj.icp_max_angle = c->p.fallback_max_angle;
  }
  return ch;
}

static int minimize_cfg(suma_pipeline* s, const GnChain& ch, double* T, suma_icp_stats* st) {
  suma_ctx* c = s->c;
  int r = enqueue_minimize(c, ch);
  if (r) return r;
  CK(hipMemcpyAsync(c->h_gn, gn_result(c), sizeof(GnState), hipMemcpyDeviceToHost, c->stream));
  CK(hipMemcpyAsync(c->h_ds, c->ds, sizeof(DevState), hipMemcpyDeviceToHost, c->stream));
  for (;;) {
    hipError_t q = hipStreamQuery(c->stream);
    if (q == hipSuccess) break;
    if (q != hipErrorNotReady) CK(q);
  }
  int rs = resolve_stats(s, false);
  if (rs) return rs;
  c->known_surfels = c->h_ds->n_surfels;
  memcpy(T, c->h_gn[0].Tk, 16 * sizeof(double));
  fill_stats(c->h_gn[0], st);
  return check_overflow(c);
}

static int update_pose(suma_pipeline* s, int32_t fixed_iterations) {
  suma_ctx* c = s->c;
  double T0[16], increment[16];
  if (!c->p.initialize_identity)
    memcpy(T0, s->last_increment, sizeof(T0));
  else
    mat4_eye(T0);
  suma_icp_stats mst;
  {
    GnChain ch = pipeline_chain(s, c->new_frame, T0, 1, fixed_iterations, false);
    ch.pose_base = s->pose_new;
    s->res_seq += 1;
    ch.report = &s->h_res[0];
    ch.report_seq = s->res_seq;
    int r0 = enqueue_minimize(c, ch);
    if (r0) return r0;
  }
  c->rendered.valid = false;
  CK(launch_map_render_single(c, nullptr, conf_threshold(s), 1, 1, s->last_model));
  c->new_frame->version++;
  s->last_model->version++;
  double I[16];
  mat4_eye(I);
  GnChain st = gn_chain_ctx(c, I, 1);
  CK(launch_gn_init(c, st));
  const uint32_t slot = s->stats_slot ^ 1u;
  {
    ProfScope ps(c, "k6k8_stats_radius", (96.0 + 81.0) * (double)c->P);
    st.report = &s->h_res[1 + slot];
    st.report_seq = s->res_seq;
    st.fuse_k8 = 1;
    CK(launch_icp_iteration(c, st, 1, 1));
    c->k8_fused_frame = s->current_frame;
    c->k8_fused_version = s->current_frame->version;
    c->k8_fused_stamp = c->timestamp;
    c->k8_fused_params = c->params_version;
  }
  struct timespec tw0, tw1;
  clock_gettime(CLOCK_MONOTONIC, &tw0);
  int r = wait_host_result(c, &s->h_res[0], s->res_seq);
  clock_gettime(CLOCK_MONOTONIC, &tw1);
  c->het.result_wait_s += (double)(tw1.tv_sec - tw0.tv_sec) + 1e-9 * (double)(tw1.tv_nsec - tw0.tv_nsec);
  if (r) return r;
  r = resolve_stats(s, false);
  if (r) return r;
  s->stats_slot = slot;
  *c->h_ds = s->h_res[0].ds;
  c->known_surfels = c->h_ds->n_surfels;
  memcpy(increment, s->h_res[0].Tk, sizeof(increment));
  fill_stats_host(s->h_res[0], &mst);
  r = check_overflow(c);
  if (r) return r;
  s->stats_mst = mst;
  s->stats_seq = s->res_seq;
  s->stats_pending = true;

  double inv_last[16], delta[16], posed[16];
  float posef[16];
  mat4_rigid_inv(s->last_increment, inv_last);
  mat4_mul(inv_last, increment, delta);
  mat4_mul(s->pose_new, increment, posed);
  mat4_cast_f(posed, posef);
  c->k7.valid = true;
  c->k7.map_version = c->map_version;
  c->k7.params_version = c->params_version;
  memcpy(c->k7.pose, posef, sizeof(posef));

  float t_err = (float)sqrt((delta[12] * delta[12] + delta[13] * delta[13]) + delta[14] * delta[14]);
  float angle = (float)(0.5 * (((delta[0] + delta[5]) + delta[10]) - 1.0));
  float r_err = (float)acos((double)fmaxf(fminf(angle, 1.0f), -1.0f));
  const bool fallback = (s->timestamp > 1 && ((double)t_err > 0.4 || (double)r_err > 0.1) && c->p.fallback_mode);
  if (fallback) {
    s->track_loss += 1;
    r = minimize_cfg(s, pipeline_chain(s, s->last_frame, T0, 1, fixed_iterations, true), increment, &mst);
    if (r) return r;
  }
  memcpy(s->last_pose, s->current_pose, sizeof(s->last_pose));
  double np[16];
  mat4_mul(s->current_pose, increment, np);
  memcpy(s->current_pose, np, sizeof(np));
  memcpy(s->last_pose_old, s->pose_old, sizeof(s->last_pose_old));
  memcpy(s->pose_old, np, sizeof(np));
  memcpy(s->pose_new, np, sizeof(np));
  memcpy(s->last_increment, increment, sizeof(increment));
  return SUMA_OK;
}

int pipeline_begin_scan_impl(suma_pipeline* s, const suma_float4* d_points, const float* d_labels, const float* d_probs,
                             uint32_t n, hipEvent_t upload_done) {
  if (!s || (n > 0 && !d_points)) return SUMA_ERR_INVALID;
  suma_ctx* c = s->c;
  if (s->phase != 0) return fail(c, SUMA_ERR_INVALID, "suma_pipeline_begin_scan: the previous scan has not been closed with suma_pipeline_update_map");
  c->obj_set = false;
  if (s->loop) {
    int ri = loop_integrate(s);
    if (ri) return ri;
  }
  std::swap(s->last_frame, s->current_frame);
  std::swap(s->last_model, s->current_model);
  int r;
  if (c->side_stream) {
    if (upload_done) HIP_TRY(c, hipStreamWaitEvent(c->side_stream, upload_done, 0));
    c->ls = c->side_stream;
    r = suma_preprocess_device(c, d_points, d_labels, d_probs, n, s->timestamp, s->current_frame);
    c->ls = c->stream;
    if (r) return r;
    r = side_handoff(c, s->current_frame);
    if (r) return r;
  } else {
    if (upload_done) HIP_TRY(c, hipStreamWaitEvent(c->stream, upload_done, 0));
    r = suma_preprocess_device(c, d_points, d_labels, d_probs, n, s->timestamp, s->current_frame);
    if (r) return r;
  }
  float po[16], pn[16];
  mat4_cast_f(s->pose_old, po);
  mat4_cast_f(s->pose_new, pn);
  r = map_render_dedup(c, po, pn, conf_threshold(s), s->last_model);
  if (r) return r;
  s->phase = 1;
  return SUMA_OK;
}

int pipeline_update_pose_impl(suma_pipeline* s, int32_t fixed_iterations) {
  if (!s) return SUMA_ERR_INVALID;
  if (s->phase != 1) return fail(s->c, SUMA_ERR_INVALID, "suma_pipeline_update_pose: call suma_pipeline_begin_scan first");
  if (s->timestamp > 0) {
    int r = update_pose(s, fixed_iterations);
    if (r) return r;
    if (s->loop && (r = loop_odometry_edge(s)) != SUMA_OK) return r;
  }
  s->phase = 2;
  return SUMA_OK;
}

int pipeline_update_map_impl(suma_pipeline* s) {
  if (!s) return SUMA_ERR_INVALID;
  suma_ctx* c = s->c;
  if (s->phase != 2) return fail(c, SUMA_ERR_INVALID, "suma_pipeline_update_map: call suma_pipeline_update_pose first");
  float pc[16];
  mat4_cast_f(s->current_pose, pc);
  int r = suma_map_update(c, pc, s->current_frame);
  if (r) return r;
  r = map_render_dedup(c, pc, pc, conf_threshold(s), s->current_model);
  if (r) return r;
  s->timestamp += 1;
  s->phase = 0;
  return SUMA_OK;
}

hipStream_t pipeline_input_stream(suma_pipeline* s) { return s->c->side_stream ? s->c->side_stream : s->c->stream; }

int pipeline_process_scan_impl(suma_pipeline* s, const suma_float4* d_points, const float* d_labels,
                               const float* d_probs, uint32_t n, int32_t fixed_iterations, hipEvent_t upload_done) {
  return pipeline_finish_scan(s, pipeline_begin_scan_impl(s, d_points, d_labels, d_probs, n, upload_done),
                              fixed_iterations, false);
}
int pipeline_finish_scan(suma_pipeline* s, int r, int32_t fixed_iterations, bool begin_only) {
  if (r == SUMA_OK && !begin_only) r = pipeline_update_pose_impl(s, fixed_iterations);
  if (r == SUMA_OK && !begin_only && s->loop && s->timestamp > 0) r = loop_check(s);
  if (r == SUMA_OK && !begin_only) r = pipeline_update_map_impl(s);
  if (r != SUMA_OK && s) s->phase = 0;
  return r;
}

extern "C" int suma_pipeline_begin_scan_device(suma_pipeline* s, const suma_float4* d_points, const float* d_labels,
                                               const float* d_probs, uint32_t n) {
  return pipeline_begin_scan_impl(s, d_points, d_labels, d_probs, n, nullptr);
}
extern "C" int suma_pipeline_update_pose(suma_pipeline* s, int32_t fixed_iterations) {
  return pipeline_update_pose_impl(s, fixed_iterations);
}
extern "C" int suma_pipeline_update_map(suma_pipeline* s) { return pipeline_update_map_impl(s); }

extern "C" int suma_pipeline_reset(suma_pipeline* s) {
  if (!s) return SUMA_ERR_INVALID;
  suma_ctx* c = s->c;
  int r = suma_synchronize(c);
  if (r) return r;
  if (c->gate_pending) c->gate_pending = 0;
  host_synced(c);
  ingest_drain(c);
  r = map_reset_impl(c);
  if (r) return r;
  r = loop_reset(s);
  if (r) return r;
  s->stats_pending = false;
  memset(&s->stats, 0, sizeof(s->stats));
  s->timestamp = 0;
  s->track_loss = 0;
  s->phase = 0;
  mat4_eye(s->current_pose);
  mat4_eye(s->last_pose);
  mat4_eye(s->pose_old);
  mat4_eye(s->pose_new);
  mat4_eye(s->last_increment);
  mat4_eye(s->last_pose_old);
  c->obj_set = false;
  c->k8_fused_frame = nullptr;
  return suma_synchronize(c);
}

extern "C" int suma_pipeline_minimize_hypotheses(suma_pipeline* s, const double* T0s, uint32_t n_hyp,
                                                 int32_t fixed_iterations, double* T_out, suma_icp_stats* stats) {
  if (!s || !T0s || !T_out || n_hyp == 0 || n_hyp > SUMA_MAX_HYP) return SUMA_ERR_INVALID;
  suma_ctx* c = s->c;
  if (s->phase != 1) return fail(c, SUMA_ERR_INVALID, "suma_pipeline_minimize_hypotheses: between suma_pipeline_begin_scan and suma_pipeline_apply_increment");
  const GnChain ch = pipeline_chain(s, c->new_frame, T0s, n_hyp, fixed_iterations, false);
  hipError_t e = hipMemcpyAsync(c->h_ds, c->ds, sizeof(DevState), hipMemcpyDeviceToHost, c->stream);
  if (e != hipSuccess) {
    c->err = std::string("hipMemcpyAsync(DevState): ") + hipGetErrorString(e);
    return SUMA_ERR_HIP;
  }
  int r = minimize_batch(c, ch, T_out, stats);
  if (r) return r;
  c->known_surfels = c->h_ds->n_surfels;
  return check_overflow(c);
}
extern "C" int suma_pipeline_apply_increment(suma_pipeline* s, const double increment[16]) {
  if (!s || !increment) return SUMA_ERR_INVALID;
  if (s->phase != 1) return fail(s->c, SUMA_ERR_INVALID, "suma_pipeline_apply_increment: call suma_pipeline_begin_scan first");
  memcpy(s->last_pose, s->current_pose, sizeof(s->last_pose));
  double np[16];
  mat4_mul(s->current_pose, increment, np);
  memcpy(s->current_pose, np, sizeof(np));
  memcpy(s->last_pose_old, s->pose_old, sizeof(s->last_pose_old));
  memcpy(s->pose_old, np, sizeof(np));
  memcpy(s->pose_new, np, sizeof(np));
  memcpy(s->last_increment, increment, 16 * sizeof(double));
  if (s->loop) {
    int r = loop_odometry_edge(s);
    if (r) return r;
  }
  s->phase = 2;
  return SUMA_OK;
}

extern "C" int suma_pipeline_integrate_loop_closures(suma_pipeline* s, const float* poses16, uint32_t n,
                                                     const double difference[16]) {
  if (!s || !difference || (!poses16 && n)) return SUMA_ERR_INVALID;
  suma_ctx* c = s->c;
  if (s->phase != 0) return fail(c, SUMA_ERR_INVALID, "suma_pipeline_integrate_loop_closures: only between scans (SurfelMapping.cpp:179)");
  int r = suma_map_update_poses(c, poses16, n);
  if (r) return r;
  double np[16];
  mat4_mul(difference, s->current_pose, np);
  memcpy(s->current_pose, np, sizeof(np));
  memcpy(s->pose_old, np, sizeof(np));
  memcpy(s->pose_new, np, sizeof(np));
  return SUMA_OK;
}
extern "C" int suma_pipeline_set_pose_old(suma_pipeline* s, const double pose_old[16]) {
  if (!s || !pose_old) return SUMA_ERR_INVALID;
  memcpy(s->pose_old, pose_old, sizeof(s->pose_old));
  return SUMA_OK;
}
extern "C" int suma_pipeline_get_pose(const suma_pipeline* s, int which, double pose[16]) {
  if (!s || !pose || which < 0 || which > 4) return SUMA_ERR_INVALID;
  const double* src[5] = {s->current_pose, s->pose_old, s->pose_new, s->last_pose_old, s->last_pose};
  memcpy(pose, src[which], 16 * sizeof(double));
  return SUMA_OK;
}
extern "C" int suma_pipeline_result_new(suma_pipeline* s, suma_icp_stats* st) { return suma_pipeline_last_stats(s, st); }

extern "C" int suma_pipeline_verify_loop_closure(suma_pipeline* s, const double pose_prior[16],
                                                 const double* initializations, uint32_t n_init, float min_valid_ratio,
                                                 float max_outlier_ratio, suma_loop_result* out) {
  if (!s) return SUMA_ERR_INVALID;
  if (s->phase != 2) return fail(s->c, SUMA_ERR_INVALID, "suma_pipeline_verify_loop_closure: between suma_pipeline_update_pose and suma_pipeline_update_map (SurfelMapping.cpp:196)");
  float pn[16];
  mat4_cast_f(s->pose_new, pn);
  return suma_loop_closure_verify(s->c, s->current_frame, pose_prior, initializations, n_init, pn, conf_threshold(s),
                                  min_valid_ratio, max_outlier_ratio, out);
}
extern "C" int suma_pipeline_track_loop_closure(suma_pipeline* s, double min_valid_ratio, double max_outlier_ratio,
                                                double max_increment_difference, suma_loop_track* out) {
  if (!s) return SUMA_ERR_INVALID;
  if (s->phase != 2) return fail(s->c, SUMA_ERR_INVALID, "suma_pipeline_track_loop_closure: between suma_pipeline_update_pose and suma_pipeline_update_map (SurfelMapping.cpp:196)");
  float pn[16];
  mat4_cast_f(s->pose_new, pn);
  return suma_loop_closure_track(s->c, s->current_frame, s->last_pose_old, s->last_increment, pn, conf_threshold(s),
                                 min_valid_ratio, max_outlier_ratio, max_increment_difference, out);
}

extern "C" int suma_pipeline_process_scan_device(suma_pipeline* s, const suma_float4* d_points, const float* d_labels,
                                                 const float* d_probs, uint32_t n, int32_t fixed_iterations) {
  return pipeline_process_scan_impl(s, d_points, d_labels, d_probs, n, fixed_iterations, nullptr);
}

extern "C" int suma_pipeline_process_scan(suma_pipeline* s, const suma_float4* points, const float* labels,
                                          const float* probs, uint32_t n, int32_t fixed_iterations) {
  if (!s || (n > 0 && !points)) return SUMA_ERR_INVALID;
  suma_ctx* c = s->c;
  (void)c;
  return pipeline_process_host_scan(s, points, labels, probs, n, fixed_iterations);
}
```

### semantic_suma_amd/csrc/suma_internal.h

```cpp
#ifndef SUMA_INTERNAL_H_
#define SUMA_INTERNAL_H_

#include <hip/hip_runtime.h>
#include <math.h>
#include <stdint.h>

#include <initializer_list>
#include <map>
#include <string>
#include <utility>
#include <vector>

#include "../../include/suma_hip.h"
#include "dev_math.h"

#ifndef SUMA_TILE
#define SUMA_TILE 1024u
#endif
#ifndef SUMA_COMPACT_BLOCKS
#define SUMA_COMPACT_BLOCKS 256u
#endif
#define SUMA_STREAM_BLOCKS 2048u
#define SUMA_EXTRACT_CAPACITY 500000u
#define SUMA_MAX_MODEL_WIDTH 5461u
#define SUMA_MAX_HYP 64u

template <class T, bool Pinned = false>
struct DevBuf {
  T* p = nullptr;
  size_t cap = 0;
  DevBuf() = default;
  DevBuf(DevBuf&& o) noexcept : p(o.p), cap(o.cap) { o.p = nullptr, o.cap = 0; }
  DevBuf& operator=(DevBuf&& o) noexcept {
    if (this != &o) {
      reset();
      p = o.p, cap = o.cap;
      o.p = nullptr, o.cap = 0;
    }
    return *this;
  }
  ~DevBuf() { reset(); }
  operator T*() const { return p; }
  T* operator->() const { return p; }
  void reset() {
    if (p) (void)(Pinned ? hipHostFree(p) : hipFree(p));
    p = nullptr, cap = 0;
  }
  hipError_t alloc(size_t n) {
    reset();
    void* q = nullptr;
    const hipError_t e = Pinned ? hipHostMalloc(&q, n * sizeof(T), hipHostMallocDefault) : hipMalloc(&q, n * sizeof(T));
    if (e == hipSuccess) p = (T*)q, cap = n;
    return e;
  }
};
template <class T>
using PinnedBuf = DevBuf<T, true>;

struct DevState {
  uint32_t n_surfels;
  uint32_t n_updated;
  uint32_t n_kept_updated;
  uint32_t n_data;
  uint32_t n_kept_data;
  uint32_t n_extracted;
  uint32_t overflow;
  uint32_t ticket;
  uint32_t reserved0;
  uint32_t cache_used;
  uint32_t fault_site;
  uint32_t n_ext_update;
  uint32_t pad[4];
};

struct WorldSpan {
  const suma_surfel* base;
  uint32_t start, count;
};

struct CacheSlot {
  uint32_t offset, count;
};

struct GnState {
  double Tk[16];
  double last_error;
  double F, F_inlier;
  uint32_t iteration;
  uint32_t k;
  uint32_t done, converged;
  uint32_t valid, outlier, invalid, n_hist;
  uint32_t pending;
  uint32_t pad[3];
  int64_t acc[SUMA_ACC_WORDS];
  double JtJ[36];
  double Jtr[6];
};

struct HostResult {
  double Tk[16];
  double F, F_inlier;
  uint32_t valid, outlier, invalid, k, converged, iteration;
  DevState ds;
  uint32_t seq;
  uint32_t n_hist;
  int64_t acc[SUMA_ACC_WORDS];
  double JtJ[36], Jtr[6];
};

struct GnChain {
  const suma_frame *current, *model;
  suma_icp_objective obj;
  uint32_t max_iterations;
  double epsilon, delta;
  const double* T0s;
  uint32_t n_hyp;
  uint32_t iteration0, iteration0_rest;
  int with_history;
  HostResult* report;
  uint32_t report_seq;
  int report_full;
  const double* pose_base;
  int fuse_k8;
};

struct MapConsts {
  float pixel_size, log_prior, log_unstable, p_unstable;
  float radconf_angle_thresh, update_angle_thresh;
};

struct suma_frame {
  suma_ctx* ctx;
  uint32_t width, height;
  DevBuf<float4> block;
  float4* map[3];
  uint64_t version;
  uint64_t last_access;
};

struct ProfEvent {
  hipEvent_t a, b;
  hipStream_t stream;
  int id;
  double bytes;
  uint32_t launches;
};

struct HostEntryTimes {
  double slot_wait_s;
  double copy_s;
  double enqueue_s;
  double launch_s;
  double result_wait_s;
  double call_s;
  uint64_t calls;
  uint32_t copy_threads;
};

struct suma_ctx {
  suma_params p;
  int device;
  hipStream_t stream;
  hipStream_t ls;
  hipStream_t side_stream;
  int side_stream_off;
  DevBuf<uint32_t> sync_flags;
  uint32_t pre_seq;
  uint32_t gate_pending;
  int gate_by_event;
  hipEvent_t pre_event;
  hipEvent_t order_event;
  uint64_t enq_seq, done_seq;
  bool cache_nothing_stale;
  const suma_frame* gate_frame;
  struct Ingest* ingest;
  PinnedBuf<HostResult> h_rec;
  uint32_t rec_seq;
  std::string err;

  proj_t pd, pm;
  MapConsts mc;
  size_t P, Pm;

  DevBuf<unsigned long long> zbuf_data;
  DevBuf<unsigned long long> zbuf_k1;
  DevBuf<float4> eroded;
  DevBuf<float4> filt_temp;
  DevBuf<unsigned long long> filt_sort;
  DevBuf<char> filt_sort_tmp;
  DevBuf<float4> scan_points;
  DevBuf<float> scan_labels, scan_probs;
  DevBuf<unsigned long long> sem_zbuf;
  DevBuf<float> sem_labels, sem_probs;
  DevBuf<char> sem_knn[2];
  DevBuf<unsigned long long> draw_zbuf;
  DevBuf<uint32_t> draw_queue;
  DevBuf<struct WorldSpan> world_spans;
  DevBuf<char> world_scratch, world_tmp;
  DevBuf<uint32_t> world_counters;
  PinnedBuf<uint32_t> world_counters_h;
  DevBuf<char> ckpt_image;
  DevBuf<struct WorldSpan> ckpt_spans;
  DevBuf<unsigned long long> ckpt_digests;

  const suma_frame *icp_current, *icp_model;
  suma_icp_objective obj;
  bool obj_set;
  DevBuf<GnState> gn;
  DevBuf<int64_t> gn_partial;
  uint32_t gn_part_launch;
  uint32_t gn_part_dirty[3];
  uint32_t gn_launch;
  const suma_frame* k8_fused_frame;
  uint64_t k8_fused_version;
  uint32_t k8_fused_stamp;
  uint64_t k8_fused_params;
  DevBuf<float> pose_block;
  HostEntryTimes het;
  uint32_t icp_iteration0;
  DevBuf<double> gn_history;
  DevBuf<double> gn_T0s;
  uint32_t gn_history_cap;
  uint32_t last_n_hist;
  uint64_t hist_seq;
  uint32_t icp_blocks;
  PinnedBuf<GnState> h_gn;

  DevBuf<suma_surfel> surfels[2];
  int cur;
  DevBuf<float> poses;
  DevBuf<float> poses_inv;
  suma_frame *old_frame, *new_frame, *composed_frame;
  DevBuf<unsigned long long> zbuf_a, zbuf_b;
  DevBuf<float4> radius_conf;
  DevBuf<float4> pixrec;
  DevBuf<uint8_t> integrated;
  DevBuf<uint8_t> extract_flags;
  struct {
    bool valid;
    int32_t i, j;
    bool fused;
    uint32_t slot;
  } flagged;
  DevBuf<uint32_t> index_map;
  DevBuf<unsigned long long> tile_status;
  DevBuf<unsigned long long> tile_group;
  uint32_t group_words;
  uint32_t n_tiles_cap;
  uint32_t epoch;
  DevBuf<DevState> ds;
  PinnedBuf<DevState> h_ds;
  uint32_t timestamp;
  int32_t origin_i, origin_j;
  DevBuf<suma_surfel> cache_arena;
  uint32_t cache_cap;
  DevBuf<CacheSlot> cache_slots;
  uint32_t cache_compactions;
  uint64_t cache_bound;
  uint32_t cache_slots_cap;
  std::map<std::pair<int32_t, int32_t>, uint32_t> cache_index;
  std::vector<std::pair<int32_t, int32_t>> extraction;

  int profiling;
  uint32_t prof_tick;
  std::string prof_filter;
  std::vector<ProfEvent> prof_events;
  std::vector<hipEvent_t> prof_pool;
  std::vector<std::string> prof_names;
  std::vector<double> prof_ms, prof_bytes;
  std::vector<uint64_t> prof_launches;
  uint32_t known_surfels;

  uint64_t map_version, params_version;
  struct {
    bool valid;
    float pose[16];
    uint64_t map_version, params_version;
  } k7;
  struct {
    bool on;
    bool have_last;
    float last_pose[16];
    uint64_t map_version, params_version;
  } k7_spec;
  struct {
    bool valid;
    float pose_old[16], pose_new[16], conf_threshold;
    uint64_t map_version, params_version;
    const suma_frame* out;
    uint64_t out_version, old_version, new_version;
  } rendered;
};

struct suma_pipeline {
  suma_ctx* c;
  suma_frame *last_frame, *current_frame, *current_model, *last_model;
  double current_pose[16], last_pose[16], pose_old[16], pose_new[16], last_increment[16];
  double last_pose_old[16];
  uint32_t timestamp;
  int phase;
  float log_unstable;
  suma_icp_stats stats;
  uint32_t track_loss;
  PinnedBuf<HostResult> h_res;
  uint32_t res_seq, stats_seq;
  bool stats_pending;
  uint32_t stats_slot;
  suma_icp_stats stats_mst;
  struct LoopState* loop;
};

int pipeline_process_scan_impl(suma_pipeline* s, const suma_float4* d_points, const float* d_labels, const float* d_probs,
                               uint32_t n, int32_t fixed_iterations, hipEvent_t upload_done);
int pipeline_begin_scan_impl(suma_pipeline* s, const suma_float4* d_points, const float* d_labels, const float* d_probs,
                             uint32_t n, hipEvent_t upload_done);
int pipeline_update_pose_impl(suma_pipeline* s, int32_t fixed_iterations);
int pipeline_update_map_impl(suma_pipeline* s);
int pipeline_finish_scan(suma_pipeline* s, int r, int32_t fixed_iterations, bool begin_only);
hipStream_t pipeline_input_stream(suma_pipeline* s);
int fail(suma_ctx* c, int code, const std::string& msg);
int fail_without_ctx(int code, const std::string& msg);
int check_overflow(suma_ctx* c);
int semantic_check(suma_ctx* c, const suma_semantic_params* sp);
int semantic_scan_input(suma_pipeline* s, uint32_t n, void* producer_event, hipStream_t* st);
void ingest_destroy(suma_ctx* c);
void ingest_drain(suma_ctx* c);
uint32_t ingest_pending(suma_ctx* c);
int ingest_stage_blocking(suma_ctx* c, const suma_float4* points, const float* labels, const float* probs, uint32_t n,
                          const suma_float4** d_points, const float** d_labels, const float** d_probs, hipEvent_t* uploaded,
                          void** slot);
void ingest_consumed(suma_ctx* c, void* slot, hipStream_t reader);
int ensure_side_stream(suma_ctx* c);
int side_handoff(suma_ctx* c, const suma_frame* frame);
void side_stream_released(suma_ctx* c);
int pipeline_process_host_scan(suma_pipeline* s, const suma_float4* points, const float* labels, const float* probs,
                               uint32_t n, int32_t fixed_iterations);

#define HIP_TRY(ctx, expr)                                                                       \
  do {                                                                                           \
    hipError_t e__ = (expr);                                                                     \
    if (e__ != hipSuccess) {                                                                     \
      (ctx)->err = std::string(#expr) + ": " + hipGetErrorString(e__);                           \
      return SUMA_ERR_HIP;                                                                       \
    }                                                                                            \
  } while (0)

template <class T, bool Pinned>
int grow(suma_ctx* c, DevBuf<T, Pinned>& b, size_t n, std::initializer_list<hipStream_t> drain, size_t alloc = 0) {
  if (n <= b.cap) return 0;
  if (b)
    for (hipStream_t st : drain)
      if (st) HIP_TRY(c, hipStreamSynchronize(st));
  HIP_TRY(c, b.alloc(alloc ? alloc : n));
  return 1;
}

int prof_begin(suma_ctx* c, const char* name, double bytes, uint32_t launches);
void prof_end(suma_ctx* c, int token);
struct ProfScope {
  suma_ctx* c;
  int tok;
  ProfScope(suma_ctx* c_, const char* name, double bytes, uint32_t launches = 1)
      : c(c_), tok(wanted(c_, name) ? prof_begin(c_, name, bytes, launches) : -1) {}
  static bool wanted(suma_ctx* c, const char* name) {
    if (c->profiling == 1) return true;
    if (c->profiling < 2 || c->prof_filter != name) return false;
    return c->profiling == 2 || (c->prof_tick++ & 3u) == 0;
  }
  ~ProfScope() {
    if (tok >= 0) prof_end(c, tok);
  }
};

hipError_t launch_preprocess(suma_ctx* c, const float4* d_pts, const float* d_labels, const float* d_probs, uint32_t n,
                             uint32_t timestamp, suma_frame* out);
hipError_t launch_k1_average(suma_ctx* c, const float4* d_pts, const float* d_labels, const float* d_probs, uint32_t n,
                             uint32_t timestamp, float4* vertex, float4* raw_semantic);
hipError_t launch_k1c_bilateral(suma_ctx* c, float4* vertex);
hipError_t launch_gn_init(suma_ctx* c, const GnChain& ch);
hipError_t launch_icp_iteration(suma_ctx* c, const GnChain& ch, int eval_only, int pixel);
const GnState* gn_result(suma_ctx* c);
hipError_t launch_map_render(suma_ctx* c, const float* pose_old, const float* pose_new, float conf_threshold,
                             suma_frame* out);
hipError_t launch_map_render_single(suma_ctx* c, const float* pose, float conf_threshold, int active, int fuse_k7,
                                    suma_frame* mirror);
hipError_t launch_map_render_composed(suma_ctx* c, const float* pose_old, const float* pose_new,
                                      float conf_threshold);
hipError_t launch_map_update(suma_ctx* c, const float* pose, const float* inv_pose, const suma_frame* f, float cx,
                             float cy, float extent, int k7_done, const float* ex, int fused_slot);
hipError_t launch_clear_index_zbuf(suma_ctx* c);
K8Out launch_k8_out(suma_ctx* c);
hipError_t launch_set_poses(suma_ctx* c, const float* d_src, uint32_t first, uint32_t n);
hipError_t launch_fill_identity_poses(suma_ctx* c);
hipError_t launch_extract(suma_ctx* c, uint32_t slot, float cx, float cy, float extent, int use_flags);
hipError_t launch_append_cached(suma_ctx* c, uint32_t slot);

hipError_t launch_signal(suma_ctx* c, hipStream_t st, uint32_t word, uint32_t seq);
hipError_t launch_gate(suma_ctx* c, hipStream_t st, uint32_t word, uint32_t seq);
hipError_t flush_gate(suma_ctx* c);

hipError_t launch_kc_pack(suma_ctx* c, const WorldSpan* d_spans, uint32_t n_spans, uint32_t n_quads, void* d_dst,
                          unsigned long long* d_digest);
hipError_t launch_kc_verify(suma_ctx* c, const void* d_src, uint64_t bytes, unsigned long long* d_digest);
hipError_t launch_kc_unpack(suma_ctx* c, const void* d_tiles, uint32_t n_parked, const void* d_tile_dir, uint32_t n_tiles,
                            uint32_t n_active, const uint32_t counters[4]);

const double* posegraph_host_poses(const suma_posegraph* g, uint32_t* n);
const double* posegraph_device_poses(const suma_posegraph* g, uint32_t* n);
const double* posegraph_host_initial(const suma_posegraph* g, uint32_t* n);
int posegraph_install_nodes(suma_posegraph* g, const double* initial12, const double* result12, uint32_t n, bool to_device);
hipError_t launch_loop_integrate(suma_ctx* c, const double* d_opt12, uint32_t n_opt, const double* d_tail16,
                                 uint32_t n_tail, const double difference[16]);
struct LoopState;
int loop_integrate(suma_pipeline* s);
int loop_odometry_edge(suma_pipeline* s);
int loop_check(suma_pipeline* s);
void loop_destroy(suma_pipeline* s);
int loop_reset(suma_pipeline* s);
void loop_ckpt_join(suma_pipeline* s);
uint64_t loop_ckpt_sizes(const suma_pipeline* s, uint64_t* graph_bytes, uint64_t* opt_bytes);
int loop_ckpt_write(suma_pipeline* s, std::vector<char>* loop, std::vector<char>* graph, std::vector<char>* opt);
int loop_ckpt_check(suma_ctx* c, const char* loop, const char* graph, const char* opt, uint32_t timestamp,
                    suma_loop_params* params);
int loop_ckpt_install(suma_pipeline* s, const char* loop, const char* graph, const char* opt);

struct LocTile {
  unsigned long long key;
  uint32_t start, count;
};
struct LocSpan {
  uint32_t src, dst, count, pad;
};
struct LocMap {
  DevBuf<float4> sorted;
  std::vector<LocTile> dir;
  uint32_t n_kept = 0, n_dropped = 0;
  DevBuf<LocSpan> spans;
};
int localize_bin(suma_ctx* c, const suma_world_surfel* d_records, uint32_t n, LocMap* m);
void localize_window_spans(const LocMap& m, int32_t oi, int32_t oj, int32_t dim, std::vector<LocSpan>* spans,
                           uint64_t* total);
int localize_gather(suma_ctx* c, LocMap* m, const std::vector<LocSpan>& spans, uint32_t total);
bool localize_cell(float extent, float x, float y, float z, int32_t* i, int32_t* j);

int icp_minimize_frames(suma_ctx* c, const suma_frame* current, const suma_frame* model, const double T0[16],
                        int32_t fixed_iterations, double T_out[16], suma_icp_stats* stats);

void rigid_inverse_f(const float* m, float* out);

static inline void mat4_eye(double* T) {
  for (int i = 0; i < 16; ++i) T[i] = (i % 5 == 0) ? 1.0 : 0.0;
}
static inline void mat4_mul(const double* A, const double* B, double* C) {
  for (int c = 0; c < 4; ++c)
    for (int r = 0; r < 4; ++r)
      C[4 * c + r] = ((A[r] * B[4 * c] + A[4 + r] * B[4 * c + 1]) + A[8 + r] * B[4 * c + 2]) + A[12 + r] * B[4 * c + 3];
}
static inline void mat4_rigid_inv(const double* m, double* out) {
  for (int c = 0; c < 3; ++c)
    for (int r = 0; r < 3; ++r) out[4 * c + r] = m[4 * r + c];
  for (int r = 0; r < 3; ++r) out[12 + r] = -((m[4 * r] * m[12] + m[4 * r + 1] * m[13]) + m[4 * r + 2] * m[14]);
  out[3] = out[7] = out[11] = 0.0;
  out[15] = 1.0;
}
static inline void mat4_orthonormalize(double* T) {
  double a[3] = {T[0], T[1], T[2]}, b[3] = {T[4], T[5], T[6]};
  double n = sqrt((a[0] * a[0] + a[1] * a[1]) + a[2] * a[2]);
  for (int r = 0; r < 3; ++r) a[r] = a[r] / n;
  const double d = (a[0] * b[0] + a[1] * b[1]) + a[2] * b[2];
  for (int r = 0; r < 3; ++r) b[r] = b[r] - d * a[r];
  n = sqrt((b[0] * b[0] + b[1] * b[1]) + b[2] * b[2]);
  for (int r = 0; r < 3; ++r) b[r] = b[r] / n;
  const double c[3] = {a[1] * b[2] - a[2] * b[1], a[2] * b[0] - a[0] * b[2], a[0] * b[1] - a[1] * b[0]};
  for (int r = 0; r < 3; ++r) T[r] = a[r], T[4 + r] = b[r], T[8 + r] = c[r];
  T[3] = T[7] = T[11] = 0.0;
  T[15] = 1.0;
}
static inline void mat4_cast_f(const double* T, float* out) {
  for (int i = 0; i < 16; ++i) out[i] = (float)T[i];
}

#endif
```

Baseline: 2864 scans/s.

## Cache projected surfel quads from single render and reuse in merged render

When the identity-pose render of the last model runs, each surfel's projected quad (corners, bounds, test count) is written to a per-surfel cache. A later merged old/new render at the same pose and map version reads these cached quads instead of recomputing the trig-heavy corner projection. Surfels appended since then are flagged as having no source and fall back to full computation. This adds per-surfel cache writes (64 bytes each) to the first render and version and pose gating on the host, in exchange for skipping the per-candidate asin/atan2 work in the second render.

```diff
diff --git a/semantic_suma_amd/core.py b/semantic_suma_amd/core.py
--- a/semantic_suma_amd/core.py
+++ b/semantic_suma_amd/core.py
@@ -182,6 +182,7 @@
     L.suma_pipeline_update_map.argtypes = [vp]
     L.suma_pipeline_integrate_loop_closures.argtypes = [vp, vp, u32, vp]
     L.suma_pipeline_set_pose_old.argtypes = [vp, vp]
+    L.suma_debug_quad_reuse.argtypes = [vp, vp]
     L.suma_pipeline_get_pose.argtypes = [vp, C.c_int, vp]
     L.suma_pipeline_result_new.argtypes = [vp, C.POINTER(IcpStats)]
     L.suma_pipeline_verify_loop_closure.argtypes = [vp, vp, vp, u32, f32, f32, C.POINTER(LoopResult)]
@@ -286,6 +287,11 @@
     def synchronize(self):
         self.check(self.L.suma_synchronize(self.h), "suma_synchronize")
 
+    def quad_reuse(self) -> dict:
+        out = (C.c_uint64 * 4)()
+        self.check(self.L.suma_debug_quad_reuse(self.h, out), "suma_debug_quad_reuse")
+        return dict(passes_reused=int(out[0]), passes_full=int(out[1]), cached=int(out[2]), computed=int(out[3]))
+
     @property
     def stream(self) -> int:
         return int(self.L.suma_ctx_stream(self.h) or 0)
diff --git a/semantic_suma_amd/csrc/k_render.hip b/semantic_suma_amd/csrc/k_render.hip
--- a/semantic_suma_amd/csrc/k_render.hip
+++ b/semantic_suma_amd/csrc/k_render.hip
@@ -29,6 +29,9 @@
   int k7_same_proj;
   proj_t k7_q;
   unsigned long long* k7_zbuf;
+  float4* qc_rec;
+  const uint32_t* qc_src;
+  unsigned long long* qc_stats;
 };
 
 struct rvtx {
@@ -142,8 +145,106 @@
   return off + __popcll(ball & ((1ull << lane) - 1ull));
 }
 
-template <bool BIG>
+__device__ __forceinline__ void render_block_rank2(bool fa, bool fb, uint32_t* s_w, uint32_t* ra, uint32_t* rb,
+                                                   uint32_t* ta, uint32_t* tb) {
+  const int lane = threadIdx.x & 63, wave = threadIdx.x >> 6;
+  const unsigned long long ba = __ballot(fa), bb = __ballot(fb);
+  if (lane == 0) s_w[wave] = (uint32_t)__popcll(ba) | ((uint32_t)__popcll(bb) << 16);
+  K4_BARRIER();
+  uint32_t off = 0, tot = 0;
+#pragma unroll
+  for (int w = 0; w < RENDER_WAVES; ++w) {
+    uint32_t c = s_w[w];
+    if (w < wave) off += c;
+    tot += c;
+  }
+  const unsigned long long below = (1ull << lane) - 1ull;
+  *ta = tot & 0xffffu;
+  *tb = tot >> 16;
+  *ra = (off & 0xffffu) + __popcll(ba & below);
+  *rb = (off >> 16) + __popcll(bb & below);
+}
+
+__device__ __forceinline__ void qc_store_no_quad(float4* qc_rec, uint32_t id) {
+  __builtin_nontemporal_store(0u, reinterpret_cast<uint32_t*>(qc_rec + 4 * (size_t)id) + 15);
+}
+
+template <bool CACHE>
+__device__ __forceinline__ uint32_t render_quad(const proj_t& pq, const v3 cp, const v3 cn, const float crad,
+                                                const float cppx, int32_t* q, float4* qc_rec, const float* idw) {
+  uint32_t ntests = 0;
+  v3 u = normalize3(mk3(cn.y - cn.z, -cn.x, cn.x));
+  v3 v = normalize3(cross3(cn, u));
+  v3 ru = scale3(crad, u), rv = scale3(crad, v);
+  v3 corner[4];
+  corner[0] = sub3(sub3(cp, ru), rv);
+  corner[1] = sub3(add3(cp, ru), rv);
+  corner[2] = add3(sub3(cp, ru), rv);
+  corner[3] = add3(add3(cp, ru), rv);
+  int32_t X[4], Y[4];
+  float Z[4];
+  bool bad = false;
+#pragma unroll
+  for (int k = 0; k < 4; ++k) {
+    const float depth = len3(corner[k]);
+    const float pitch = -sdm_asin(corner[k].z / depth);
+    const float y01 = 1.0f - ((pitch * SUMA_RAD2DEG_F) + pq.fov_up) / pq.fov;
+    Z[k] = 0.5f * (2.0f * ((depth - pq.min_depth) / (pq.max_depth - pq.min_depth)) - 1.0f) + 0.5f;
+    const float yw = y01 * pq.height;
+    if (sdm_isnan(yw) || sdm_isnan(Z[k])) bad = true;
+    Y[k] = (int32_t)sdm_floor(yw * 256.0f + 0.5f);
+  }
+  const int32_t minY = min(min(Y[0], Y[1]), min(Y[2], Y[3])), maxY = max(max(Y[0], Y[1]), max(Y[2], Y[3]));
+  int32_t j0 = (minY - 128 + 255) >> 8, j1 = (maxY - 128) >> 8;
+  j0 = max(j0, 0);
+  j1 = min(j1, pq.H - 1);
+  if (!bad && j0 <= j1) {
+#pragma unroll
+    for (int k = 0; k < 4; ++k) {
+      const float yaw = sdm_atan2(corner[k].y, corner[k].x);
+      float x01 = 0.5f * ((-yaw * SUMA_INV_PI_F) + 1.0f);
+      if (cppx - x01 > 0.5f) x01 += 1.0f;
+      if (x01 - cppx > 0.5f) x01 -= 1.0f;
+      const float xw = x01 * pq.width;
+      if (sdm_isnan(xw)) bad = true;
+      X[k] = (int32_t)sdm_floor(xw * 256.0f + 0.5f);
+    }
+    if (!bad) {
+      const int32_t minX = min(min(X[0], X[1]), min(X[2], X[3])), maxX = max(max(X[0], X[1]), max(X[2], X[3]));
+      int32_t i0 = (minX - 128 + 255) >> 8, i1 = (maxX - 128) >> 8;
+      i0 = max(i0, 0);
+      i1 = min(i1, pq.W - 1);
+      if (i0 <= i1) {
+        const int32_t w = i1 - i0 + 1;
+        ntests = (uint32_t)w * (uint32_t)(j1 - j0 + 1);
+#pragma unroll
+        for (int k = 0; k < 4; ++k) {
+          q[k] = X[k];
+          q[4 + k] = Y[k];
+          q[8 + k] = __float_as_int(Z[k]);
+        }
+        q[12] = i0;
+        q[13] = j0;
+        q[14] = w;
+        if (CACHE) {
+          float4* crec = qc_rec + 4 * (size_t)__float_as_uint(*idw);
+          store_stream(crec, f4(__int_as_float(X[0]), __int_as_float(X[1]), __int_as_float(X[2]), __int_as_float(X[3])));
+          store_stream(crec + 1, f4(__int_as_float(Y[0]), __int_as_float(Y[1]), __int_as_float(Y[2]), __int_as_float(Y[3])));
+          store_stream(crec + 2, f4(Z[0], Z[1], Z[2], Z[3]));
+          store_stream(crec + 3, f4(__int_as_float(i0), __int_as_float(j0), __int_as_float(w), __uint_as_float(ntests)));
+        }
+      }
+    }
+  }
+  if (CACHE && ntests == 0) qc_store_no_quad(qc_rec, __float_as_uint(*idw));
+  return ntests;
+}
+
+#define RENDER_FORM(big, qc) ((big) ? 1 : 0) + 2 * (qc)
+template <int FORM>
 __global__ void __launch_bounds__(RENDER_THREADS) __attribute__((amdgpu_waves_per_eu(5, 8))) k_render(RenderArgs a) {
+  constexpr bool BIG = (FORM & 1) != 0;
+  constexpr int QC = FORM >> 1;
   __shared__ float s_cand[RENDER_THREADS][9];
   __shared__ int32_t s_rec[RENDER_THREADS][17];
   __shared__ uint32_t s_incl[RENDER_THREADS];
@@ -176,6 +277,8 @@
 #ifndef K4_PREFETCH
     fetch_tile(tile);
 #endif
+    uint32_t qsrc = SUMA_QC_NO_SOURCE;
+    if (QC == 2 && i < S) qsrc = a.qc_src[i];
     const bool live = (i < S) && !(a.use_stability && !(s1.w > a.conf_threshold));
     const float radius = s0.w, count = s2.w;
     const int32_t creation = (int32_t)count;
@@ -197,18 +300,106 @@
           selmask = ((slot.mode == 0) ? sel_old : sel_new) ? (1u << sl) : 0u;
       }
       const bool selected = selmask != 0;
-      const bool k7 = (sl == 0) && a.k7_enabled && (i < S);
-      bool cand = false;
+      uint32_t ntests = 0;
       unsigned long long k7_key = SUMA_EMPTY_KEY;
       uint32_t k7_pix = 0;
+      if (QC == 2) {
+        const bool hasq = qsrc != SUMA_QC_NO_SOURCE;
+        float4 c0 = f4(0, 0, 0, 0), c1 = c0, c2 = c0, c3 = c0;
+        if (selected && hasq) {
+          const float4* __restrict__ cr = a.qc_rec + 4 * (size_t)qsrc;
+          c3 = cr[3];
+          c0 = cr[0];
+          c1 = cr[1];
+          c2 = cr[2];
+        }
+        const uint32_t cnt = __float_as_uint(c3.w);
+        const bool candA = cnt != 0u, candB = selected && !hasq;
+        uint32_t rA, rB, nA, nB;
+        render_block_rank2(candA, candB, s_w[trip & 1u], &rA, &rB, &nA, &nB);
+        trip += 1;
+        PH(1);
+        if (nA + nB == 0) {
+#ifdef K4_PREFETCH
+          if (sl == last_pass) fetch_tile(tile + gridDim.x);
+#endif
+          continue;
+        }
+        if (candA) {
+          int32_t* q = s_rec[rA];
+          q[0] = __float_as_int(c0.x);
+          q[1] = __float_as_int(c0.y);
+          q[2] = __float_as_int(c0.z);
+          q[3] = __float_as_int(c0.w);
+          q[4] = __float_as_int(c1.x);
+          q[5] = __float_as_int(c1.y);
+          q[6] = __float_as_int(c1.z);
+          q[7] = __float_as_int(c1.w);
+          q[8] = __float_as_int(c2.x);
+          q[9] = __float_as_int(c2.y);
+          q[10] = __float_as_int(c2.z);
+          q[11] = __float_as_int(c2.w);
+          q[12] = __float_as_int(c3.x);
+          q[13] = __float_as_int(c3.y);
+          q[14] = __float_as_int(c3.z);
+          q[15] = (int32_t)i;
+          q[16] = (int32_t)selmask;
+          s_incl[rA] = cnt;
+        }
+        if (candB) {
+          float* r = s_cand[rB];
+          r[0] = s0.x;
+          r[1] = s0.y;
+          r[2] = s0.z;
+          r[3] = s1.x;
+          r[4] = s1.y;
+          r[5] = s1.z;
+          r[6] = radius;
+          r[7] = count;
+          r[8] = __uint_as_float(i);
+          s_mask[rB] = (uint8_t)selmask;
+        }
+#ifdef K4_PREFETCH
+        if (sl == last_pass) fetch_tile(tile + gridDim.x);
+#endif
+        K4_BARRIER();
+        PH(2);
+        bool fullcand = false;
+        if (threadIdx.x < nA) {
+          ntests = s_incl[threadIdx.x];
+        } else if (threadIdx.x < nA + nB) {
+          const float* r = s_cand[threadIdx.x - nA];
+          v3 p, n;
+          surfel_to_sensor(a.poses, inv_pose, r[7], mk3(r[0], r[1], r[2]), mk3(r[3], r[4], r[5]), &p, &n);
+          const float lp = len3(p);
+          if (dot3(n, divs3(neg3(p), lp)) > 0.01f) {
+            const v3 pp = project01(a.q, p);
+            if (pp.x >= 0.0f && pp.y >= 0.0f && pp.z >= 0.0f && pp.x < 1.0f && pp.y < 1.0f && pp.z < 1.0f) {
+              fullcand = true;
+              int32_t* q = s_rec[threadIdx.x];
+              ntests = render_quad<false>(a.q, p, n, r[6], pp.x, q, nullptr, nullptr);
+              q[15] = __float_as_int(r[8]);
+              q[16] = (int32_t)s_mask[threadIdx.x - nA];
+            }
+          }
+        }
+        if (a.qc_stats != nullptr) {
+          const unsigned long long fb = __ballot(fullcand);
+          if (lane == 0 && fb) atomicAdd(&a.qc_stats[1], (unsigned long long)__popcll(fb));
+          if (threadIdx.x == 0 && nA) atomicAdd(&a.qc_stats[0], (unsigned long long)nA);
+        }
+      } else {
+      const bool k7 = (sl == 0) && a.k7_enabled && (i < S);
+      const bool geo = (QC == 1) && (i < S);
+      bool cand = false;
       v3 p = mk3(0, 0, 0), n = p;
       float ppx = 0.f;
-      if (selected || k7) {
+      if (selected || k7 || geo) {
         surfel_to_sensor(a.poses, inv_pose, count, xyz(s0), xyz(s1), &p, &n);
         float lp = len3(p);
         if (dot3(n, divs3(neg3(p), lp)) > 0.01f) {
           v3 pp = mk3(0, 0, 0);
-          if (selected || a.k7_same_proj) pp = project01(a.q, p);
+          if (selected || a.k7_same_proj || geo) pp = project01(a.q, p);
           if (k7) {
             const v3 pr = a.k7_same_proj ? pp : project01(a.k7_q, p);
             float fx = sdm_floor(pr.x * a.k7_q.width), fy = sdm_floor(pr.y * a.k7_q.height);
@@ -218,12 +409,13 @@
               k7_pix = (uint32_t)(int32_t)fy * (uint32_t)a.k7_q.W + (uint32_t)(int32_t)fx;
             }
           }
-          if (selected) {
+          if (selected || geo) {
             cand = (pp.x >= 0.0f && pp.y >= 0.0f && pp.z >= 0.0f && pp.x < 1.0f && pp.y < 1.0f && pp.z < 1.0f);
             ppx = pp.x;
           }
         }
       }
+      if (geo && !cand) qc_store_no_quad(a.qc_rec, i);
 #ifdef K4_PREFETCH
       if (sl == last_pass) fetch_tile(tile + gridDim.x);
 #endif
@@ -250,70 +442,14 @@
       }
       K4_BARRIER();
       PH(2);
-      uint32_t ntests = 0;
       if (threadIdx.x < ncand) {
         const float* r = s_cand[threadIdx.x];
-        const v3 cp = mk3(r[0], r[1], r[2]), cn = mk3(r[3], r[4], r[5]);
-        const float crad = r[6], cppx = r[7];
-        v3 u = normalize3(mk3(cn.y - cn.z, -cn.x, cn.x));
-        v3 v = normalize3(cross3(cn, u));
-        v3 ru = scale3(crad, u), rv = scale3(crad, v);
-        v3 corner[4];
-        corner[0] = sub3(sub3(cp, ru), rv);
-        corner[1] = sub3(add3(cp, ru), rv);
-        corner[2] = add3(sub3(cp, ru), rv);
-        corner[3] = add3(add3(cp, ru), rv);
-        int32_t X[4], Y[4];
-        float Z[4];
-        bool bad = false;
-#pragma unroll
-        for (int k = 0; k < 4; ++k) {
-          const float depth = len3(corner[k]);
-          const float pitch = -sdm_asin(corner[k].z / depth);
-          const float y01 = 1.0f - ((pitch * SUMA_RAD2DEG_F) + a.q.fov_up) / a.q.fov;
-          Z[k] = 0.5f * (2.0f * ((depth - a.q.min_depth) / (a.q.max_depth - a.q.min_depth)) - 1.0f) + 0.5f;
-          const float yw = y01 * a.q.height;
-          if (sdm_isnan(yw) || sdm_isnan(Z[k])) bad = true;
-          Y[k] = (int32_t)sdm_floor(yw * 256.0f + 0.5f);
-        }
-        const int32_t minY = min(min(Y[0], Y[1]), min(Y[2], Y[3])), maxY = max(max(Y[0], Y[1]), max(Y[2], Y[3]));
-        int32_t j0 = (minY - 128 + 255) >> 8, j1 = (maxY - 128) >> 8;
-        j0 = max(j0, 0);
-        j1 = min(j1, a.q.H - 1);
-        if (!bad && j0 <= j1) {
-#pragma unroll
-          for (int k = 0; k < 4; ++k) {
-            const float yaw = sdm_atan2(corner[k].y, corner[k].x);
-            float x01 = 0.5f * ((-yaw * SUMA_INV_PI_F) + 1.0f);
-            if (cppx - x01 > 0.5f) x01 += 1.0f;
-            if (x01 - cppx > 0.5f) x01 -= 1.0f;
-            const float xw = x01 * a.q.width;
-            if (sdm_isnan(xw)) bad = true;
-            X[k] = (int32_t)sdm_floor(xw * 256.0f + 0.5f);
-          }
-          if (!bad) {
-            const int32_t minX = min(min(X[0], X[1]), min(X[2], X[3])), maxX = max(max(X[0], X[1]), max(X[2], X[3]));
-            int32_t i0 = (minX - 128 + 255) >> 8, i1 = (maxX - 128) >> 8;
-            i0 = max(i0, 0);
-            i1 = min(i1, a.q.W - 1);
-            if (i0 <= i1) {
-              const int32_t w = i1 - i0 + 1;
-              ntests = (uint32_t)w * (uint32_t)(j1 - j0 + 1);
-              int32_t* q = s_rec[threadIdx.x];
-#pragma unroll
-              for (int k = 0; k < 4; ++k) {
-                q[k] = X[k];
-                q[4 + k] = Y[k];
-                q[8 + k] = __float_as_int(Z[k]);
-              }
-              q[12] = i0;
-              q[13] = j0;
-              q[14] = w;
-              q[15] = __float_as_int(r[8]);
-              q[16] = (int32_t)s_mask[threadIdx.x];
-            }
-          }
-        }
+        int32_t* q = s_rec[threadIdx.x];
+        ntests = render_quad<QC == 1>(a.q, mk3(r[0], r[1], r[2]), mk3(r[3], r[4], r[5]), r[6], r[7], q, a.qc_rec, &r[8]);
+        q[15] = __float_as_int(r[8]);
+        q[16] = (int32_t)s_mask[threadIdx.x];
+        if (QC == 1 && s_mask[threadIdx.x] == 0) ntests = 0;
+      }
       }
       PH(3);
       uint32_t incl = wave_inclusive_scan(ntests);
@@ -495,11 +631,16 @@
   for (int i = 0; i < 16; ++i) d.m[i] = s[i];
 }
 
-static void run_render(suma_ctx* c, const RenderArgs& a, uint32_t grid) {
-  if ((size_t)a.q.W * (size_t)a.q.H >= ((size_t)1 << 21))
-    k_render<true><<<grid, RENDER_THREADS, 0, c->ls>>>(a);
-  else
-    k_render<false><<<grid, RENDER_THREADS, 0, c->ls>>>(a);
+static void run_render(suma_ctx* c, const RenderArgs& a, uint32_t grid, int qc = 0) {
+  const bool big = (size_t)a.q.W * (size_t)a.q.H >= ((size_t)1 << 21);
+  switch (RENDER_FORM(big, qc)) {
+    case RENDER_FORM(false, 0): k_render<RENDER_FORM(false, 0)><<<grid, RENDER_THREADS, 0, c->ls>>>(a); break;
+    case RENDER_FORM(true, 0): k_render<RENDER_FORM(true, 0)><<<grid, RENDER_THREADS, 0, c->ls>>>(a); break;
+    case RENDER_FORM(false, 1): k_render<RENDER_FORM(false, 1)><<<grid, RENDER_THREADS, 0, c->ls>>>(a); break;
+    case RENDER_FORM(true, 1): k_render<RENDER_FORM(true, 1)><<<grid, RENDER_THREADS, 0, c->ls>>>(a); break;
+    case RENDER_FORM(false, 2): k_render<RENDER_FORM(false, 2)><<<grid, RENDER_THREADS, 0, c->ls>>>(a); break;
+    default: k_render<RENDER_FORM(true, 2)><<<grid, RENDER_THREADS, 0, c->ls>>>(a); break;
+  }
 }
 static RenderArgs render_args(suma_ctx* c, float conf_threshold, int32_t thr) {
   RenderArgs a;
@@ -519,6 +660,9 @@
   a.k7_q = c->pd;
   a.k7_same_proj = (memcmp(&c->pd, &c->pm, sizeof(proj_t)) == 0) ? 1 : 0;
   a.k7_zbuf = c->zbuf_data;
+  a.qc_rec = c->qc_rec;
+  a.qc_src = c->qc_src;
+  a.qc_stats = c->qc_stats;
   return a;
 }
 static uint32_t stream_grid(suma_ctx* c) {
@@ -541,7 +685,7 @@
 }
 
 hipError_t launch_map_render(suma_ctx* c, const float* pose_old, const float* pose_new, float conf_threshold,
-                             suma_frame* out) {
+                             suma_frame* out, int reuse_quads) {
   float inv_old[16], inv_new[16];
   rigid_inverse_f(pose_old, inv_old);
   rigid_inverse_f(pose_new, inv_new);
@@ -561,9 +705,11 @@
     a.slot[1].zbuf = c->zbuf_b;
     set_m4(a.slot[1].inv_pose, inv_new);
     a.merged = (memcmp(inv_old, inv_new, sizeof(inv_old)) == 0 && !getenv("SUMA_RENDER_NO_MERGE")) ? 1 : 0;
+    const int qc = (reuse_quads && a.merged) ? 2 : 0;
+    (qc ? c->qc.passes_reused : c->qc.passes_full) += 1;
     {
       ProfScope ps(c, "k4_render_surfels", 64.0 * S);
-      run_render(c, a, stream_grid(c));
+      run_render(c, a, stream_grid(c), qc);
     }
     ResolveArgs r = resolve_args(c);
     set_m4(r.inv_a, inv_old);
@@ -613,7 +759,7 @@
 }
 
 hipError_t launch_map_render_single(suma_ctx* c, const float* pose, float conf_threshold, int active, int fuse_k7,
-                                    suma_frame* mirror) {
+                                    suma_frame* mirror, int write_quads) {
   float inv[16] = {1, 0, 0, 0, 0, 1, 0, 0, 0, 0, 1, 0, 0, 0, 0, 1};
   if (pose) rigid_inverse_f(pose, inv);
   int32_t thr = (int32_t)(c->timestamp - 100u);
@@ -627,7 +773,7 @@
   a.k7_enabled = fuse_k7;
   {
     ProfScope ps(c, fuse_k7 ? "k4k7_render_indexmap" : "k4_render_surfels", 64.0 * (double)c->known_surfels);
-    run_render(c, a, stream_grid(c));
+    run_render(c, a, stream_grid(c), write_quads ? 1 : 0);
   }
   ResolveArgs r = resolve_args(c);
   set_m4(r.inv_a, inv);
diff --git a/semantic_suma_amd/csrc/k_update.hip b/semantic_suma_amd/csrc/k_update.hip
--- a/semantic_suma_amd/csrc/k_update.hip
+++ b/semantic_suma_amd/csrc/k_update.hip
@@ -213,6 +213,7 @@
   float* poses_inv_w;
   uint32_t pose_idx;
   int write_pose;
+  uint32_t* qc_src;
 };
 
 __device__ __forceinline__ void load_pose(const float* __restrict__ table, int32_t idx, float* M) {
@@ -517,14 +518,15 @@
         const float4 v = s_out[pb][slot][c & 3u];
         store_stream(&dst4[d], v);
         if (XF) {
-          if (s_ext[pb][slot]) {
+          if (s_ext[pb][slot] & 1) {
             const uint32_t xr = prefix_x + s_xrank[pb][slot];
             if (xr < SUMA_EXTRACT_CAPACITY && (uint64_t)xbase + xr < a.x_cap)
               store_stream(&xdst4[4ull * ((uint64_t)xbase + xr) + (c & 3u)], v);
           }
         } else if (a.ex_flags != nullptr && (c & 3u) == 0) {
-          a.ex_flags[d >> 2] = s_ext[pb][slot];
+          a.ex_flags[d >> 2] = s_ext[pb][slot] & 1;
         }
+        if ((c & 3u) == 0) a.qc_src[d >> 2] = (s_ext[pb][slot] & 2) ? SUMA_QC_NO_SOURCE : tile_id * SUMA_TILE + slot;
       }
     }
     if (tile_id == ntiles - 1 && threadIdx.x == 0) {
@@ -587,7 +589,11 @@
         const uint32_t slot = (uint32_t)u * K9_THREADS + threadIdx.x;
         xt[u] = in_tile && emit[u];
         xb[u] = XF ? __ballot(xt[u]) : 0ull;
-        s_ext[buf][slot] = in_tile ? 1 : 0;
+        const uint32_t moved = ((__float_as_uint(o.a.x) ^ __float_as_uint(in[u].a.x)) | (__float_as_uint(o.a.y) ^ __float_as_uint(in[u].a.y))) |
+                               ((__float_as_uint(o.a.z) ^ __float_as_uint(in[u].a.z)) | (__float_as_uint(o.a.w) ^ __float_as_uint(in[u].a.w))) |
+                               ((__float_as_uint(o.b.x) ^ __float_as_uint(in[u].b.x)) | (__float_as_uint(o.b.y) ^ __float_as_uint(in[u].b.y))) |
+                               ((__float_as_uint(o.b.z) ^ __float_as_uint(in[u].b.z)) | (__float_as_uint(o.c.w) ^ __float_as_uint(in[u].c.w)));
+        s_ext[buf][slot] = (in_tile ? 1 : 0) | (moved ? 2 : 0);
         s_out[buf][slot][0] = o.a;
         s_out[buf][slot][1] = o.b;
         s_out[buf][slot][2] = o.c;
@@ -782,6 +788,7 @@
       uint64_t dst = (uint64_t)base + s_prefix + (XF ? (rk & 0xffffu) : rk);
       if (dst < aT.max_surfels) {
         store_surfel(aT.out, (uint32_t)dst, s);
+        aT.qc_src[dst] = SUMA_QC_NO_SOURCE;
         if (XF) {
           if (in_tile) {
             const uint64_t xr = (uint64_t)xfirst + s_prefix_x + (rk >> 16);
@@ -895,6 +902,7 @@
   a.x_slots = c->cache_slots;
   a.x_cap = c->cache_cap;
   a.x_slot = xf ? (uint32_t)fused_slot : 0u;
+  a.qc_src = c->qc_src;
   a.ex_cx = ex ? ex[0] : 0.0f;
   a.ex_cy = ex ? ex[1] : 0.0f;
   a.ex_extent = ex ? ex[2] : 0.0f;
@@ -1119,7 +1127,7 @@
 __global__ void __launch_bounds__(256)
     k_append_cached(suma_surfel* surfels, const suma_surfel* arena, DevState* ds, const CacheSlot* slots,
                     uint32_t slot, uint32_t max_surfels, const float* poses, uint8_t* ex_flags, float ex_cx, float ex_cy,
-                    float ex_extent) {
+                    float ex_extent, uint32_t* qc_src) {
   const CacheSlot cs = slots[slot];
   const uint32_t S = ds->n_surfels;
   const float4* __restrict__ src = reinterpret_cast<const float4*>(arena + cs.offset);
@@ -1128,6 +1136,8 @@
   if ((uint64_t)S + n > max_surfels) n = max_surfels - S;
   for (uint64_t k = (uint64_t)blockIdx.x * blockDim.x + threadIdx.x; k < 4ull * n; k += (uint64_t)gridDim.x * blockDim.x)
     dst[4ull * S + k] = src[k];
+  for (uint64_t k = (uint64_t)blockIdx.x * blockDim.x + threadIdx.x; k < n; k += (uint64_t)gridDim.x * blockDim.x)
+    qc_src[S + k] = SUMA_QC_NO_SOURCE;
   if (ex_flags != nullptr)
     for (uint64_t k = (uint64_t)blockIdx.x * blockDim.x + threadIdx.x; k < n; k += (uint64_t)gridDim.x * blockDim.x) {
       const float4 pa = src[4 * k];
@@ -1155,7 +1165,7 @@
   }
   k_append_cached<<<1024, 256, 0, c->ls>>>(c->surfels[c->cur], c->cache_arena, c->ds, c->cache_slots, slot,
                                                c->p.max_surfels, c->poses, c->flagged.valid ? c->extract_flags : nullptr,
-                                               ex[0], ex[1], ex[2]);
+                                               ex[0], ex[1], ex[2], c->qc_src);
   k_append_commit<<<1, 1, 0, c->ls>>>(c->ds, c->cache_slots, slot, c->p.max_surfels);
   return hipGetLastError();
 }
diff --git a/semantic_suma_amd/csrc/suma_api.hip b/semantic_suma_amd/csrc/suma_api.hip
--- a/semantic_suma_amd/csrc/suma_api.hip
+++ b/semantic_suma_amd/csrc/suma_api.hip
@@ -216,6 +216,7 @@
   c->map_version++;
   c->rendered.valid = false;
   c->k7.valid = false;
+  c->qc.stage = 0;
   c->k8_fused_frame = nullptr;
   return SUMA_OK;
 }
@@ -294,6 +295,13 @@
     CK(hipMemsetAsync(c->zbuf_a, 0xFF, Pm * 8, c->stream));
     CK(hipMemsetAsync(c->zbuf_b, 0xFF, Pm * 8, c->stream));
     for (int b = 0; b < 2; ++b) CK(c->surfels[b].alloc(params->max_surfels));
+    CK(c->qc_rec.alloc((size_t)4 * params->max_surfels));
+    CK(c->qc_src.alloc(params->max_surfels));
+    c->qc_off = getenv("SUMA_NO_QUAD_REUSE") != nullptr;
+    if (getenv("SUMA_QUAD_REUSE_STATS")) {
+      CK(c->qc_stats.alloc(2));
+      CK(hipMemsetAsync(c->qc_stats, 0, 2 * sizeof(unsigned long long), c->stream));
+    }
     CK(c->poses.alloc((size_t)params->max_poses * 16));
     CK(c->poses_inv.alloc((size_t)params->max_poses * 16));
     c->n_tiles_cap = (uint32_t)(((size_t)params->max_surfels + 2 * P) / SUMA_TILE + 2);
@@ -1015,6 +1023,9 @@
                   memcmp(c->k7_spec.last_pose, pose, 16 * sizeof(float)) == 0))
     c->k7_spec.on = true;
   c->k7_spec.have_last = false;
+  const bool qc_ok = c->qc.stage == 1 && c->qc.map_version == c->map_version &&
+                     c->qc.params_version == c->params_version && memcmp(c->qc.pose, pose, 16 * sizeof(float)) == 0;
+  c->qc.stage = 0;
   accessed(c, frame);
   if (c->k8_fused_frame == frame && c->k8_fused_version != frame->version) c->k8_fused_frame = nullptr;
   float ex[3];
@@ -1041,6 +1052,10 @@
   int r = update_active_submaps(c, pose);
   if (r) return r;
   c->timestamp += 1;
+  if (qc_ok) {
+    c->qc.stage = 2;
+    c->qc.map_version = c->map_version;
+  }
   return SUMA_OK;
 }
 
@@ -1053,7 +1068,11 @@
       memcmp(r.pose_old, pose_old, 16 * sizeof(float)) == 0 && memcmp(r.pose_new, pose_new, 16 * sizeof(float)) == 0)
     return SUMA_OK;
   if (c->gate_pending && c->gate_frame == out) CK(flush_gate(c));
-  CK(launch_map_render(c, pose_old, pose_new, conf_threshold, out));
+  const int reuse_quads = c->qc.stage == 2 && c->qc.map_version == c->map_version &&
+                          c->qc.params_version == c->params_version &&
+                          memcmp(c->qc.pose, pose_old, 16 * sizeof(float)) == 0 &&
+                          memcmp(c->qc.pose, pose_new, 16 * sizeof(float)) == 0;
+  CK(launch_map_render(c, pose_old, pose_new, conf_threshold, out, reuse_quads));
   out->version++;
   if (c->old_frame != out) c->old_frame->version++;
   if (c->new_frame != out) c->new_frame->version++;
@@ -1091,7 +1110,7 @@
   } else if (c->k7_spec.on && c->p.data_width == c->p.model_width && !getenv("SUMA_NO_K7_SPECULATION")) {
     fuse_k7 = 1;
   }
-  CK(launch_map_render_single(c, pose, conf_threshold, 1, fuse_k7, nullptr));
+  CK(launch_map_render_single(c, pose, conf_threshold, 1, fuse_k7, nullptr, 0));
   c->new_frame->version++;
   accessed(c, c->new_frame);
   if (fuse_k7) {
@@ -1109,7 +1128,7 @@
 extern "C" int suma_map_render_inactive(suma_ctx* c, const float pose[16], float conf_threshold) {
   if (!c || !pose) return SUMA_ERR_INVALID;
   if (c->gate_pending && c->gate_frame == c->old_frame) CK(flush_gate(c));
-  CK(launch_map_render_single(c, pose, conf_threshold, 0, 0, nullptr));
+  CK(launch_map_render_single(c, pose, conf_threshold, 0, 0, nullptr, 0));
   c->old_frame->version++;
   accessed(c, c->old_frame);
   return SUMA_OK;
@@ -1631,7 +1650,9 @@
     if (r0) return r0;
   }
   c->rendered.valid = false;
-  CK(launch_map_render_single(c, nullptr, conf_threshold(s), 1, 1, s->last_model));
+  c->qc.stage = 0;
+  const int write_quads = c->qc_off ? 0 : 1;
+  CK(launch_map_render_single(c, nullptr, conf_threshold(s), 1, 1, s->last_model, write_quads));
   c->new_frame->version++;
   s->last_model->version++;
   double I[16];
@@ -1679,6 +1700,12 @@
   c->k7.map_version = c->map_version;
   c->k7.params_version = c->params_version;
   memcpy(c->k7.pose, posef, sizeof(posef));
+  if (write_quads) {
+    c->qc.stage = 1;
+    c->qc.map_version = c->map_version;
+    c->qc.params_version = c->params_version;
+    memcpy(c->qc.pose, posef, sizeof(posef));
+  }
 
   float t_err = (float)sqrt((delta[12] * delta[12] + delta[13] * delta[13]) + delta[14] * delta[14]);
   float angle = (float)(0.5 * (((delta[0] + delta[5]) + delta[10]) - 1.0));
@@ -1856,6 +1883,7 @@
   if (s->phase != 0) return fail(c, SUMA_ERR_INVALID, "suma_pipeline_integrate_loop_closures: only between scans (SurfelMapping.cpp:179)");
   int r = suma_map_update_poses(c, poses16, n);
   if (r) return r;
+  c->qc.stage = 0;
   double np[16];
   mat4_mul(difference, s->current_pose, np);
   memcpy(s->current_pose, np, sizeof(np));
@@ -1866,6 +1894,21 @@
 extern "C" int suma_pipeline_set_pose_old(suma_pipeline* s, const double pose_old[16]) {
   if (!s || !pose_old) return SUMA_ERR_INVALID;
   memcpy(s->pose_old, pose_old, sizeof(s->pose_old));
+  s->c->qc.stage = 0;
+  return SUMA_OK;
+}
+extern "C" int suma_debug_quad_reuse(suma_ctx* c, uint64_t out[4]) {
+  if (!c || !out) return SUMA_ERR_INVALID;
+  out[0] = c->qc.passes_reused;
+  out[1] = c->qc.passes_full;
+  out[2] = out[3] = 0;
+  if (c->qc_stats) {
+    unsigned long long h[2] = {0, 0};
+    CK(hipMemcpyAsync(h, c->qc_stats, sizeof(h), hipMemcpyDeviceToHost, c->stream));
+    CK(hipStreamSynchronize(c->stream));
+    out[2] = h[0];
+    out[3] = h[1];
+  }
   return SUMA_OK;
 }
 extern "C" int suma_pipeline_get_pose(const suma_pipeline* s, int which, double pose[16]) {
diff --git a/semantic_suma_amd/csrc/suma_internal.h b/semantic_suma_amd/csrc/suma_internal.h
--- a/semantic_suma_amd/csrc/suma_internal.h
+++ b/semantic_suma_amd/csrc/suma_internal.h
@@ -24,6 +24,7 @@
 #define SUMA_EXTRACT_CAPACITY 500000u
 #define SUMA_MAX_MODEL_WIDTH 5461u
 #define SUMA_MAX_HYP 64u
+#define SUMA_QC_NO_SOURCE 0xffffffffu
 
 template <class T, bool Pinned = false>
 struct DevBuf {
@@ -243,6 +244,10 @@
     uint32_t slot;
   } flagged;
   DevBuf<uint32_t> index_map;
+  DevBuf<float4> qc_rec;
+  DevBuf<uint32_t> qc_src;
+  DevBuf<unsigned long long> qc_stats;
+  bool qc_off;
   DevBuf<unsigned long long> tile_status;
   DevBuf<unsigned long long> tile_group;
   uint32_t group_words;
@@ -283,6 +288,12 @@
     float last_pose[16];
     uint64_t map_version, params_version;
   } k7_spec;
+  struct {
+    int stage;
+    float pose[16];
+    uint64_t map_version, params_version;
+    uint64_t passes_reused, passes_full;
+  } qc;
   struct {
     bool valid;
     float pose_old[16], pose_new[16], conf_threshold;
@@ -381,9 +392,9 @@
 hipError_t launch_icp_iteration(suma_ctx* c, const GnChain& ch, int eval_only, int pixel);
 const GnState* gn_result(suma_ctx* c);
 hipError_t launch_map_render(suma_ctx* c, const float* pose_old, const float* pose_new, float conf_threshold,
-                             suma_frame* out);
+                             suma_frame* out, int reuse_quads);
 hipError_t launch_map_render_single(suma_ctx* c, const float* pose, float conf_threshold, int active, int fuse_k7,
-                                    suma_frame* mirror);
+                                    suma_frame* mirror, int write_quads);
 hipError_t launch_map_render_composed(suma_ctx* c, const float* pose_old, const float* pose_new,
                                       float conf_threshold);
 hipError_t launch_map_update(suma_ctx* c, const float* pose, const float* inv_pose, const suma_frame* f, float cx,
```

Result: slower. 2683 scans/s (-6.3%).
